# lxtGH/Video-K-Net

Hardware: AMD Instinct MI355X
Metric: frames/sec (S=3, N=100, 1024x2048) (higher is better)
Workload: dtype f32; 1 GPU; cfg2 video_knet_s3_r50: VideoKernelIterHead S=3, N=100 proposals + 17 stuff = 117 kernels, C=256, 1024x2048 frame -> 128x256 stride-8 features, ffn tracking link, x4 bilinear upsample of the final logits; streams_per_gpu=1, parallelism=frame-sharded dp1, x_storage=fp32

## Files before the change

include/vkn.h:

```cpp
#ifndef VKN_H
#define VKN_H
#include <stddef.h>
#include <stdint.h>

#ifdef __cplusplus
extern "C" {
#endif

#define VKN_VERSION 0x000600

#define VKN_OK 0
#define VKN_E_ARG (-1)
#define VKN_E_SHAPE (-2)
#define VKN_E_WORKSPACE (-3)
#define VKN_E_LAUNCH (-4)
#define VKN_E_ALIGN (-5)
#define VKN_E_RANGE (-6)

#define VKN_STATUS_RANGE 1u

#define VKN_FLAG_REF_KERNELS 1u
#define VKN_FLAG_EXACT_GEMM 2u
#define VKN_FLAG_LOGITS_HANDOFF 4u
#define VKN_FLAG_BITS_HANDOFF 16u
#define VKN_X_F32 0
#define VKN_X_F16 1
#define VKN_X_BF16 2
#define VKN_FLAG_X_F16 64u
#define VKN_FLAG_X_BF16 128u
#define VKN_FLAG_CHAIN_LAUNCHES 256u
#define VKN_FLAG_CHAIN_PERSISTENT 512u
#define VKN_FLAG_JOIN_EARLY 32768u
#define VKN_FLAG_LINK_RESERVE 262144u
#define VKN_FLAG_LINK_NO_RESERVE 524288u
#define VKN_FLAG_SCALED_F16 16384u
#define VKN_FLAG_CHAIN_BF16X3 65536u
#define VKN_FLAG_CHAIN_KSPLIT 8192u
#define VKN_FLAG_SERIAL_LINK 32u
#define VKN_FLAG_CLIP_LINK 8u

#define VKN_FLAG_INIT_SEPARATE 131072u
#define VKN_FLAG_PHASE_A 1024u
#define VKN_FLAG_PHASE_B 2048u
#define VKN_FLAG_PHASE_C 4096u
#define VKN_FLAG_PHASE_MASK (VKN_FLAG_PHASE_A | VKN_FLAG_PHASE_B | VKN_FLAG_PHASE_C)

#define VKN_MAX_FCS 4

typedef struct VknDims {
    int B;
    int N;
    int C;
    int H, W;
    int heads;
    int ff;
    int ncls;
    int n_cls_fcs, n_mask_fcs;
    float thr_logit;
    float ln_eps;
} VknDims;

typedef struct VknStageWeights {
    const float *ft_w, *ft_b, *ft_wT;
    const float *dyn_w, *dyn_b;
    const float *inp_w, *inp_b;
    const float *ig_w, *ig_b, *ug_w, *ug_b;
    const float *norm_in_w, *norm_in_b;
    const float *norm_out_w, *norm_out_b;
    const float *inorm_in_w, *inorm_in_b;
    const float *inorm_out_w, *inorm_out_b;
    const float *fc_w, *fc_b, *fc_norm_w, *fc_norm_b;
    const float *attn_in_w, *attn_in_b;
    const float *attn_out_w, *attn_out_b;
    const float *attn_norm_w, *attn_norm_b;
    const float *ffn1_w, *ffn1_b;
    const float *ffn2_w, *ffn2_b;
    const float *ffn_norm_w, *ffn_norm_b;
    const float *cls_fc_w[VKN_MAX_FCS], *cls_ln_w[VKN_MAX_FCS], *cls_ln_b[VKN_MAX_FCS];
    const float *fc_cls_w, *fc_cls_b;
    const float *mask_fc_w[VKN_MAX_FCS], *mask_ln_w[VKN_MAX_FCS], *mask_ln_b[VKN_MAX_FCS];
    const float *fc_mask_w, *fc_mask_b;
    const float *pa_in_w, *pa_in_b, *pa_out_w, *pa_out_b, *pa_norm_w, *pa_norm_b;
    const float *lffn1_w, *lffn1_b, *lffn2_w, *lffn2_b, *lffn_norm_w, *lffn_norm_b;
    const void* prepared;
    size_t prepared_bytes;
} VknStageWeights;

int vkn_version(void);
const char* vkn_strerror(int code);
int vkn_workspace_init(void* ws, size_t ws_bytes, void* stream);
int vkn_workspace_status(void* ws, size_t ws_bytes, void* stream);
size_t vkn_sizeof_dims(void);
size_t vkn_sizeof_stage_weights(void);

size_t vkn_gather_workspace_bytes(int B, int N, int C, int P);
int vkn_mask_gather_f32(const float* x, const float* mask_logits, float thr_logit, float* xraw_out, float* cnt_out, int B,
                        int N, int C, int P, void* ws, size_t ws_bytes, unsigned flags, void* stream);

int vkn_mask_gather_real_f32(const float* x, const float* a, float* out, float* asum_out, int B, int N, int C, int P, void* ws,
                             size_t ws_bytes, void* stream);

size_t vkn_decode_workspace_bytes(int B, int N, int C);
int vkn_mask_decode_f32(const float* x, const float* kernels, const float* bias, float* out, int B, int N, int C, int P,
                        void* ws, size_t ws_bytes, unsigned flags, void* stream);
int vkn_mask_decode_scaled_f32(const float* x, const float* kernels, const float* bias, const float* out_scale, float* out, int B,
                               int N, int C, int P, void* ws, size_t ws_bytes, unsigned flags, void* stream);

int vkn_split_planes_f32(const float* kernels, void* kf_hi, void* kf_lo, int B, int N, int C, void* stream);
int vkn_mask_decode_planes_f32(const float* x, const void* kf_hi, const void* kf_lo, const float* bias, float* out, int B,
                               int N, int C, int P, void* stream);
int vkn_mask_decode_planes_x(const void* x, int x_dtype, const void* kf_hi, const void* kf_lo, const float* bias, float* out, int B,
                             int N, int C, int P, void* stream);

int vkn_decode_gather_supported(int C, int P);
int vkn_decode_gather_f32(const float* x, const void* kf_hi, const void* kf_lo, const float* bias, float thr_logit,
                          float* xraw_out, float* cnt_out, int B, int N, int C, int P, void* ws, size_t ws_bytes, void* stream);
int vkn_decode_gather_x(const void* x, int x_dtype, const void* kf_hi, const void* kf_lo, const float* bias, float thr_logit,
                        float* xraw_out, float* cnt_out, int B, int N, int C, int P, void* ws, size_t ws_bytes, void* stream);

int vkn_upsample_bilinear_f32(const float* in, float* out, int planes, int H, int W, int S, void* stream);
int vkn_upsample_bilinear_f16out(const float* in, void* out_f16, int planes, int H, int W, int S, void* stream);
int vkn_upsample_bilinear_bwd_f32(const float* grad_out, float* grad_in, int planes, int H, int W, int S, void* stream);

int vkn_focal_loss_blocks(int M, int ncls);
int vkn_focal_loss_f32(const float* logits, const long long* labels, const float* weight, int weight_elementwise, int M, int ncls,
                       float alpha, float gamma, float* partial, float* grad, void* stream);

size_t vkn_prepared_bytes(const VknDims* d, const VknStageWeights* w);
int vkn_prepare_stage_f32(const VknDims* d, const VknStageWeights* w, void* prepared, size_t bytes, void* stream);

int vkn_split_weight_f32(const float* W, void* w_split, int Nout, int K, void* stream);
int vkn_linear_f32(const float* A, const float* W, const void* w_split, const float* bias, float* out, int M, int K, int Nout,
                   int act, int ksplit, void* ws, size_t ws_bytes, void* stream);

int vkn_split_weight_t_f32(const float* W, void* w_split_t, int Nout, int K, void* stream);
#define VKN_SPLIT_MAX_ITEMS 64
typedef struct VknSplitItem {
    const float* W;
    void* images;
    long long ldn, ldk;
    int Nout, K, kvalid, reserved;
} VknSplitItem;
size_t vkn_sizeof_split_item(void);
int vkn_split_weights_batch_f32(const VknSplitItem* items, int nitems, void* stream);
int vkn_linear_dw_f32(const float* dY, int ldy, const float* A, int lda, float* dW, float* db, int M, int K, int Nout, int accumulate,
                      void* stream);
#define VKN_DW_MAX_ITEMS 48
typedef struct VknDwItem {
    const float* dY;
    const float* A;
    float* dW;
    float* db;
    int ldy, lda, Nout, K;
} VknDwItem;
size_t vkn_sizeof_dw_item(void);
int vkn_linear_dw_batch_f32(const VknDwItem* items, int nitems, int M, void* stream);
int vkn_layernorm_act_fwd_f32(const float* in, int ldi, const float* resid, int ldr, const float* gamma, const float* beta, float eps,
                              int act, float* out, int ldo, float* stats, int M, int C, void* stream);
int vkn_layernorm_act_bwd_f32(const float* dy, int lddy, const float* in, int ldi, const float* resid, int ldr, const float* gamma,
                              const float* beta, const float* stats, int act, float* dx, int lddx, float* dgamma, float* dbeta, int M,
                              int C, void* stream);
typedef struct VknUpdatorNorms {
    const float *norm_in_w, *norm_in_b, *norm_out_w, *norm_out_b, *input_norm_in_w, *input_norm_in_b, *input_norm_out_w, *input_norm_out_b;
    const float *input_gate_b, *update_gate_b;
} VknUpdatorNorms;
typedef struct VknUpdatorNormGrads {
    float *norm_in_w, *norm_in_b, *norm_out_w, *norm_out_b, *input_norm_in_w, *input_norm_in_b, *input_norm_out_w, *input_norm_out_b;
} VknUpdatorNormGrads;
size_t vkn_sizeof_updator_norms(void);
size_t vkn_sizeof_updator_norm_grads(void);
int vkn_updator_gate_product_f32(const float* params, const float* inputs, float* gate_feats, int M, int C, void* stream);
int vkn_updator_gate_product_bwd_f32(const float* d_gate_feats, const float* params, const float* inputs, float* d_params, float* d_inputs,
                                     int M, int C, void* stream);
int vkn_updator_mix_fwd_f32(const float* gates, const float* params, const float* inputs, const VknUpdatorNorms* norms, float eps,
                            float* features, float* stats, int M, int C, void* stream);
int vkn_updator_mix_bwd_f32(const float* d_features, const float* gates, const float* params, const float* inputs,
                            const VknUpdatorNorms* norms, const float* stats, float* d_gates, float* d_params, float* d_inputs,
                            const VknUpdatorNormGrads* d_norms, int M, int C, void* stream);
int vkn_attention_f32(const float* Q, int ldq, const float* K, const float* V, int ldkv, float* out, int ldo, int B, int Nq, int Nk,
                      int heads, int hd, void* stream);
int vkn_attention_bwd_f32(const float* Q, int ldq, const float* K, const float* V, int ldkv, const float* O, int ldo, const float* dO,
                          int lddo, float* dQ, int lddq, float* dK, float* dV, int lddkv, int B, int Nq, int Nk, int heads, int hd,
                          void* stream);

int vkn_kernel_updator_f32(const VknDims* d, const VknStageWeights* w, const float* update_feature,
                           const float* input_feature, float* out, void* ws, size_t ws_bytes, void* stream);

size_t vkn_stage_workspace_bytes(const VknDims* d);
int vkn_stage_forward_f32(const VknDims* d, const VknStageWeights* w, const float* x, const float* obj_in,
                          const float* masks_in, const float* prev_obj, float* cls_logits, float* masks_out, float* obj_out,
                          float* x_feat_out, float* track_out, void* ws, size_t ws_bytes, unsigned flags, void* stream);

int vkn_track_link_f32(const VknDims* d, const VknStageWeights* w, const float* cur_obj, const float* prev_obj,
                       float* track_out, void* ws, size_t ws_bytes, void* stream);
int vkn_track_link_flags_f32(const VknDims* d, const VknStageWeights* w, const float* cur_obj, const float* prev_obj,
                             float* track_out, void* ws, size_t ws_bytes, unsigned flags, void* stream);

int vkn_link_block_f32(const VknDims* d, const VknStageWeights* w, const float* update_feature, const float* cur,
                       const float* prev, float* out, void* ws, size_t ws_bytes, void* stream);

size_t vkn_query_merge_workspace_bytes(const VknDims* d, int num_frames);
int vkn_query_merge_f32(const VknDims* d, int num_frames, const VknStageWeights* w, const float* query, const float* keys,
                        const float* pos, float* out, void* ws, size_t ws_bytes, void* stream);

int vkn_stage_forward_link_f32(const VknDims* d, const VknStageWeights* w, const VknStageWeights* link_pre,
                               const VknStageWeights* link_track, int track_src, const float* x, const float* obj_in,
                               const float* masks_in, const float* prev_obj, float* cls_logits, float* masks_out, float* obj_out,
                               float* x_feat_out, float* track_out, void* ws, size_t ws_bytes, unsigned flags, void* stream);

int vkn_stage_chain_f32(const VknDims* d, const VknStageWeights* w, const float* x_feat, const float* obj_in, float* cls_logits,
                        float* kernels_out, float* kb_out, float* obj_out, void* ws, size_t ws_bytes, unsigned flags,
                        void* stream);

size_t vkn_head_workspace_bytes(const VknDims* d);
int vkn_head_forward_f32(const VknDims* d, int num_stages, const VknStageWeights* stages, const float* x,
                         const float* proposal_feats, const float* mask_preds_in, const float* prev_obj, float* obj_out,
                         float* cls_prob, float* mask_preds_out, float* scaled_out, int upsample_stride, float* track_out,
                         void* ws, size_t ws_bytes, unsigned flags, void* stream);

int vkn_head_forward_link_f32(const VknDims* d, int num_stages, const VknStageWeights* stages, const VknStageWeights* link_pre,
                              const VknStageWeights* link_track, int track_src, const float* x, const float* proposal_feats,
                              const float* mask_preds_in, const float* prev_obj, float* obj_out, float* cls_prob,
                              float* mask_preds_out, float* scaled_out, int upsample_stride, float* track_out, void* ws,
                              size_t ws_bytes, unsigned flags, void* stream);

int vkn_head_forward_prof_f32(const VknDims* d, int num_stages, const VknStageWeights* stages, const float* x,
                              const float* proposal_feats, const float* mask_preds_in, const float* prev_obj, float* obj_out,
                              float* cls_prob, float* mask_preds_out, float* scaled_out, int upsample_stride, float* track_out,
                              void* ws, size_t ws_bytes, unsigned flags, void* stream, void* ev_decode_start,
                              void* ev_decode_stop);

size_t vkn_kernel_init_workspace_bytes(int B, int Np, int ncls, int C, int P);
int vkn_kernel_init_f32(const float* loc_feats, const float* sem_feats, const float* init_w, const float* seg_w,
                        const float* seg_b, int num_thing_classes, int cat_stuff, int with_obj, float thr_logit, float* x_feats,
                        float* mask_preds, float* seg_preds, float* proposal_feats, int B, int Np, int ncls, int C, int P,
                        void* ws, size_t ws_bytes, unsigned flags, void* stream);

typedef struct VknPanopticCfg {
    int num_proposals;
    int num_thing_classes;
    int max_per_img;
    float instance_score_thr;
    double overlap_thr;
    int up;
    int Hm, Wm;
    int Hb, Wb;
    int h, w;
    int Ho, Wo;
} VknPanopticCfg;
#define VKN_PANOPTIC_INFO_FIELDS 6
size_t vkn_sizeof_panoptic_cfg(void);
size_t vkn_panoptic_workspace_bytes(const VknPanopticCfg* cfg, int B, int N);
int vkn_panoptic_joint_f32(const VknPanopticCfg* cfg, const float* cls_prob, const float* mask_logits, int B, int N, int ncls,
                           int* panoptic_seg, int* info, int* nseg, int* bbox, void* ws, size_t ws_bytes, void* stream);

size_t vkn_merge_workspace_bytes(int Kt, int Ks);
int vkn_panoptic_thing_first_u8(const unsigned char* thing_masks, const float* thing_scores, const int* thing_labels,
                                const int* thing_order, int Kt, const unsigned char* stuff_masks, const int* stuff_labels,
                                const int* stuff_order, int Ks, int HW, double instance_score_thr, double iou_thr,
                                int stuff_max_area, int* panoptic_seg, int* info, int* nseg, void* ws, size_t ws_bytes,
                                void* stream);

typedef struct VknAssignCfg {
    float cls_weight, dice_weight, mask_weight;
    float focal_alpha, focal_gamma, focal_eps;
    float dice_eps;
    float dice_pred_min, mask_pred_min;
} VknAssignCfg;
size_t vkn_sizeof_assign_cfg(void);
size_t vkn_assign_workspace_bytes(int N, int G, int P);
int vkn_assign_costs_f32(const VknAssignCfg* cfg, const float* mask_logits, const float* cls_logits, const float* gt_masks,
                         const int* gt_labels, int N, int G, int ncls, int P, float* cost_out, void* ws, size_t ws_bytes,
                         void* stream);
typedef struct VknAssignProblem {
    const float* mask_logits;
    const float* cls_logits;
    const float* gt_masks;
    const int* gt_labels;
    int G;
    float* cost_out;
} VknAssignProblem;
size_t vkn_sizeof_assign_problem(void);
int vkn_assign_costs_batch_f32(const VknAssignCfg* cfg, const VknAssignProblem* probs, int nprob, int N, int ncls, int P, void* ws,
                               size_t ws_bytes, void* stream);
size_t vkn_assign_lowres_workspace_bytes(int nprob, int N, int Gmax, int h, int w, int S);
int vkn_assign_costs_lowres_batch_f32(const VknAssignCfg* cfg, const VknAssignProblem* probs, int nprob, int N, int ncls, int h, int w,
                                      int S, void* ws, size_t ws_bytes, void* stream);
int vkn_lsap_f32(const float* cost, int nr, int nc, int* row_ind, int* col_ind);
#define VKN_LSAP_MAX_BATCH 64
typedef struct VknLsapProblem {
    const float* cost;
    int nr, nc;
    long long* gt_inds;
    int* row_ind;
    int* col_ind;
} VknLsapProblem;
size_t vkn_sizeof_lsap_problem(void);
int vkn_lsap_batch_f32(const VknLsapProblem* probs, int nprob, int* status, void* stream);

int vkn_mask_losses_chunks(int P);
int vkn_mask_losses_blocks(int P);
int vkn_mask_losses_fwd_f32(const float* pred, const float* target, const long long* pos_rows, const int* rowk, int K, int B, int Ns,
                            int P, int with_rank, float* row_partial, float* lse, int* top, float* rank_partial, void* stream);
int vkn_mask_losses_bwd_f32(const float* pred, const float* target, const int* rowk, const float* rowcoef, const float* coef,
                            const float* lse, const int* top, int B, int Ns, int P, int with_rank, float* grad, void* stream);

#define VKN_TAIL_MAX_IMAGES 64
typedef struct VknTailImage {
    const int* row_ind;
    const int* col_ind;
    const long long* gt_labels;
    const long long* sem_cls;
    int k, n_sem;
    int gt_row0, sem_row0;
    int pos0;
    int reserved;
} VknTailImage;
typedef struct VknTailCfg {
    float w_cls, w_mask, w_dice, dice_eps, w_rank, avg_factor;
    int with_rank;
} VknTailCfg;
size_t vkn_sizeof_tail_image(void);
size_t vkn_sizeof_tail_cfg(void);
int vkn_stage_targets(const VknTailImage* imgs, int B, int N, int S, int T, int ncls, float pos_weight, long long* labels,
                      float* label_weights, float* row_weight, int* rowk, long long* pos_rows, int* tgt_row, int* status, void* stream);
int vkn_mask_losses_fwd_bank_f32(const float* pred, const float* bank, const int* tgt_row, const long long* pos_rows, const int* rowk,
                                 int K, int B, int Ns, int P, int with_rank, float* row_partial, float* lse, int* top,
                                 float* rank_partial, void* stream);
int vkn_stage_losses_final_f32(const VknTailCfg* cfg, const float* avg_factor_dev, const float* focal_partial, int n_focal,
                               const float* row_partial, int K, int nchunk, const float* rank_partial, int n_rank,
                               const float* cls_logits, const long long* labels, const long long* pos_rows, int ncls, int B, int P,
                               float* losses, float* dice_a, float* dice_bc, void* stream);
int vkn_mask_losses_bwd_bank_f32(const float* pred, const float* bank, const int* tgt_row, const int* rowk, const float* dice_a,
                                 const float* dice_bc, const float* g_mask, const float* g_dice, const float* g_rank, float w_mask,
                                 float w_dice, float w_rank, int K, const float* lse, const int* top, int B, int Ns, int P,
                                 int with_rank, float* grad, void* stream);
int vkn_mask_losses_bwd_lowres_f32(const float* low, const float* bank, const int* tgt_row, const int* rowk, const float* dice_a,
                                   const float* dice_bc, const float* g_mask, const float* g_dice, const float* g_rank, float w_mask,
                                   float w_dice, float w_rank, int K, const float* lse, const int* top, int B, int Ns, int h, int w, int S,
                                   int with_rank, float* grad_low, void* stream);
// ... 75 lines not shown
```

video-k-net_amd/csrc/vkn_api.hip:

```cpp
#include "../../include/vkn.h"
#include "../../include/vkn_decode.h"
#include "vkn_common.h"
#include "vkn_launch.h"

namespace {

struct Carver {
    char* base;
    size_t off;
    template <class T>
    T* take(size_t n) {
        off = (off + 255) & ~(size_t)255;
        T* p = base ? reinterpret_cast<T*>(base + off) : nullptr;
        off += n * sizeof(T);
        return p;
    }
};

inline bool aligned16(const void* p) { return (reinterpret_cast<uintptr_t>(p) & 15) == 0; }
inline int npt_of(int N) { return (N + 31) / 32 * 32; }

struct StageWs {
    float *part, *cntp, *xraw, *cnt, *xfeat, *params, *inputf, *ig, *ug, *f, *obj1, *qkv, *ao, *obj2, *h, *partial, *t1, *t2,
        *maskfeat, *kb, *kern32, *lq, *lkv, *lobj, *lupd, *lf;
    _Float16 *kfh, *kfl;
    int* status;
};


enum MasksFrom {
    FROM_LOGITS,
    FROM_BITS,
    FROM_GATHERED,
    FROM_XFEAT
};
enum MasksTo {
    TO_LOGITS,
    TO_BITS,
    TO_GATHER,
    TO_KERNELS,
    TO_NONE
};
struct StageCall {
    const VknStageWeights* w = nullptr;
    const float *x = nullptr, *obj_in = nullptr;
    float *obj_out = nullptr, *cls_logits = nullptr, *x_feat_out = nullptr;
    bool cls_sigmoid = false;
    MasksFrom from = FROM_LOGITS;
    const float *masks_in = nullptr, *xfeat_in = nullptr;
    const unsigned* bits_in = nullptr;
    MasksTo to = TO_LOGITS;
    float* masks_out = nullptr;
    unsigned* bits_out = nullptr;
    float *kern_out = nullptr, *kb_out = nullptr;
    hipEvent_t prof0 = nullptr, prof1 = nullptr, obj_ready = nullptr;
    float* up_out = nullptr;
    int up_stride = 0, up_chunk = 0;
    bool* up_done = nullptr;
    int link_reserve = 0;
    const float* prev_obj = nullptr;
    float* track_out = nullptr;
    const VknStageWeights* link_pre = nullptr;
    const float* prev_pre = nullptr;
    const VknStageWeights* link_track = nullptr;
    int track_src = 0;
    bool keep_xfeat = false;
    const void* touch_next = nullptr;
    size_t touch_next_bytes = 0;
};

struct PrepW {
    const void *ft, *ftT, *dyn, *inp, *ig, *ug, *fc, *attn_in, *attn_out, *ffn1, *ffn2, *cls_fc[VKN_MAX_FCS], *fc_cls,
        *mask_fc[VKN_MAX_FCS], *fc_mask, *pa_in, *pa_in_kv, *pa_out, *lffn1, *lffn2;
    const void *dynft, *dec;
    float *dynft32, *bcnt, *dec32, *decb, *dvec, *kb0, *fmT;
    float* chain_consts;
    const void* h2[VKN_H2_COUNT];
    float* h2_scale;
    unsigned* h2_scratch;
};

inline bool has_composites(const VknDims* d, const VknStageWeights* w) {
    return w->ft_w && w->ft_wT && w->ft_b && w->dyn_w && w->dyn_b && w->fc_mask_w && w->fc_mask_b && d->n_mask_fcs > 0;
}

struct PrepItem {
    const float* src;
    int nout, k;
    const void** dst;
};

struct H2Shape { int nout, k; };
inline H2Shape h2_shape(const VknDims* d, const VknStageWeights* w, int i) {
    const int C = d->C, FF = d->ff;
    switch (i) {
        case VKN_H2_DYNFT: case VKN_H2_DYN: case VKN_H2_INP: return H2Shape{2 * C, C};
        case VKN_H2_IN: return H2Shape{3 * C, C};
        case VKN_H2_FFN1: return H2Shape{FF, C};
        case VKN_H2_FFN2: return H2Shape{C, FF};
        case VKN_H2_FCCLS: return H2Shape{w->fc_cls_w ? d->ncls : 0, C};
        default: return H2Shape{C, C};
    }
}

inline bool chain_width_ok(const VknDims* d) { return d->C == 256 && d->ff % 256 == 0 && d->ff <= 2048; }
inline bool chain_shape_ok(const VknDims* d) { return chain_width_ok(d) && d->n_cls_fcs == 1 && d->n_mask_fcs == 1; }

size_t carve_prepared(const VknDims* d, const VknStageWeights* w, char* base, PrepW* p, PrepItem* it = nullptr, int* n_out = nullptr) {
    const int C = d->C, FF = d->ff;
    Carver c{base, 0};
    int n = 0;
    auto add = [&](const float* src, int nout, int k, const void** dst) {
        *dst = src ? c.take<char>(vkn_split_w3_bytes(nout, k)) : nullptr;
        if (src && it) it[n] = PrepItem{src, nout, k, dst};
        if (src) ++n;
    };
    add(w->ft_w, C, C, &p->ft); add(w->ft_wT, C, C, &p->ftT);
    add(w->dyn_w, 2 * C, C, &p->dyn); add(w->inp_w, 2 * C, C, &p->inp);
    add(w->ig_w, C, C, &p->ig); add(w->ug_w, C, C, &p->ug); add(w->fc_w, C, C, &p->fc);
    add(w->attn_in_w, 3 * C, C, &p->attn_in); add(w->attn_out_w, C, C, &p->attn_out);
    add(w->ffn1_w, FF, C, &p->ffn1); add(w->ffn2_w, C, FF, &p->ffn2);
    for (int i = 0; i < VKN_MAX_FCS; ++i) add(i < d->n_cls_fcs ? w->cls_fc_w[i] : nullptr, C, C, &p->cls_fc[i]);
    add(w->fc_cls_w, d->ncls, C, &p->fc_cls);
    for (int i = 0; i < VKN_MAX_FCS; ++i) add(i < d->n_mask_fcs ? w->mask_fc_w[i] : nullptr, C, C, &p->mask_fc[i]);
    add(w->fc_mask_w, C, C, &p->fc_mask);
    add(w->pa_in_w, C, C, &p->pa_in); add(w->pa_in_w ? w->pa_in_w + (size_t)C * C : nullptr, 2 * C, C, &p->pa_in_kv);
    add(w->pa_out_w, C, C, &p->pa_out);
    add(w->lffn1_w, FF, C, &p->lffn1); add(w->lffn2_w, C, FF, &p->lffn2);
    p->dynft = p->dec = nullptr;
    p->dynft32 = p->bcnt = p->dec32 = p->decb = p->dvec = p->kb0 = p->fmT = p->chain_consts = nullptr;
    if (has_composites(d, w)) {
        const size_t Cs = d->C;
        p->dynft = c.take<char>(vkn_split_w3_bytes(2 * C, C));
        p->dec = c.take<char>(vkn_split_w3_bytes(C, C));
        p->dynft32 = c.take<float>(2 * Cs * Cs);
        p->bcnt = c.take<float>(2 * Cs);
        p->dec32 = c.take<float>(Cs * Cs);
        p->decb = c.take<float>(Cs);
        p->dvec = c.take<float>(Cs);
        p->kb0 = c.take<float>(4);
        p->fmT = c.take<float>(Cs * Cs);
        if (C == 256 && FF <= 2048) p->chain_consts = c.take<float>(vkn_chain_consts_floats());
    }
    for (int i = 0; i < VKN_H2_COUNT; ++i) p->h2[i] = nullptr;
    p->h2_scale = nullptr;
    p->h2_scratch = nullptr;
    if (has_composites(d, w) && chain_shape_ok(d) && w->inp_w && w->ig_w && w->ug_w && w->fc_w && w->attn_in_w && w->attn_out_w && w->ffn1_w &&
        w->ffn2_w && w->cls_fc_w[0] && w->mask_fc_w[0]) {
        for (int i = 0; i < VKN_H2_COUNT; ++i) {
            const H2Shape h = h2_shape(d, w, i);
            if (h.nout > 0) p->h2[i] = c.take<char>(vkn_split_h2_bytes(h.nout, h.k));
        }
        p->h2_scale = c.take<float>(VKN_H2_COUNT * 8);
        p->h2_scratch = c.take<unsigned>(4);
    }
    if (n_out) *n_out = n;
    return (c.off + 255) & ~(size_t)255;
}

int ffn_hsplit(int M, int FF) {
    if (FF % 256 != 0) return 0;
    const int chunks = FF / 256, rt = (M + 31) / 32;
    int hs = 1;
    while (hs < chunks && rt * hs < 256 && chunks % (hs * 2) == 0) hs *= 2;
    return hs;
}

int ffn_ksplit(int M, int K) {
    const int rt = (M + 31) / 32, ktiles = K / 32;
    int ks = 256 / (rt > 0 ? rt : 1);
    if (ks > 16) ks = 16;
    if (ks > ktiles) ks = ktiles;
    if (ks < 1) ks = 1;
    return ks;
}

size_t carve_stage(const VknDims* d, char* base, StageWs* s) {
    Carver c{base, 0};
    const size_t B = d->B, N = d->N, C = d->C, P = (size_t)d->H * d->W, M = B * N, FF = d->ff;
    const size_t G = vkn_gather_groups(d->B, (int)P), NPT = npt_of(d->N);
    s->status = c.take<int>(64);
    s->part = c.take<float>(B * G * NPT * C);
    s->cntp = c.take<float>(B * G * NPT);
    s->xraw = c.take<float>(M * C);
    s->cnt = c.take<float>(M);
    s->xfeat = c.take<float>(M * C);
    s->params = c.take<float>(M * 2 * C);
    s->inputf = c.take<float>(M * 2 * C);
    s->ig = c.take<float>(M * 2 * C);
    s->ug = c.take<float>(M * C);
    s->f = c.take<float>(M * C);
    s->obj1 = c.take<float>(M * C);
    s->qkv = c.take<float>(M * 3 * C);
    s->ao = c.take<float>(M * C);
    s->obj2 = c.take<float>(M * C);
    s->h = c.take<float>(M * FF);
    {
        const size_t ks = (size_t)ffn_ksplit((int)M, (int)FF), hs = (size_t)ffn_hsplit((int)M, (int)FF);
        const size_t ks1 = (size_t)ffn_ksplit((int)N, (int)FF), hs1 = (size_t)ffn_hsplit((int)N, (int)FF);
        const size_t k4 = 4;
        const size_t a = (ks > hs ? (ks > k4 ? ks : k4) : (hs > k4 ? hs : k4)) * M * C, b1 = (ks1 > hs1 ? (ks1 > k4 ? ks1 : k4) : (hs1 > k4 ? hs1 : k4)) * N * C;
        s->partial = c.take<float>(a > b1 ? a : b1);
    }
    s->t1 = c.take<float>(M * C);
    s->t2 = c.take<float>(M * C);
    s->maskfeat = c.take<float>(M * C);
    s->kb = c.take<float>(M);
    s->kern32 = c.take<float>(M * C);
    s->lq = c.take<float>(M * C);
    s->lkv = c.take<float>(M * 2 * C);
    s->lobj = c.take<float>(M * C);
    s->lupd = c.take<float>(M * C);
    s->lf = c.take<float>(M * C);
    s->kfh = c.take<_Float16>(B * NPT * C);
    s->kfl = c.take<_Float16>(B * NPT * C);
    return (c.off + 255) & ~(size_t)255;
}

int stage_ws(const VknDims* d, void* ws, size_t ws_bytes, StageWs* s) {
    if (!ws || ws_bytes < carve_stage(d, nullptr, s) || !aligned16(ws)) return VKN_E_WORKSPACE;
    carve_stage(d, static_cast<char*>(ws), s);
    return VKN_OK;
}

struct GatherWs { float *part, *cntp, *cnt; };
size_t carve_gather(int B, int N, int C, int P, char* base, GatherWs* g) {
    const size_t G = vkn_gather_groups(B, P), NPT = npt_of(N);
    Carver c{base, 0};
    g->part = c.take<float>((size_t)B * G * NPT * C);
    g->cntp = c.take<float>((size_t)B * G * NPT);
    g->cnt = c.take<float>((size_t)B * N);
    return (c.off + 255) & ~(size_t)255;
}
size_t carve_planes(int B, int N, int C, char* base, _Float16** kfh, _Float16** kfl) {
    Carver c{base, 0};
    *kfh = c.take<_Float16>((size_t)B * npt_of(N) * C);
    *kfl = c.take<_Float16>((size_t)B * npt_of(N) * C);
    return (c.off + 255) & ~(size_t)255;
}

int check_dims(const VknDims* d) {
    if (!d) return VKN_E_ARG;
    if (d->B <= 0 || d->N <= 0 || d->C <= 0 || d->H <= 0 || d->W <= 0 || d->heads <= 0 || d->ff <= 0 || d->ncls <= 0)
        return VKN_E_ARG;
    if (d->C % 32 != 0 || d->C > 256) return VKN_E_SHAPE;
    if (d->C % d->heads != 0 || d->C / d->heads > 64 || (d->C % 8) != 0 || d->C / 8 > 64) return VKN_E_SHAPE;
    {
        const int hd = d->C / d->heads, hd8 = d->C / 8;
        if (hd < 4 || (hd & (hd - 1)) || hd8 < 4 || (hd8 & (hd8 - 1))) return VKN_E_SHAPE;
    }
    if (d->ff % 32 != 0) return VKN_E_SHAPE;
    if (d->N > 256) return VKN_E_SHAPE;
    if (d->ncls > 256) return VKN_E_SHAPE;
    if (d->n_cls_fcs < 0 || d->n_cls_fcs > VKN_MAX_FCS || d->n_mask_fcs < 0 || d->n_mask_fcs > VKN_MAX_FCS) return VKN_E_SHAPE;
    return VKN_OK;
}

inline int xdt_of(unsigned flags) { return (flags & VKN_FLAG_X_F16) ? 1 : ((flags & VKN_FLAG_X_BF16) ? 2 : 0); }

VknEpi mk_epi(const VknDims* d) {
    VknEpi e{};
    e.eps = d->ln_eps;
    return e;
}

#define VKN_TRY(expr)             \
    do {                          \
        const int rc_ = (expr);   \
        if (rc_ != VKN_OK) return rc_; \
    } while (0)

int run_ffn(const VknDims* d, const StageWs& s, const float* in, const float* w1, const void* w1s, const float* b1,
            const float* w2, const void* w2s, const float* b2, const float* nw, const float* nb, float* out, hipStream_t st) {
    const int M = d->B * d->N, C = d->C, FF = d->ff;
    VknEpi e = mk_epi(d);
    int hsplit = ffn_hsplit(M, FF);
    {
        const int hs_dbg = vkn_dbg_env("VKN_FFN_HS", 0);
        if (hs_dbg > 0 && hs_dbg <= hsplit) hsplit = hs_dbg;
    }
    if (w1s && w2s && C == 256 && hsplit > 0 && vkn_dbg_env("VKN_FFN_FUSED", 1) != 0) {
        e.bias = b2; e.resid = in; e.ldr = C; e.ln_w = nw; e.ln_b = nb; e.out = out; e.ldo = C;
        return vkn_launch_ffn_fused(in, C, w1s, b1, w2s, M, C, FF, hsplit, s.partial, e, st);
    }
    e.bias = b1; e.act = 1; e.out = s.h; e.ldo = FF;
    VKN_TRY(vkn_launch_gemm(in, nullptr, C, w1, w1s, M, C, FF, 1, nullptr, e, st));
    e = mk_epi(d);
    e.bias = b2; e.resid = in; e.ldr = C; e.ln_w = nw; e.ln_b = nb; e.out = out; e.ldo = C;
    return vkn_launch_gemm(s.h, nullptr, FF, w2, w2s, M, FF, C, ffn_ksplit(M, FF), s.partial, e, st);
}

int run_attention(const VknDims* d, const StageWs& s, const float* qsrc, const float* kvsrc, int heads, const float* in_w,
                  const void* in_ws, const void* in_kv_ws, const float* in_b, const float* out_w, const void* out_ws, const float* out_b,
                  const float* nw, const float* nb, float* out, hipStream_t st) {
    const int M = d->B * d->N, C = d->C, hd = C / heads;
    VknEpi e = mk_epi(d);
    if (qsrc == kvsrc) {
        e.bias = in_b; e.out = s.qkv; e.ldo = 3 * C;
        VKN_TRY(vkn_launch_gemm(qsrc, nullptr, C, in_w, in_ws, M, C, 3 * C, 1, nullptr, e, st));
        VKN_TRY(vkn_launch_attn(s.qkv, 3 * C, s.qkv + C, s.qkv + 2 * C, 3 * C, s.ao, C, d->B, d->N, d->N, heads, hd, st));
    } else {
        e.bias = in_b; e.out = s.lq; e.ldo = C;
        VKN_TRY(vkn_launch_gemm(qsrc, nullptr, C, in_w, in_ws, M, C, C, 1, nullptr, e, st));
        e = mk_epi(d);
        e.bias = in_b + C; e.out = s.lkv; e.ldo = 2 * C;
        VKN_TRY(vkn_launch_gemm(kvsrc, nullptr, C, in_w + (size_t)C * C, in_kv_ws, M, C, 2 * C, 1, nullptr, e, st));
        VKN_TRY(vkn_launch_attn(s.lq, C, s.lkv, s.lkv + C, 2 * C, s.ao, C, d->B, d->N, d->N, heads, hd, st));
    }
    e = mk_epi(d);
    e.bias = out_b; e.resid = qsrc; e.ldr = C; e.ln_w = nw; e.ln_b = nb; e.out = out; e.ldo = C;
    return vkn_launch_gemm(s.ao, nullptr, C, out_w, out_ws, M, C, C, 1, nullptr, e, st);
}

int run_updator(const VknDims* d, const VknStageWeights* w, const PrepW& pw, const float* xfeat, const float* xraw,
                const float* cnt, const float* obj_in, float* out, const StageWs& s, hipStream_t st) {
    const int C = d->C, M = d->B * d->N;
    const bool fuse = (C == 256);
    VknGemmProb pr[2];
    VknEpi e = mk_epi(d); e.out = s.params; e.ldo = 2 * C;
    if (fuse) { e.ln_w = w->norm_out_w; e.ln_b = w->norm_out_b; e.ln_from_col = C; }
    if (xraw && pw.dynft) {
        e.bias = pw.bcnt; e.rowscale = cnt; e.bias2 = w->dyn_b;
        pr[0] = VknGemmProb{xraw, nullptr, nullptr, nullptr, C, pw.dynft32, pw.dynft, 2 * C, e};
    } else {
        e.bias = w->dyn_b;
        pr[0] = VknGemmProb{xfeat, nullptr, nullptr, nullptr, C, w->dyn_w, pw.dyn, 2 * C, e};
    }
    e = mk_epi(d); e.bias = w->inp_b; e.out = s.inputf; e.ldo = 2 * C;
    if (fuse) { e.ln_w = w->inorm_out_w; e.ln_b = w->inorm_out_b; e.ln_from_col = C; }
    pr[1] = VknGemmProb{obj_in, nullptr, nullptr, nullptr, C, w->inp_w, pw.inp, 2 * C, e};
    VKN_TRY(vkn_launch_gemm_group(pr, 2, M, C, 1, nullptr, st));
    float* ig = s.ig;
    float* ug = fuse ? s.ig + C : s.ug;
    const int ldg = fuse ? 2 * C : C;
    e = mk_epi(d); e.bias = w->ig_b; e.ln_w = w->inorm_in_w; e.ln_b = w->inorm_in_b; e.act = 2; e.out = ig; e.ldo = ldg;
    pr[0] = VknGemmProb{s.inputf, s.params, nullptr, nullptr, 2 * C, w->ig_w, pw.ig, C, e};
    e = mk_epi(d); e.bias = w->ug_b; e.ln_w = w->norm_in_w; e.ln_b = w->norm_in_b; e.act = 2; e.out = ug; e.ldo = ldg;
    pr[1] = VknGemmProb{s.inputf, s.params, nullptr, nullptr, 2 * C, w->ug_w, pw.ug, C, e};
    VKN_TRY(vkn_launch_gemm_group(pr, 2, M, C, 1, nullptr, st));
    e = mk_epi(d); e.bias = w->fc_b; e.ln_w = w->fc_norm_w; e.ln_b = w->fc_norm_b; e.act = 1; e.out = out; e.ldo = C;
    if (fuse) {
        pr[0] = VknGemmProb{ug, s.params + C, ig, s.inputf + C, 2 * C, w->fc_w, pw.fc, C, e};
        return vkn_launch_gemm_group(pr, 1, M, C, 1, nullptr, st);
    }
    VKN_TRY(vkn_launch_ku_mix(s.params, s.inputf, ig, ug, w->norm_out_w, w->norm_out_b, w->inorm_out_w, w->inorm_out_b,
                              d->ln_eps, s.f, M, C, st));
    return vkn_launch_gemm(s.f, nullptr, C, w->fc_w, pw.fc, M, C, C, 1, nullptr, e, st);
}

bool link_ks_ok(const VknDims* d, const VknStageWeights* w, const PrepW& pw, unsigned flags);
int run_link_ks(const VknDims* d, const VknStageWeights* w, const PrepW& pw, const float* cur, const float* kv, float* out,
                const StageWs& s, hipStream_t st);
int run_link(const VknDims* d, const VknStageWeights* w, const PrepW& pw, const float* cur, const float* prev,
             float* out, const StageWs& s, hipStream_t st, const float* update_feature = nullptr, unsigned flags = 0) {
    if (!w->pa_in_w || !w->lffn1_w) return VKN_E_ARG;
    const float* kv = prev;
    if (update_feature) {
        if (!w->dyn_w) return VKN_E_ARG;
        StageWs su = s;
        su.f = s.lf;
        VKN_TRY(run_updator(d, w, pw, update_feature, nullptr, nullptr, prev, s.lupd, su, st));
        kv = s.lupd;
    }
    if (link_ks_ok(d, w, pw, flags)) return run_link_ks(d, w, pw, cur, kv, out, s, st);
    VKN_TRY(run_attention(d, s, cur, kv, 8, w->pa_in_w, pw.pa_in, pw.pa_in_kv, w->pa_in_b, w->pa_out_w, pw.pa_out, w->pa_out_b,
                          w->pa_norm_w, w->pa_norm_b, s.t1, st));
    return run_ffn(d, s, s.t1, w->lffn1_w, pw.lffn1, w->lffn1_b, w->lffn2_w, pw.lffn2, w->lffn2_b, w->lffn_norm_w,
                   w->lffn_norm_b, out, st);
}

int carve_pw(const VknDims* d, const VknStageWeights* w, unsigned flags, PrepW* pw) {
    *pw = PrepW{};
    if (w->prepared && !(flags & VKN_FLAG_EXACT_GEMM) &&
        carve_prepared(d, w, static_cast<char*>(const_cast<void*>(w->prepared)), pw) > w->prepared_bytes)
        return VKN_E_WORKSPACE;
    return VKN_OK;
}

int run_track_link(const VknDims* d, const StageWs& s, hipStream_t st, const float* cur, const float* prev, float* out,
                   const VknStageWeights* w, const VknStageWeights* link_track, int track_src, const float* xfeat, unsigned flags) {
    const VknStageWeights* lw = link_track ? link_track : w;
    PrepW pw;
    VKN_TRY(carve_pw(d, lw, flags, &pw));
    return run_link(d, lw, pw, cur, prev, out, s, st, link_track ? (track_src == 2 ? cur : xfeat) : nullptr, flags);
}

int run_gather(const VknDims* d, const float* x, const float* masks, const unsigned* bits, const StageWs& s, unsigned flags,
               hipStream_t st, const void* touch = nullptr, size_t touch_bytes = 0) {
    const int B = d->B, N = d->N, C = d->C, P = d->H * d->W, xdt = xdt_of(flags);
    if (flags & VKN_FLAG_REF_KERNELS) return vkn_launch_gather_ref(x, masks, d->thr_logit, s.xraw, s.cnt, B, N, C, P, st);
    if (bits) return vkn_launch_gather_bits(x, bits, s.xraw, s.cnt, s.part, s.cntp, B, N, C, P, st, xdt, s.status, touch, touch_bytes);
    return vkn_launch_gather(x, masks, d->thr_logit, s.xraw, s.cnt, s.part, s.cntp, B, N, C, P, st, xdt, s.status, touch, touch_bytes);
}

int final_decode(const VknDims* d, const float* x, const StageWs& s, const float* kb, float* masks_out, unsigned flags,
                 hipStream_t st, hipEvent_t prof0, hipEvent_t prof1, float* up_out, int up_stride, int up_chunk, bool* up_done,
                 int max_workgroups = 0) {
    const int B = d->B, N = d->N, C = d->C, P = d->H * d->W;
    if ((flags & VKN_FLAG_REF_KERNELS) || (P & 1)) return vkn_launch_decode_ref(x, s.kern32, kb, masks_out, B, N, C, P, st);
    const int ch = (up_out && up_chunk > 0 && up_chunk < B) ? up_chunk : B;
    const size_t NPTC = (size_t)npt_of(N) * C;
    for (int b0 = 0; b0 < B; b0 += ch) {
        const int bn = (B - b0 < ch) ? B - b0 : ch;
        const float* xb = reinterpret_cast<const float*>(reinterpret_cast<const char*>(x) + (size_t)b0 * C * P * (xdt_of(flags) ? 2 : 4));
        if (b0 == 0 && prof0 && hipEventRecord(prof0, st) != hipSuccess) return VKN_E_LAUNCH;
        VKN_TRY(vkn_launch_decode_wg(xb, s.kfh + b0 * NPTC, s.kfl + b0 * NPTC, kb ? kb + (size_t)b0 * N : nullptr,
                                     masks_out + (size_t)b0 * N * P, bn, N, C, P, ch == B ? max_workgroups : 0, st, xdt_of(flags)));
        if (b0 == 0 && prof1 && hipEventRecord(prof1, st) != hipSuccess) return VKN_E_LAUNCH;
        if (ch < B)
            VKN_TRY(vkn_launch_upsample(masks_out + (size_t)b0 * N * P,
                                        (flags & VKN_FLAG_SCALED_F16) ? reinterpret_cast<float*>(reinterpret_cast<_Float16*>(up_out) + (size_t)b0 * N * P * up_stride * up_stride)
                                                                      : up_out + (size_t)b0 * N * P * up_stride * up_stride,
                                        bn * N, d->H, d->W, up_stride, st, (flags & VKN_FLAG_SCALED_F16) ? 1 : 0));
    }
    if (ch < B && up_done) *up_done = true;
    return VKN_OK;
}

#define VKN_LINK_RESERVE_CUS 64
#define VKN_LINK_RESERVE_MIN_FRAMES 8
inline int link_reserve_wg(const VknDims* d, int mode, bool persistent_chain, unsigned flags) {
    const VknDecodeSplit dflt = vkn_decode_split(d->B, d->H * d->W, 0);
    const long long grid = (long long)d->B * dflt.G2;
    const int full = VKN_DECODE_CUS - VKN_LINK_RESERVE_CUS;
    if (mode == 2) {
        const long long q = grid * 3 / 4;
        return (int)(q > full ? full : (q < d->B ? d->B : q));
    }
    if (mode != 1 || !persistent_chain || d->B < VKN_LINK_RESERVE_MIN_FRAMES || xdt_of(flags) != 0) return 0;
    return grid == VKN_DECODE_CUS ? full : 0;
}

inline int persistent_min_row_tiles(const PrepW& pw, unsigned flags) {
    return (!(flags & VKN_FLAG_CHAIN_BF16X3) && pw.h2_scale && pw.h2[VKN_H2_DYNFT]) ? 22 : 64;
}
inline unsigned pw_off(const VknStageWeights* w, const void* p) {
    return (unsigned)(static_cast<const char*>(p) - static_cast<const char*>(w->prepared));
}
inline bool chain_weights_ok(const PrepW& pw, bool have_cls) {
    return pw.dynft && pw.dyn && pw.dec && pw.inp && pw.ig && pw.ug && pw.fc && pw.attn_in && pw.attn_out && pw.ffn1 && pw.ffn2 &&
           pw.cls_fc[0] && pw.mask_fc[0] && (!have_cls || pw.fc_cls);
}
inline bool chain_stage_ok(const VknDims* d, const VknStageWeights* w, const PrepW& pw, bool have_cls) {
    return chain_shape_ok(d) && w->prepared && w->prepared_bytes < (1ull << 31) && chain_weights_ok(pw, have_cls) && w->ffn1_w &&
           w->cls_ln_w[0] && w->mask_ln_w[0];
}
bool chain_fast_ok(const VknDims* d, const VknStageWeights* w, const PrepW& pw, unsigned flags, bool have_cls) {
    if (flags & (VKN_FLAG_CHAIN_LAUNCHES | VKN_FLAG_EXACT_GEMM)) return false;
    if (vkn_dbg_env("VKN_CHAIN_LAUNCHES", 0)) return false;
    if (!(flags & VKN_FLAG_CHAIN_PERSISTENT) && !vkn_dbg_env("VKN_CHAIN_PERSISTENT", 0) &&
        (d->B * d->N + 31) / 32 < persistent_min_row_tiles(pw, flags))
        return false;
    return pw.chain_consts && chain_stage_ok(d, w, pw, have_cls);
}
inline bool chain_h2(const PrepW& pw, unsigned flags, bool have_cls) {
    return !(flags & VKN_FLAG_CHAIN_BF16X3) && pw.h2_scale && pw.h2[VKN_H2_DYNFT] && pw.h2[VKN_H2_DEC] && (!have_cls || pw.h2[VKN_H2_FCCLS]);
}

int run_chain_fast(const VknDims* d, const VknStageWeights* w, const PrepW& pw, const float* a0, bool a0_raw, const float* cnt,
                   const float* obj_in, float* obj_out, float* cls_logits, bool cls_sigmoid, float* kern32_out, const StageWs& s,
                   hipStream_t st, bool h2 = false) {
    const int M = d->B * d->N, C = d->C;
    VknChainA a{};
    a.a0 = a0; a.obj_in = obj_in; a.rowscale = a0_raw ? cnt : nullptr;
    a.wbase = w->prepared; a.wbytes = w->prepared_bytes;
    if (h2) {
        a.off_dyn = pw_off(w, pw.h2[a0_raw ? VKN_H2_DYNFT : VKN_H2_DYN]);
        a.off_inp = pw_off(w, pw.h2[VKN_H2_INP]); a.off_ig = pw_off(w, pw.h2[VKN_H2_IG]); a.off_ug = pw_off(w, pw.h2[VKN_H2_UG]);
        a.off_fc = pw_off(w, pw.h2[VKN_H2_FC]); a.off_in = pw_off(w, pw.h2[VKN_H2_IN]);
    } else {
        a.off_dyn = pw_off(w, a0_raw ? pw.dynft : pw.dyn);
        a.off_inp = pw_off(w, pw.inp); a.off_ig = pw_off(w, pw.ig); a.off_ug = pw_off(w, pw.ug); a.off_fc = pw_off(w, pw.fc);
        a.off_in = pw_off(w, pw.attn_in);
    }
    a.consts = pw.chain_consts;
    a.eps = d->ln_eps; a.M = M; a.obj1 = s.obj1; a.qkv = s.qkv; a.status = s.status;
    VKN_TRY(h2 ? vkn_launch_chain_a_h2(a, st) : vkn_launch_chain_a(a, st));
    VKN_TRY(vkn_launch_attn(s.qkv, 3 * C, s.qkv + C, s.qkv + 2 * C, 3 * C, s.ao, C, d->B, d->N, d->N, d->heads, C / d->heads, st));
    VknChainC c{};
    c.ao = s.ao; c.obj1 = s.obj1; c.wbase = w->prepared; c.wbytes = w->prepared_bytes;
    if (h2) {
        c.off_out = pw_off(w, pw.h2[VKN_H2_OUT]); c.off_ffn1 = pw_off(w, pw.h2[VKN_H2_FFN1]); c.off_ffn2 = pw_off(w, pw.h2[VKN_H2_FFN2]);
        c.off_clsfc = pw_off(w, pw.h2[VKN_H2_CLSFC]); c.off_maskfc = pw_off(w, pw.h2[VKN_H2_MASKFC]);
        c.off_fccls = pw.h2[VKN_H2_FCCLS] ? pw_off(w, pw.h2[VKN_H2_FCCLS]) : 0u; c.off_dec = pw_off(w, pw.h2[VKN_H2_DEC]);
    } else {
        c.off_out = pw_off(w, pw.attn_out); c.off_ffn1 = pw_off(w, pw.ffn1); c.off_ffn2 = pw_off(w, pw.ffn2);
        c.off_clsfc = pw_off(w, pw.cls_fc[0]); c.off_maskfc = pw_off(w, pw.mask_fc[0]);
        c.off_fccls = pw.fc_cls ? pw_off(w, pw.fc_cls) : 0u; c.off_dec = pw_off(w, pw.dec);
    }
    c.consts = pw.chain_consts; c.kb0 = pw.kb0;
    c.ff = d->ff; c.ncls = d->ncls; c.cls_sigmoid = cls_sigmoid ? 1 : 0; c.eps = d->ln_eps; c.M = M;
    c.obj_out = obj_out; c.cls_out = cls_logits; c.kb_out = s.kb;
    if (kern32_out) c.kern_out = kern32_out;
    else { c.plane_hi = s.kfh; c.plane_lo = s.kfl; }
    c.rows_per_frame = d->N; c.NPT = npt_of(d->N); c.status = s.status;
    return h2 ? vkn_launch_chain_c_h2(c, st) : vkn_launch_chain_c(c, st);
}

#define VKN_KS_MAX_ROW_TILES 16
inline bool ks_width_ok(const VknDims* d) {
    return chain_width_ok(d) && (d->ff % 512 == 0 || d->ff <= 1024);
}
bool chain_ks_ok(const VknDims* d, const VknStageWeights* w, const PrepW& pw, unsigned flags, bool have_cls) {
    if (flags & (VKN_FLAG_CHAIN_LAUNCHES | VKN_FLAG_CHAIN_PERSISTENT | VKN_FLAG_EXACT_GEMM)) return false;
    if (vkn_dbg_env("VKN_CHAIN_LAUNCHES", 0) || vkn_dbg_env("VKN_CHAIN_PERSISTENT", 0) || !vkn_dbg_env("VKN_CHAIN_KSPLIT", 1)) return false;
    if (!(flags & VKN_FLAG_CHAIN_KSPLIT) && (d->B * d->N + 31) / 32 > VKN_KS_MAX_ROW_TILES) return false;
    if (!ks_width_ok(d) || !chain_stage_ok(d, w, pw, have_cls)) return false;
    const void* v16[] = {w->inorm_in_w, w->inorm_in_b, w->norm_in_w, w->norm_in_b, w->norm_out_w, w->norm_out_b, w->inorm_out_w, w->inorm_out_b,
                         w->fc_norm_w, w->fc_norm_b, w->attn_norm_w, w->attn_norm_b, w->ffn_norm_w, w->ffn_norm_b, w->ffn2_b,
                         w->cls_ln_w[0], w->cls_ln_b[0], w->mask_ln_w[0], w->mask_ln_b[0], pw.dvec};
    for (const void* p : v16)
        if (!p || !aligned16(p)) return false;
    return true;
}

VknKsProb ks_prob(const float* a, int lda, const void* W, int Nout, int KT, float eps) {
    VknKsProb p{};
    p.pro.a[0] = a; p.pro.lda[0] = lda; p.pro.nsum = 1; p.pro.eps = eps;
    p.Wsplit = W; p.Nout = Nout; p.KT = KT;
    return p;
}

int run_chain_ks(const VknDims* d, const VknStageWeights* w, const PrepW& pw, const float* a0, bool a0_raw, const float* cnt,
                 const float* obj_in, float* obj_out, float* cls_logits, bool cls_sigmoid, float* kern32_out, const StageWs& s,
                 hipStream_t st, hipEvent_t obj_ready) {
    const int M = d->B * d->N, C = d->C, FF = d->ff;
    const float eps = d->ln_eps;
    VknKsProb pr[2];
    pr[0] = ks_prob(a0, C, a0_raw ? pw.dynft : pw.dyn, 2 * C, 8, eps);
    if (a0_raw) { pr[0].epi.bias = pw.bcnt; pr[0].epi.rowscale = cnt; pr[0].epi.bias2 = w->dyn_b; }
    else pr[0].epi.bias = w->dyn_b;
    pr[0].epi.out = s.params; pr[0].epi.ldo = 2 * C;
    pr[1] = ks_prob(obj_in, C, pw.inp, 2 * C, 8, eps);
    pr[1].epi.bias = w->inp_b; pr[1].epi.out = s.inputf; pr[1].epi.ldo = 2 * C;
    VKN_TRY(vkn_launch_gemm_ks(pr, 2, 0, 0, 1, 0, M, st));
    pr[0] = ks_prob(s.inputf, 2 * C, pw.ig, C, 8, eps);
    pr[0].pro.a[1] = s.params; pr[0].pro.lda[1] = 2 * C;
    pr[1] = pr[0];
    pr[0].epi.bias = w->ig_b; pr[0].epi.out = s.ig; pr[0].epi.ldo = 2 * C;
    pr[1].Wsplit = pw.ug; pr[1].epi.bias = w->ug_b; pr[1].epi.out = s.ig + C; pr[1].epi.ldo = 2 * C;
    VKN_TRY(vkn_launch_gemm_ks(pr, 2, 1, 0, 1, 0, M, st));
    pr[0] = ks_prob(s.ig, 2 * C, pw.fc, C, 8, eps);
    pr[0].pro.a[1] = s.ig + C; pr[0].pro.lda[1] = 2 * C;
    pr[0].pro.a[2] = s.params + C; pr[0].pro.lda[2] = 2 * C;
    pr[0].pro.a[3] = s.inputf + C; pr[0].pro.lda[3] = 2 * C;
    pr[0].pro.ln_w[0] = w->inorm_in_w; pr[0].pro.ln_b[0] = w->inorm_in_b;
    pr[0].pro.ln_w[1] = w->norm_in_w; pr[0].pro.ln_b[1] = w->norm_in_b;
    pr[0].pro.ln_w[2] = w->norm_out_w; pr[0].pro.ln_b[2] = w->norm_out_b;
    pr[0].pro.ln_w[3] = w->inorm_out_w; pr[0].pro.ln_b[3] = w->inorm_out_b;
    pr[0].epi.bias = w->fc_b; pr[0].epi.out = s.f; pr[0].epi.ldo = C;
    VKN_TRY(vkn_launch_gemm_ks(pr, 1, 2, 0, 1, 0, M, st));
    pr[0] = ks_prob(s.f, C, pw.attn_in, 3 * C, 8, eps);
    pr[0].pro.ln_w[0] = w->fc_norm_w; pr[0].pro.ln_b[0] = w->fc_norm_b; pr[0].pro.act = 1;
    pr[0].pro.side_out = s.obj1; pr[0].pro.ld_side = C;
    pr[0].epi.bias = w->attn_in_b; pr[0].epi.out = s.qkv; pr[0].epi.ldo = 3 * C;
    VKN_TRY(vkn_launch_gemm_ks(pr, 1, 0, 0, 1, 0, M, st));
    VKN_TRY(vkn_launch_attn(s.qkv, 3 * C, s.qkv + C, s.qkv + 2 * C, 3 * C, s.ao, C, d->B, d->N, d->N, d->heads, C / d->heads, st));
    pr[0] = ks_prob(s.ao, C, pw.attn_out, C, 8, eps);
    pr[0].epi.bias = w->attn_out_b; pr[0].epi.resid = s.obj1; pr[0].epi.ldr = C; pr[0].epi.out = s.obj2; pr[0].epi.ldo = C;
    VKN_TRY(vkn_launch_gemm_ks(pr, 1, 0, 0, 1, 0, M, st));
    pr[0] = ks_prob(s.obj2, C, pw.ffn1, FF, 8, eps);
    pr[0].pro.ln_w[0] = w->attn_norm_w; pr[0].pro.ln_b[0] = w->attn_norm_b;
    pr[0].pro.side_out = s.t1; pr[0].pro.ld_side = C;
    pr[0].epi.bias = w->ffn1_b; pr[0].epi.act = 1; pr[0].epi.out = s.h; pr[0].epi.ldo = FF;
    VKN_TRY(vkn_launch_gemm_ks(pr, 1, 0, 0, 1, 0, M, st));
    const int kpw = (FF % 512 == 0) ? 2 : 1, zch = FF / (256 * kpw);
    pr[0] = ks_prob(s.h, FF, pw.ffn2, C, FF / 32, eps);
    pr[0].epi.out = s.partial; pr[0].epi.ldo = C;
    VKN_TRY(vkn_launch_gemm_ks(pr, 1, 0, zch, kpw, (long long)M * C, M, st));
    pr[0] = ks_prob(s.partial, C, pw.cls_fc[0], C, 8, eps);
    pr[0].pro.nsum = zch; pr[0].pro.sum_stride = (long long)M * C;
    pr[0].pro.pbias = w->ffn2_b; pr[0].pro.presid = s.t1; pr[0].pro.ldr = C;
    pr[0].pro.ln_w[0] = w->ffn_norm_w; pr[0].pro.ln_b[0] = w->ffn_norm_b;
    pr[1] = pr[0];
    pr[0].pro.side_out = obj_out; pr[0].pro.ld_side = C;
    pr[0].epi.out = s.lkv; pr[0].epi.ldo = 2 * C;
    pr[1].Wsplit = pw.mask_fc[0]; pr[1].epi.out = s.lkv + C; pr[1].epi.ldo = 2 * C;
    VKN_TRY(vkn_launch_gemm_ks(pr, 2, 0, 0, 1, 0, M, st));
    if (obj_ready && hipEventRecord(obj_ready, st) != hipSuccess) return VKN_E_LAUNCH;
    int np = 0;
    if (cls_logits) {
        pr[np] = ks_prob(s.lkv, 2 * C, pw.fc_cls, d->ncls, 8, eps);
        pr[np].pro.ln_w[0] = w->cls_ln_w[0]; pr[np].pro.ln_b[0] = w->cls_ln_b[0]; pr[np].pro.act = 1;
        pr[np].epi.bias = w->fc_cls_b; pr[np].epi.act = cls_sigmoid ? 2 : 0; pr[np].epi.out = cls_logits; pr[np].epi.ldo = d->ncls;
        ++np;
    }
    pr[np] = ks_prob(s.lkv + C, 2 * C, pw.dec, C, 8, eps);
    pr[np].pro.ln_w[0] = w->mask_ln_w[0]; pr[np].pro.ln_b[0] = w->mask_ln_b[0]; pr[np].pro.act = 1;
    pr[np].pro.dot_vec = pw.dvec; pr[np].pro.dot_bias = pw.kb0; pr[np].pro.dot_out = s.kb;
    pr[np].epi.bias = pw.decb; pr[np].epi.ldo = C;
    if (kern32_out) pr[np].epi.out = kern32_out;
    else { pr[np].epi.plane_hi = s.kfh; pr[np].epi.plane_lo = s.kfl; pr[np].epi.rows_per_frame = d->N; pr[np].epi.NPT = npt_of(d->N); }
    ++np;
    return vkn_launch_gemm_ks(pr, np, 0, 0, 1, 0, M, st);
}

bool link_ks_ok(const VknDims* d, const VknStageWeights* w, const PrepW& pw, unsigned flags) {
    if (flags & (VKN_FLAG_CHAIN_LAUNCHES | VKN_FLAG_CHAIN_PERSISTENT | VKN_FLAG_EXACT_GEMM)) return false;
    if (vkn_dbg_env("VKN_CHAIN_LAUNCHES", 0) || !vkn_dbg_env("VKN_CHAIN_KSPLIT", 1)) return false;
    if (!(flags & VKN_FLAG_CHAIN_KSPLIT) && (d->B * d->N + 31) / 32 > VKN_KS_MAX_ROW_TILES) return false;
    if (!ks_width_ok(d)) return false;
    if (!pw.pa_in || !pw.pa_in_kv || !pw.pa_out || !pw.lffn1 || !pw.lffn2) return false;
    if (!w->pa_norm_w || !w->pa_norm_b || !aligned16(w->pa_norm_w) || !aligned16(w->pa_norm_b)) return false;
    return true;
}

int run_link_ks(const VknDims* d, const VknStageWeights* w, const PrepW& pw, const float* cur, const float* kv, float* out,
                const StageWs& s, hipStream_t st) {
    const int M = d->B * d->N, C = d->C, FF = d->ff;
    const float eps = d->ln_eps;
    VknKsProb pr[2];
    pr[0] = ks_prob(cur, C, pw.pa_in, C, 8, eps);
    pr[0].epi.bias = w->pa_in_b; pr[0].epi.out = s.lq; pr[0].epi.ldo = C;
    pr[1] = ks_prob(kv, C, pw.pa_in_kv, 2 * C, 8, eps);
    pr[1].epi.bias = w->pa_in_b ? w->pa_in_b + C : nullptr; pr[1].epi.out = s.lkv; pr[1].epi.ldo = 2 * C;
    VKN_TRY(vkn_launch_gemm_ks(pr, 2, 0, 0, 1, 0, M, st));
    VKN_TRY(vkn_launch_attn(s.lq, C, s.lkv, s.lkv + C, 2 * C, s.ao, C, d->B, d->N, d->N, 8, C / 8, st));
    pr[0] = ks_prob(s.ao, C, pw.pa_out, C, 8, eps);
    pr[0].epi.bias = w->pa_out_b; pr[0].epi.resid = cur; pr[0].epi.ldr = C; pr[0].epi.out = s.t1; pr[0].epi.ldo = C;
    VKN_TRY(vkn_launch_gemm_ks(pr, 1, 0, 0, 1, 0, M, st));
    pr[0] = ks_prob(s.t1, C, pw.lffn1, FF, 8, eps);
    pr[0].pro.ln_w[0] = w->pa_norm_w; pr[0].pro.ln_b[0] = w->pa_norm_b;
    pr[0].pro.side_out = s.lf; pr[0].pro.ld_side = C;
    pr[0].epi.bias = w->lffn1_b; pr[0].epi.act = 1; pr[0].epi.out = s.h; pr[0].epi.ldo = FF;
    VKN_TRY(vkn_launch_gemm_ks(pr, 1, 0, 0, 1, 0, M, st));
    const int kpw = (FF % 512 == 0) ? 2 : 1, zch = FF / (256 * kpw);
    pr[0] = ks_prob(s.h, FF, pw.lffn2, C, FF / 32, eps);
    pr[0].epi.out = s.partial; pr[0].epi.ldo = C;
    VKN_TRY(vkn_launch_gemm_ks(pr, 1, 0, zch, kpw, (long long)M * C, M, st));
    VknEpi e = mk_epi(d);
    e.bias = w->lffn2_b; e.resid = s.lf; e.ldr = C; e.ln_w = w->lffn_norm_w; e.ln_b = w->lffn_norm_b; e.out = out; e.ldo = C;
    return vkn_launch_rowepi(s.partial, zch, M, C, e, st);
}

int emit_masks(const VknDims* d, const StageCall& c, const StageWs& s, bool ref_decode, const float* kern32, const float* kb,
               const void* touch, size_t touch_bytes, unsigned flags, hipStream_t st, bool persistent_chain = false) {
    const int B = d->B, N = d->N, C = d->C, P = d->H * d->W, xdt = xdt_of(flags);
    if (c.to == TO_KERNELS) {
        if (c.kb_out && kb && hipMemcpyAsync(c.kb_out, kb, (size_t)B * N * sizeof(float), hipMemcpyDeviceToDevice, st) != hipSuccess)
            return VKN_E_LAUNCH;
        return VKN_OK;
    }
    if (c.to == TO_NONE) return VKN_OK;
    if (ref_decode) return vkn_launch_decode_ref(c.x, kern32, kb, c.masks_out, B, N, C, P, st);
    if (c.to == TO_GATHER)
        return vkn_launch_fused_decode_gather(c.x, s.kfh, s.kfl, kb, d->thr_logit, s.xraw, s.cnt, s.part, s.cntp, B, N, C, P, st, xdt, s.status,
                                              touch, touch_bytes);
    if (c.to == TO_BITS) return vkn_launch_decode_bits(c.x, s.kfh, s.kfl, kb, c.bits_out, d->thr_logit, B, N, C, P, st, xdt);
    return final_decode(d, c.x, s, kb, c.masks_out, flags, st, c.prof0, c.prof1, c.up_out, c.up_stride, c.up_chunk, c.up_done,
                        link_reserve_wg(d, c.link_reserve, persistent_chain, flags));
}

int run_stage(const VknDims* d, const StageCall& c, const StageWs& s, unsigned flags, hipStream_t st) {
    const VknStageWeights* w = c.w;
    const int N = d->N, C = d->C, P = d->H * d->W, M = d->B * N;
    const bool ref = (flags & VKN_FLAG_REF_KERNELS) != 0;
    const bool chain_only = c.to == TO_KERNELS, given_xfeat = c.from == FROM_XFEAT;
    const bool ref_decode = ref || (P & 1) || chain_only;
    const bool has_ft = w->ft_w != nullptr;
    const bool have_cls = w->fc_cls_w && c.cls_logits;
    float* const cls_logits = have_cls ? c.cls_logits : nullptr;
    const bool pre_link = c.link_pre && c.prev_pre;
    const bool need_xfeat = (pre_link && c.link_pre->dyn_w) || (c.link_track && c.track_src == 1) || c.keep_xfeat;
    if (xdt_of(flags) && !chain_only && (ref || (P % 64) != 0)) return VKN_E_SHAPE;
    PrepW pw;
    VKN_TRY(carve_pw(d, w, flags, &pw));
    const bool comp = pw.dynft != nullptr;
    const bool fewrow = comp && chain_ks_ok(d, w, pw, flags, have_cls), persistent = comp && chain_fast_ok(d, w, pw, flags, have_cls);
    const bool fast = fewrow || persistent;

    const bool will_fast = !given_xfeat && persistent && vkn_dbg_env("VKN_CHAIN_TOUCH", 1);
    const void* touch_nx = vkn_dbg_env("VKN_CHAIN_TOUCH", 1) ? c.touch_next : nullptr;
    const size_t touch_nx_bytes = touch_nx ? c.touch_next_bytes : 0;
    if (c.from == FROM_LOGITS || c.from == FROM_BITS)
        VKN_TRY(run_gather(d, c.x, c.masks_in, c.from == FROM_BITS ? c.bits_in : nullptr, s, flags, st, will_fast ? w->prepared : nullptr,
                           will_fast ? w->prepared_bytes : 0));

    float* xfeat = c.x_feat_out ? c.x_feat_out : s.xfeat;
    VknEpi e = mk_epi(d);
    if (given_xfeat) {
        xfeat = const_cast<float*>(c.xfeat_in);
    } else if (has_ft) {
        if (!comp || c.x_feat_out || need_xfeat) {
            e.bias = w->ft_b; e.rowscale = s.cnt; e.out = xfeat; e.ldo = C;
            VKN_TRY(vkn_launch_gemm(s.xraw, nullptr, C, w->ft_w, pw.ft, M, C, C, 1, nullptr, e, st));
        }
    } else {
        if (hipMemcpyAsync(xfeat, s.xraw, (size_t)M * C * sizeof(float), hipMemcpyDeviceToDevice, st) != hipSuccess)
            return VKN_E_LAUNCH;
    }

    const float* obj_in = c.obj_in;
    if (pre_link) {
        PrepW pl;
        VKN_TRY(carve_pw(d, c.link_pre, flags, &pl));
        VKN_TRY(run_link(d, c.link_pre, pl, obj_in, c.prev_pre, s.lobj, s, st, c.link_pre->dyn_w ? xfeat : nullptr, flags));
        obj_in = s.lobj;
    }

    const float* kb = has_ft ? s.kb : nullptr;
    float* const kern32 = ref_decode ? (chain_only ? c.kern_out : s.kern32) : nullptr;
    const bool link = c.prev_obj && c.track_out;
    if (fast) {
        const bool raw = !given_xfeat;
        if (fewrow) {
            VKN_TRY(run_chain_ks(d, w, pw, raw ? s.xraw : xfeat, raw, s.cnt, obj_in, c.obj_out, cls_logits, c.cls_sigmoid, kern32, s, st, c.obj_ready));
        } else {
            VKN_TRY(run_chain_fast(d, w, pw, raw ? s.xraw : xfeat, raw, s.cnt, obj_in, c.obj_out, cls_logits, c.cls_sigmoid, kern32, s, st,
                                   chain_h2(pw, flags, have_cls)));
            if (c.obj_ready && hipEventRecord(c.obj_ready, st) != hipSuccess) return VKN_E_LAUNCH;
        }
        VKN_TRY(emit_masks(d, c, s, ref_decode, s.kern32, kb, touch_nx, touch_nx_bytes, flags, st, !fewrow));
        if (link) VKN_TRY(run_track_link(d, s, st, c.obj_out, c.prev_obj, c.track_out, w, c.link_track, c.track_src, xfeat, flags));
        return VKN_OK;
    }

    VKN_TRY(run_updator(d, w, pw, xfeat, (comp && !given_xfeat) ? s.xraw : nullptr, s.cnt, obj_in, s.obj1, s, st));

    VKN_TRY(run_attention(d, s, s.obj1, s.obj1, d->heads, w->attn_in_w, pw.attn_in, nullptr, w->attn_in_b, w->attn_out_w,
                          pw.attn_out, w->attn_out_b, w->attn_norm_w, w->attn_norm_b, s.obj2, st));
    if (w->ffn1_w) {
        VKN_TRY(run_ffn(d, s, s.obj2, w->ffn1_w, pw.ffn1, w->ffn1_b, w->ffn2_w, pw.ffn2, w->ffn2_b, w->ffn_norm_w,
                        w->ffn_norm_b, c.obj_out, st));
    } else {
        if (hipMemcpyAsync(c.obj_out, s.obj2, (size_t)M * C * sizeof(float), hipMemcpyDeviceToDevice, st) != hipSuccess)
            return VKN_E_LAUNCH;
    }
    const float* obj3 = c.obj_out;

    const bool fork_late = vkn_dbg_env("VKN_LINK_FORK_LATE", 0) != 0;
    if (c.obj_ready && !fork_late && hipEventRecord(c.obj_ready, st) != hipSuccess) return VKN_E_LAUNCH;

    const float* tc = obj3;
    const float* tm = obj3;
    const int nl = d->n_cls_fcs > d->n_mask_fcs ? d->n_cls_fcs : d->n_mask_fcs;
    VknGemmProb pr[2];
    for (int i = 0; i < nl; ++i) {
        int np = 0;
        if (i < d->n_cls_fcs) {
            float* dst = (i & 1) ? s.t2 : s.t1;
            e = mk_epi(d); e.ln_w = w->cls_ln_w[i]; e.ln_b = w->cls_ln_b[i]; e.act = 1; e.out = dst; e.ldo = C;
            pr[np++] = VknGemmProb{tc, nullptr, nullptr, nullptr, C, w->cls_fc_w[i], pw.cls_fc[i], C, e};
            tc = dst;
        }
        if (i < d->n_mask_fcs) {
            float* dst = (i & 1) ? s.lq : s.f;
            e = mk_epi(d); e.ln_w = w->mask_ln_w[i]; e.ln_b = w->mask_ln_b[i]; e.act = 1; e.out = dst; e.ldo = C;
            if (comp && i == d->n_mask_fcs - 1) { e.dot_vec = pw.dvec; e.dot_bias = pw.kb0; e.dot_out = s.kb; }
            pr[np++] = VknGemmProb{tm, nullptr, nullptr, nullptr, C, w->mask_fc_w[i], pw.mask_fc[i], C, e};
            tm = dst;
        }
        VKN_TRY(vkn_launch_gemm_group(pr, np, M, C, 1, nullptr, st));
    }
    auto to_kernels = [&](VknEpi& ep) {
        ep.ldo = C;
        if (kern32) ep.out = kern32;
        else { ep.plane_hi = s.kfh; ep.plane_lo = s.kfl; ep.rows_per_frame = N; ep.NPT = npt_of(N); }
    };
    int np = 0;
    if (have_cls) {
        e = mk_epi(d); e.bias = w->fc_cls_b; e.out = cls_logits; e.ldo = d->ncls;
        if (c.cls_sigmoid) e.act = 2;
        pr[np++] = VknGemmProb{tc, nullptr, nullptr, nullptr, C, w->fc_cls_w, pw.fc_cls, d->ncls, e};
    }
    const float* kern = s.kern32;
    if (comp) {
        e = mk_epi(d); e.bias = pw.decb; to_kernels(e);
        pr[np++] = VknGemmProb{tm, nullptr, nullptr, nullptr, C, pw.dec32, pw.dec, C, e};
        VKN_TRY(vkn_launch_gemm_group(pr, np, M, C, 1, nullptr, st));
    } else {
        e = mk_epi(d); e.bias = w->fc_mask_b; e.out = (chain_only && !has_ft) ? c.kern_out : s.maskfeat; e.ldo = C;
        if (has_ft) { e.dot_vec = w->ft_b; e.dot_out = s.kb; }
        pr[np++] = VknGemmProb{tm, nullptr, nullptr, nullptr, C, w->fc_mask_w, pw.fc_mask, C, e};
        VKN_TRY(vkn_launch_gemm_group(pr, np, M, C, 1, nullptr, st));
        if (has_ft) {
            e = mk_epi(d); to_kernels(e);
            VKN_TRY(vkn_launch_gemm(s.maskfeat, nullptr, C, w->ft_wT, pw.ftT, M, C, C, 1, nullptr, e, st));
        } else if (chain_only) {
            if (c.kb_out && hipMemsetAsync(c.kb_out, 0, (size_t)M * sizeof(float), st) != hipSuccess) return VKN_E_LAUNCH;
        } else if (!ref_decode) {
            VKN_TRY(vkn_launch_split_planes(s.maskfeat, s.kfh, s.kfl, d->B, N, C, st));
        } else if (c.to == TO_NONE) {
            if (hipMemcpyAsync(s.kern32, s.maskfeat, (size_t)M * C * sizeof(float), hipMemcpyDeviceToDevice, st) != hipSuccess)
                return VKN_E_LAUNCH;
        } else {
            kern = s.maskfeat;
        }
    }
    VKN_TRY(emit_masks(d, c, s, ref_decode, kern, kb, touch_nx, touch_nx_bytes, flags, st));

    if (c.obj_ready && fork_late && hipEventRecord(c.obj_ready, st) != hipSuccess) return VKN_E_LAUNCH;
    if (link) VKN_TRY(run_track_link(d, s, st, obj3, c.prev_obj, c.track_out, w, c.link_track, c.track_src, xfeat, flags));
    return VKN_OK;
}

StageWs frame_ws(const StageWs& s, const VknDims* d, int b) {
    StageWs r = s;
    const size_t R = (size_t)b * d->N, C = d->C;
    r.xraw += R * C; r.cnt += R; r.xfeat += R * C; r.params += R * 2 * C; r.inputf += R * 2 * C; r.ig += R * 2 * C; r.ug += R * C;
    r.f += R * C; r.obj1 += R * C; r.qkv += R * 3 * C; r.ao += R * C; r.obj2 += R * C; r.h += R * d->ff; r.t1 += R * C; r.t2 += R * C;
    r.maskfeat += R * C; r.kb += R; r.kern32 += R * C; r.lq += R * C; r.lkv += R * 2 * C; r.lobj += R * C; r.lupd += R * C; r.lf += R * C;
    r.kfh += (size_t)b * npt_of(d->N) * C; r.kfl += (size_t)b * npt_of(d->N) * C;
    return r;
}

struct InitWs {
    _Float16 *ih, *il, *sh, *sl;
    float *part, *cntp, *cnt, *obj, *seg;
    _Float16 *ph, *pl;
    unsigned* bits;
};
size_t carve_init(int B, int Np, int ncls, int C, int P, bool need_seg, char* base, InitWs* s) {
    Carver c{base, 0};
    const size_t G = vkn_gather_groups(B, P), NPTp = npt_of(Np), NPTs = npt_of(ncls > 0 ? ncls : 1);
    s->ih = c.take<_Float16>(NPTp * C);
    s->il = c.take<_Float16>(NPTp * C);
    s->sh = c.take<_Float16>(NPTs * C);
    s->sl = c.take<_Float16>(NPTs * C);
    s->part = c.take<float>((size_t)B * G * NPTp * C);
    s->cntp = c.take<float>((size_t)B * G * NPTp);
    s->cnt = c.take<float>((size_t)B * Np);
    s->obj = c.take<float>((size_t)B * Np * C);
    s->seg = need_seg ? c.take<float>((size_t)B * ncls * P) : nullptr;
    s->ph = s->pl = nullptr;
    s->bits = nullptr;
    if (ncls > 0 && vkn_init_pass_supported(Np, ncls, C, P)) {
        s->ph = c.take<_Float16>((size_t)160 * C);
        s->pl = c.take<_Float16>((size_t)160 * C);
        s->bits = c.take<unsigned>((size_t)B * (P / 32) * NPTp);
    }
    return (c.off + 255) & ~(size_t)255;
}

}

extern "C" {

int vkn_version(void) { return VKN_VERSION; }
size_t vkn_sizeof_dims(void) { return sizeof(VknDims); }
size_t vkn_sizeof_stage_weights(void) { return sizeof(VknStageWeights); }

const char* vkn_strerror(int code) {
    switch (code) {
        case VKN_OK: return "ok";
        case VKN_E_ARG: return "invalid argument (null pointer or non-positive size)";
        case VKN_E_SHAPE:
            return "unsupported shape (need C % 32 == 0, C <= 256, N <= 256, head_dim a power of two in [4, 64], ff % 32 == 0, ncls <= 256, "
                   "conv_kernel_size == 1)";
        case VKN_E_WORKSPACE: return "workspace missing or too small";
        case VKN_E_LAUNCH: return "HIP launch failed";
        case VKN_E_ALIGN: return "pointer not 16-byte aligned";
        case VKN_E_RANGE:
            return "feature map outside the f16-split envelope: |x| >= 65504 or a non-finite x reached a mask gather (its sums are not finite)";
        default: return "unknown error";
    }
}

size_t vkn_gather_workspace_bytes(int B, int N, int C, int P) {
    if (B <= 0 || N <= 0 || C <= 0 || P <= 0) return 0;
    GatherWs g;
    return carve_gather(B, N, C, P, nullptr, &g);
}

int vkn_mask_gather_f32(const float* x, const float* mask_logits, float thr_logit, float* xraw_out, float* cnt_out, int B,
                        int N, int C, int P, void* ws, size_t ws_bytes, unsigned flags, void* stream) {
    if (!x || !mask_logits || !xraw_out || B <= 0 || N <= 0 || C <= 0 || P <= 0) return VKN_E_ARG;
    if (!aligned16(x) || !aligned16(mask_logits) || !aligned16(xraw_out)) return VKN_E_ALIGN;
    if (C % 32 != 0 || C > 256 || N > 256) return VKN_E_SHAPE;
    if (!ws || ws_bytes < vkn_gather_workspace_bytes(B, N, C, P) || !aligned16(ws)) return VKN_E_WORKSPACE;
    GatherWs g;
    carve_gather(B, N, C, P, static_cast<char*>(ws), &g);
    float* cnt = cnt_out ? cnt_out : g.cnt;
    hipStream_t st = static_cast<hipStream_t>(stream);
    if (flags & VKN_FLAG_REF_KERNELS) {
        if (xdt_of(flags)) return VKN_E_SHAPE;
        return vkn_launch_gather_ref(x, mask_logits, thr_logit, xraw_out, cnt, B, N, C, P, st);
    }
    return vkn_launch_gather(x, mask_logits, thr_logit, xraw_out, cnt, g.part, g.cntp, B, N, C, P, st, xdt_of(flags));
}

int vkn_mask_gather_real_f32(const float* x, const float* a, float* out, float* asum_out, int B, int N, int C, int P, void* ws,
                             size_t ws_bytes, void* stream) {
    if (!x || !a || !out || B <= 0 || N <= 0 || C <= 0 || P <= 0) return VKN_E_ARG;
    if (!aligned16(x) || !aligned16(a) || !aligned16(out)) return VKN_E_ALIGN;
    if (C % 32 != 0 || C > 256 || N > 256) return VKN_E_SHAPE;
    if (!ws || ws_bytes < vkn_gather_workspace_bytes(B, N, C, P) || !aligned16(ws)) return VKN_E_WORKSPACE;
    GatherWs g;
    carve_gather(B, N, C, P, static_cast<char*>(ws), &g);
    return vkn_launch_gather_real(x, a, out, asum_out ? asum_out : g.cnt, g.part, g.cntp, B, N, C, P, N, static_cast<hipStream_t>(stream));
}

size_t vkn_decode_workspace_bytes(int B, int N, int C) {
    if (B <= 0 || N <= 0 || C <= 0) return 0;
    _Float16 *kfh, *kfl;
    return carve_planes(B, N, C, nullptr, &kfh, &kfl);
}

int vkn_mask_decode_f32(const float* x, const float* kernels, const float* bias, float* out, int B, int N, int C, int P,
                        void* ws, size_t ws_bytes, unsigned flags, void* stream) {
    if (!x || !kernels || !out || B <= 0 || N <= 0 || C <= 0 || P <= 0) return VKN_E_ARG;
    if (!aligned16(x) || !aligned16(kernels) || !aligned16(out)) return VKN_E_ALIGN;
    if (C % 32 != 0 || C > 256 || N > 256) return VKN_E_SHAPE;
    hipStream_t st = static_cast<hipStream_t>(stream);
    if ((flags & VKN_FLAG_REF_KERNELS) || (P & 1)) {
        if (xdt_of(flags)) return VKN_E_SHAPE;
        return vkn_launch_decode_ref(x, kernels, bias, out, B, N, C, P, st);
    }
    if (!ws || ws_bytes < vkn_decode_workspace_bytes(B, N, C) || !aligned16(ws)) return VKN_E_WORKSPACE;
    _Float16 *kfh, *kfl;
    carve_planes(B, N, C, static_cast<char*>(ws), &kfh, &kfl);
    VKN_TRY(vkn_launch_split_planes(kernels, kfh, kfl, B, N, C, st));
    return vkn_launch_decode(x, kfh, kfl, bias, out, B, N, C, P, st, xdt_of(flags));
}

int vkn_mask_decode_scaled_f32(const float* x, const float* kernels, const float* bias, const float* out_scale, float* out, int B,
                               int N, int C, int P, void* ws, size_t ws_bytes, unsigned flags, void* stream) {
    if (!x || !kernels || !out || !out_scale || B <= 0 || N <= 0 || C <= 0 || P <= 0) return VKN_E_ARG;
    if (!aligned16(x) || !aligned16(kernels) || !aligned16(out)) return VKN_E_ALIGN;
    if (C % 32 != 0 || C > 256 || N > 256) return VKN_E_SHAPE;
    if ((flags & VKN_FLAG_REF_KERNELS) || (P & 1)) return VKN_E_SHAPE;
    if (!ws || ws_bytes < vkn_decode_workspace_bytes(B, N, C) || !aligned16(ws)) return VKN_E_WORKSPACE;
    hipStream_t st = static_cast<hipStream_t>(stream);
    _Float16 *kfh, *kfl;
    carve_planes(B, N, C, static_cast<char*>(ws), &kfh, &kfl);
    VKN_TRY(vkn_launch_split_planes(kernels, kfh, kfl, B, N, C, st));
    return vkn_launch_decode_ex(x, kfh, kfl, bias, out, B, N, C, P, 0, N, st, xdt_of(flags), out_scale);
}

int vkn_split_planes_f32(const float* kernels, void* kf_hi, void* kf_lo, int B, int N, int C, void* stream) {
    if (!kernels || !kf_hi || !kf_lo || B <= 0 || N <= 0 || C <= 0) return VKN_E_ARG;
    if (!aligned16(kf_hi) || !aligned16(kf_lo)) return VKN_E_ALIGN;
    return vkn_launch_split_planes(kernels, static_cast<_Float16*>(kf_hi), static_cast<_Float16*>(kf_lo), B, N, C,
                                   static_cast<hipStream_t>(stream));
}

int vkn_mask_decode_planes_f32(const float* x, const void* kf_hi, const void* kf_lo, const float* bias, float* out, int B,
                               int N, int C, int P, void* stream) {
    return vkn_mask_decode_planes_x(x, VKN_X_F32, kf_hi, kf_lo, bias, out, B, N, C, P, stream);
}

int vkn_mask_decode_planes_x(const void* x, int x_dtype, const void* kf_hi, const void* kf_lo, const float* bias, float* out, int B,
                             int N, int C, int P, void* stream) {
    if (!x || !kf_hi || !kf_lo || !out || B <= 0 || N <= 0 || C <= 0 || P <= 0 || x_dtype < 0 || x_dtype > 2) return VKN_E_ARG;
    if (!aligned16(x) || !aligned16(kf_hi) || !aligned16(kf_lo) || !aligned16(out)) return VKN_E_ALIGN;
    if (C % 32 != 0 || C > 256 || N > 256) return VKN_E_SHAPE;
    return vkn_launch_decode(static_cast<const float*>(x), static_cast<const _Float16*>(kf_hi), static_cast<const _Float16*>(kf_lo),
                             bias, out, B, N, C, P, static_cast<hipStream_t>(stream), x_dtype);
}

int vkn_mask_decode_planes_wg_f32(const float* x, const void* kf_hi, const void* kf_lo, const float* bias, float* out, int B,
// ... 663 lines not shown
```

video-k-net_amd/csrc/vkn_fused.hip:

```cpp
#include "vkn_common.h"
#include "vkn_launch.h"

#define FU_THREADS 256
#define FU_WAVES 4
#define FU_TILE 64

typedef unsigned int fu_u32x2 __attribute__((ext_vector_type(2)));

#ifdef VKN_DEBUG
#include "../../tools/experiments/fused_variants.inc"
#endif

#define FS_THREADS 512
#define FS_TILE 32

#define FS_V_DEFAULT 7
#ifdef VKN_DEBUG
__device__ unsigned long long g_fs_prof[8][8];
#define FS_STAMP(k)                                                     \
    do {                                                                \
        if constexpr ((V & 8) != 0) {                                   \
            const unsigned long long now_ = __builtin_amdgcn_s_memtime(); \
            prof[k] += now_ - tprev;                                    \
            tprev = now_;                                               \
        }                                                               \
    } while (0)
#else
#define FS_STAMP(k) do { } while (0)
#endif
typedef short fs_short4 __attribute__((ext_vector_type(4)));
typedef short fs_short8 __attribute__((ext_vector_type(8)));
#define FS_WRITELANE(wd, val, row) asm volatile("v_writelane_b32 %0, %1, %2" : "+v"(wd) : "s"(val), "n"(row))

#ifdef VKN_DEBUG
#include "../../tools/experiments/fused_older.inc"
#endif

template <int NB, int C, int XH = 0, int PF = 0>
__global__ __launch_bounds__(FS_THREADS, 2) void k_fused_il(const float* __restrict__ x, const _Float16* __restrict__ kfh,
                                                             const _Float16* __restrict__ kfl, const float* __restrict__ kb,
                                                             float thr, float* __restrict__ part, float* __restrict__ cntp,
                                                             int N, int NPT, int n0_in, int P, int NZ) {
    constexpr int KS = C / 16;
    constexpr int NFG = KS / 16, NFD = KS / 4 - NFG, NF = NFD;
    static_assert(KS % 4 == 0 && 4 * (NFD + NFG) == KS, "C must be a multiple of 64");
    constexpr int NCB = C / 32;
    constexpr int CBW = (NCB + 3) / 4;
    constexpr bool ALLDEC = (NB == 4), ALLCB = (NCB % 4) == 0;
    constexpr int LDK = C + 8;
    constexpr int PLANE = FS_TILE * LDK;
    constexpr int IMG = 2 * PLANE;
    constexpr int V = PF ? 8 : 0;

    extern __shared__ __attribute__((aligned(16))) char smem[];
    _Float16* dimg = reinterpret_cast<_Float16*>(smem);
    half8* lut = reinterpret_cast<half8*>(dimg + 3 * IMG);
    unsigned* wbits = reinterpret_cast<unsigned*>(lut + 256);
    float* kbs = reinterpret_cast<float*>(wbits + 256);

    const int b = blockIdx.y, gidx = blockIdx.x / NZ, G = gridDim.x / NZ;
    const int n0 = n0_in + (blockIdx.x - gidx * NZ) * (NB * 32);
    const int tid = threadIdx.x, lane = tid & 63;
    const int wave = __builtin_amdgcn_readfirstlane(tid >> 6);
    const int g = lane >> 5, li = lane & 31;
    unsigned long long prof[8] = {0, 0, 0, 0, 0, 0, 0, 0}, tprev = 0;
    (void)prof; (void)tprev;

    const int nsup = ((P >> 6) - gidx + G - 1) / G;
    const int T = 2 * nsup;
    auto tile_p0 = [&](int t) { return (((t >> 1) * G + gidx) << 6) + ((t & 1) << 5); };

    for (int v = tid; v < 256; v += FS_THREADS) {
        half8 h;
#pragma unroll
        for (int e = 0; e < 8; ++e) h[e] = ((v >> ((e >> 1) + 4 * (e & 1))) & 1) ? (_Float16)1.f : (_Float16)0.f;
        lut[v] = h;
    }
    if (tid < 128) {
        const int n = n0 + tid;
        kbs[tid] = (kb && tid < NB * 32 && n < N) ? kb[(size_t)b * N + n] : 0.f;
        wbits[128 + tid] = 0u;
    }
    for (int v = tid; v < IMG / 8; v += FS_THREADS)
        reinterpret_cast<half8*>(dimg + 2 * IMG)[v] = half8{0, 0, 0, 0, 0, 0, 0, 0};

    const __amdgpu_buffer_rsrc_t xrs =
        XH ? __builtin_amdgcn_make_buffer_rsrc(const_cast<unsigned short*>(reinterpret_cast<const unsigned short*>(x) + (size_t)b * C * P), 0,
                                               C * P * 2, 0x00020000)
           : __builtin_amdgcn_make_buffer_rsrc(const_cast<float*>(x + (size_t)b * C * P), 0, C * P * 4, 0x00020000);
    const int lq = lane >> 4, lp = lane & 15;
    constexpr int XSH = XH ? 1 : 2;
    const int voff = (((lq << 2) * P + 2 * lp) << XSH);
    fu_u32x2 raw[2][NF][4];
    auto frag_ks = [&](int f) { return wave < 4 ? wave + 4 * f : 4 * NFD + (wave - 4) + 4 * f; };
    auto issue = [&](int slot, int t, int f) {
        const int ks = frag_ks(f);
        {
            const int soff = ((ks << 4) * P + tile_p0(t)) << XSH;
#pragma unroll
            for (int e = 0; e < 4; ++e) {
                if (XH) raw[slot][f][e] = fu_u32x2{__builtin_amdgcn_raw_buffer_load_b32(xrs, voff, soff + ((e * P) << 1), 0), 0u};
                else raw[slot][f][e] = __builtin_amdgcn_raw_buffer_load_b64(xrs, voff, soff + ((e * P) << 2), 3);
            }
        }
    };
    auto commit = [&](int slot, int buf, int f) {
        const int ks = frag_ks(f);
        {
            half4 h0, l0, h1, l1;
#pragma unroll
            for (int e = 0; e < 4; ++e) {
                const unsigned u0 = raw[slot][f][e][0], u1 = raw[slot][f][e][1];
                _Float16 h, l;
                if (XH == 1) {
                    h0[e] = __builtin_bit_cast(_Float16, (unsigned short)(u0 & 0xFFFFu));
                    h1[e] = __builtin_bit_cast(_Float16, (unsigned short)(u0 >> 16));
                } else if (XH == 2) {
                    h0[e] = (_Float16)__uint_as_float(u0 << 16);
                    h1[e] = (_Float16)__uint_as_float(u0 & 0xFFFF0000u);
                } else {
                    vkn_split_f16(__uint_as_float(u0), h, l);
                    h0[e] = h;
                    l0[e] = l;
                    vkn_split_f16(__uint_as_float(u1), h, l);
                    h1[e] = h;
                    l1[e] = l;
                }
            }
            _Float16* dh = dimg + (size_t)buf * IMG + lp * LDK + (ks << 4) + (lq << 2);
            *reinterpret_cast<half4*>(dh) = h0;
            *reinterpret_cast<half4*>(dh + 16 * LDK) = h1;
            if (!XH) {
                *reinterpret_cast<half4*>(dh + PLANE) = l0;
                *reinterpret_cast<half4*>(dh + 16 * LDK + PLANE) = l1;
            }
        }
    };
    half4 ch0, cl0, ch1, cl1;
    auto loader_unit = [&](int nf, int slot, int buf, int tnext, int u) {
        const int NU = nf * 4;
        if (!XH && !VKN_ABL_IS(PF, 4) && u < NU) {
            const int ff = u >> 2, j = u & 3, px = j >> 1, ep = j & 1, ks = frag_ks(ff);
            vkn_half2 h2, l2;
            vkn_split_f16x2(__uint_as_float(raw[slot][ff][2 * ep][px]), __uint_as_float(raw[slot][ff][2 * ep + 1][px]), h2, l2);
            if (px == 0) {
                ch0[2 * ep] = h2[0]; ch0[2 * ep + 1] = h2[1];
                cl0[2 * ep] = l2[0]; cl0[2 * ep + 1] = l2[1];
            } else {
                ch1[2 * ep] = h2[0]; ch1[2 * ep + 1] = h2[1];
                cl1[2 * ep] = l2[0]; cl1[2 * ep + 1] = l2[1];
            }
            if (j == 3) {
                _Float16* dh = dimg + (size_t)buf * IMG + lp * LDK + (ks << 4) + (lq << 2);
                *reinterpret_cast<half4*>(dh) = ch0;
                *reinterpret_cast<half4*>(dh + 16 * LDK) = ch1;
                *reinterpret_cast<half4*>(dh + PLANE) = cl0;
                *reinterpret_cast<half4*>(dh + 16 * LDK + PLANE) = cl1;
            }
        } else if (u < NU) {
            const int ff = u >> 2, e = u & 3, ks = frag_ks(ff);
            {
                const unsigned u0 = raw[slot][ff][e][0], u1 = raw[slot][ff][e][1];
                _Float16 h, l;
                if (XH == 1) {
                    ch0[e] = __builtin_bit_cast(_Float16, (unsigned short)(u0 & 0xFFFFu));
                    ch1[e] = __builtin_bit_cast(_Float16, (unsigned short)(u0 >> 16));
                } else if (XH == 2) {
                    ch0[e] = (_Float16)__uint_as_float(u0 << 16);
                    ch1[e] = (_Float16)__uint_as_float(u0 & 0xFFFF0000u);
                } else {
                    vkn_split_f16(__uint_as_float(u0), h, l);
                    ch0[e] = h;
                    cl0[e] = l;
                    vkn_split_f16(__uint_as_float(u1), h, l);
                    ch1[e] = h;
                    cl1[e] = l;
                }
                if (e == 3) {
                    _Float16* dh = dimg + (size_t)buf * IMG + lp * LDK + (ks << 4) + (lq << 2);
                    *reinterpret_cast<half4*>(dh) = ch0;
                    *reinterpret_cast<half4*>(dh + 16 * LDK) = ch1;
                    if (!XH) {
                        *reinterpret_cast<half4*>(dh + PLANE) = cl0;
                        *reinterpret_cast<half4*>(dh + 16 * LDK + PLANE) = cl1;
                    }
                }
            }
        } else if (u < 2 * NU) {
            const int v = u - NU, ff = v >> 2, e = v & 3, ks = frag_ks(ff);
            {
                const int soff = ((ks << 4) * P + tile_p0(tnext)) << XSH;
                if (XH) raw[slot][ff][e] = fu_u32x2{__builtin_amdgcn_raw_buffer_load_b32(xrs, voff, soff + ((e * P) << 1), 0), 0u};
                else raw[slot][ff][e] = __builtin_amdgcn_raw_buffer_load_b64(xrs, voff, soff + ((e * P) << 2), 3);
            }
        }
    };
    const int tlast = max(T - 1, 0);
    float* pp = part + ((size_t)b * G + gidx) * NPT * C;

    if (wave < 4) {
        if constexpr (PF == 2) __builtin_amdgcn_s_setprio(2);
        const bool has_dec = wave < NB;
        half8 Ah[KS], Al[KS];
        {
            const int n = n0 + wave * 32 + li;
            const bool ok = has_dec && (n < N);
            const size_t base = ((size_t)b * NPT + (ok ? n : 0)) * C + (g << 3);
#pragma unroll
            for (int ks = 0; ks < KS; ++ks) {
                half8 vh = {0, 0, 0, 0, 0, 0, 0, 0}, vl = {0, 0, 0, 0, 0, 0, 0, 0};
                if (ok) {
                    vh = *reinterpret_cast<const half8*>(kfh + base + (ks << 4));
                    vl = *reinterpret_cast<const half8*>(kfl + base + (ks << 4));
                }
                Ah[ks] = vh;
                Al[ks] = vl;
            }
        }
        unsigned cnt_i = 0;
#pragma unroll
        for (int f = 0; f < NFD; ++f) issue(0, 0, f);
#pragma unroll
        for (int f = 0; f < NFD; ++f) issue(1, min(1, tlast), f);
        __builtin_amdgcn_s_waitcnt(0x0F70);
        __builtin_amdgcn_sched_barrier(0);
#pragma unroll
        for (int f = 0; f < NFD; ++f) commit(0, 0, f);
        __builtin_amdgcn_sched_barrier(0);
#pragma unroll
        for (int f = 0; f < NFD; ++f) issue(0, min(2, tlast), f);
        __syncthreads();
#ifdef VKN_DEBUG
        if constexpr (PF != 0) tprev = __builtin_amdgcn_s_memtime();
#endif
        for (int i0 = 0; i0 < T; i0 += 2) {
#pragma unroll
            for (int u = 0; u < 2; ++u) {
                const int i = i0 + u;
                f32x16 acc;
                const _Float16* bp = dimg + (size_t)(i % 3) * IMG + li * LDK + (g << 3);
#pragma unroll
                for (int r = 0; r < 16; ++r) acc[r] = kbs[wave * 32 + vkn_cd_row(r, lane)];
                {
                    half8 rbh[3], rbl[3];
                    auto ldb = [&](int slot, int ks) {
                        rbh[slot] = *reinterpret_cast<const half8*>(bp + (ks << 4));
                        if (!XH) rbl[slot] = *reinterpret_cast<const half8*>(bp + (ks << 4) + PLANE);
                    };
                    ldb(0, 0);
                    if (KS > 1) ldb(1, 1);
                    constexpr int NUNIT = 2 * NFD * 4;
#pragma unroll
                    for (int ks = 0; ks < KS; ++ks) {
                        if (ks + 2 < KS) ldb((ks + 2) % 3, ks + 2);
                        if (ALLDEC || has_dec) {
                            acc = __builtin_amdgcn_mfma_f32_32x32x16_f16(Ah[ks], rbh[ks % 3], acc, 0, 0, 0);
                            if (!XH) acc = __builtin_amdgcn_mfma_f32_32x32x16_f16(Ah[ks], rbl[ks % 3], acc, 0, 0, 0);
                            acc = __builtin_amdgcn_mfma_f32_32x32x16_f16(Al[ks], rbh[ks % 3], acc, 0, 0, 0);
                        }
#pragma unroll
                        for (int uu = (ks * NUNIT) / KS; uu < ((ks + 1) * NUNIT) / KS; ++uu) loader_unit(NFD, u ^ 1, (i + 1) % 3, min(i + 3, tlast), uu);
                        __builtin_amdgcn_sched_barrier(0);
                    }
                }
                if (ALLDEC || has_dec) {
                    unsigned long long m[16];
#pragma unroll
                    for (int r = 0; r < 16; ++r) m[r] = __ballot(acc[r] >= thr);
                    __builtin_amdgcn_sched_barrier(0);
                    int wd = 0;
#define FS_WL2(r) (int)(unsigned)m[r], (int)(unsigned)(m[r] >> 32)
#define FS_WL8(wd, r0)                                                                                                              \
    asm volatile("v_writelane_b32 %0, %1, %17\n\tv_writelane_b32 %0, %2, %18\n\tv_writelane_b32 %0, %3, %19\n\tv_writelane_b32 %0, %4, %20\n\t"   \
                 "v_writelane_b32 %0, %5, %21\n\tv_writelane_b32 %0, %6, %22\n\tv_writelane_b32 %0, %7, %23\n\tv_writelane_b32 %0, %8, %24\n\t"   \
                 "v_writelane_b32 %0, %9, %25\n\tv_writelane_b32 %0, %10, %26\n\tv_writelane_b32 %0, %11, %27\n\tv_writelane_b32 %0, %12, %28\n\t" \
                 "v_writelane_b32 %0, %13, %29\n\tv_writelane_b32 %0, %14, %30\n\tv_writelane_b32 %0, %15, %31\n\tv_writelane_b32 %0, %16, %32"      \
                 : "+v"(wd)                                                                                                         \
                 : "s"((int)(unsigned)m[r0]), "s"((int)(unsigned)(m[r0] >> 32)), "s"((int)(unsigned)m[r0 + 1]),                     \
                   "s"((int)(unsigned)(m[r0 + 1] >> 32)), "s"((int)(unsigned)m[r0 + 2]), "s"((int)(unsigned)(m[r0 + 2] >> 32)),      \
                   "s"((int)(unsigned)m[r0 + 3]), "s"((int)(unsigned)(m[r0 + 3] >> 32)), "s"((int)(unsigned)m[r0 + 4]),              \
                   "s"((int)(unsigned)(m[r0 + 4] >> 32)), "s"((int)(unsigned)m[r0 + 5]), "s"((int)(unsigned)(m[r0 + 5] >> 32)),      \
                   "s"((int)(unsigned)m[r0 + 6]), "s"((int)(unsigned)(m[r0 + 6] >> 32)), "s"((int)(unsigned)m[r0 + 7]),              \
                   "s"((int)(unsigned)(m[r0 + 7] >> 32)), "n"(FS_ROW(r0)), "n"(FS_ROW(r0) + 4), "n"(FS_ROW(r0 + 1)),                 \
                   "n"(FS_ROW(r0 + 1) + 4), "n"(FS_ROW(r0 + 2)), "n"(FS_ROW(r0 + 2) + 4), "n"(FS_ROW(r0 + 3)), "n"(FS_ROW(r0 + 3) + 4), \
                   "n"(FS_ROW(r0 + 4)), "n"(FS_ROW(r0 + 4) + 4), "n"(FS_ROW(r0 + 5)), "n"(FS_ROW(r0 + 5) + 4), "n"(FS_ROW(r0 + 6)),   \
                   "n"(FS_ROW(r0 + 6) + 4), "n"(FS_ROW(r0 + 7)), "n"(FS_ROW(r0 + 7) + 4))
#define FS_ROW(r) (((r)&3) + 8 * ((r) >> 2))
                    FS_WL8(wd, 0);
                    FS_WL8(wd, 8);
                    if (lane < 32) {
                        wbits[(i & 1) * 128 + wave * 32 + lane] = (unsigned)wd;
                        cnt_i += __popc((unsigned)wd);
                    }
                }
                __builtin_amdgcn_sched_barrier(0);
                FS_STAMP(4);
                __syncthreads();
                FS_STAMP(5);
            }
        }
#ifdef VKN_DEBUG
        if constexpr (PF != 0)
            if (lane == 0 && blockIdx.x == 0 && blockIdx.y == 0)
                for (int k = 0; k < 8; ++k) g_fs_prof[wave][k] = prof[k];
#endif
        if (has_dec && lane < 32 && n0 + wave * 32 + lane < NPT) cntp[((size_t)b * G + gidx) * NPT + n0 + wave * 32 + lane] = (float)cnt_i;
    } else {
        if constexpr (PF == 3) __builtin_amdgcn_s_setprio(2);
        const int gw = wave - 4;
        f32x16 accg[CBW][NB];
#pragma unroll
        for (int j = 0; j < CBW; ++j)
#pragma unroll
            for (int nb = 0; nb < NB; ++nb)
#pragma unroll
                for (int r = 0; r < 16; ++r) accg[j][nb][r] = 0.f;
#pragma unroll
        for (int f = 0; f < NFG; ++f) issue(0, 0, f);
#pragma unroll
        for (int f = 0; f < NFG; ++f) issue(1, min(1, tlast), f);
        __builtin_amdgcn_s_waitcnt(0x0F70);
        __builtin_amdgcn_sched_barrier(0);
#pragma unroll
        for (int f = 0; f < NFG; ++f) commit(0, 0, f);
        __builtin_amdgcn_sched_barrier(0);
#pragma unroll
        for (int f = 0; f < NFG; ++f) issue(0, min(2, tlast), f);
        __syncthreads();
        constexpr int NSTEP = 2 * CBW;
        half8 a[2][NB], fbh[3], fbl[3];
        typedef __attribute__((address_space(3))) fs_short4 lds_s4;
        const int tg = lane >> 4, ta = (lane >> 2) & 3, tq = lane & 3;
        const int toff = (4 * (tg >> 1) + (ta >> 1) + 16 * (ta & 1)) * LDK + 16 * (tg & 1) + 4 * tq;
        auto ldf = [&](int slot, int st, const _Float16* dh) {
            const int cb = gw + 4 * (st >> 1);
            if (ALLCB || cb < NCB) {
                const _Float16* cp = dh + toff + (8 * (st & 1)) * LDK + cb * 32;
                const fs_short4 h0 = __builtin_amdgcn_ds_read_tr16_b64_v4i16((lds_s4*)(cp));
                const fs_short4 h1 = __builtin_amdgcn_ds_read_tr16_b64_v4i16((lds_s4*)(cp + 2 * LDK));
                fbh[slot] = __builtin_bit_cast(half8, (fs_short8)__builtin_shufflevector(h0, h1, 0, 1, 2, 3, 4, 5, 6, 7));
                if (!XH) {
                    const fs_short4 l0 = __builtin_amdgcn_ds_read_tr16_b64_v4i16((lds_s4*)(cp + PLANE));
                    const fs_short4 l1 = __builtin_amdgcn_ds_read_tr16_b64_v4i16((lds_s4*)(cp + PLANE + 2 * LDK));
                    fbl[slot] = __builtin_bit_cast(half8, (fs_short8)__builtin_shufflevector(l0, l1, 0, 1, 2, 3, 4, 5, 6, 7));
                }
            }
        };
        auto prep = [&](int img, int wb) {
            const _Float16* dh = dimg + (size_t)img * IMG;
#pragma unroll
            for (int nb = 0; nb < NB; ++nb) {
                const unsigned wv = wbits[wb * 128 + nb * 32 + li];
#pragma unroll
                for (int ps = 0; ps < 2; ++ps)
                    a[ps][nb] = lut[((wv >> (8 * ps + 4 * g)) & 0xFu) | (((wv >> (16 + 8 * ps + 4 * g)) & 0xFu) << 4)];
            }
            ldf(0, 0, dh);
            if (NSTEP > 1) ldf(1, 1, dh);
        };
        auto gather = [&](int t) {
            const _Float16* dh = dimg + (size_t)(t % 3) * IMG;
#pragma unroll
            for (int st = 0; st < NSTEP; ++st) {
                if (st + 2 < NSTEP) ldf((st + 2) % 3, st + 2, dh);
                const int j = st >> 1, ps = st & 1, cb = gw + 4 * j;
                if (ALLCB || cb < NCB) {
#pragma unroll
                    for (int nb = 0; nb < NB; ++nb) {
                        accg[j][nb] = __builtin_amdgcn_mfma_f32_32x32x16_f16(a[ps][nb], fbh[st % 3], accg[j][nb], 0, 0, 0);
                        if (!XH) accg[j][nb] = __builtin_amdgcn_mfma_f32_32x32x16_f16(a[ps][nb], fbl[st % 3], accg[j][nb], 0, 0, 0);
                    }
                }
            }
        };
#ifdef VKN_DEBUG
        if constexpr (PF != 0) tprev = __builtin_amdgcn_s_memtime();
#endif
        for (int i0 = 0; i0 < T; i0 += 2) {
#pragma unroll
            for (int u = 0; u < 2; ++u) {
                const int i = i0 + u;
                prep((i + 2) % 3, (i + 1) & 1);
                {
                    const _Float16* dh = dimg + (size_t)((i + 2) % 3) * IMG;
                    constexpr int NUNIT = 2 * NFG * 4, NCH = NSTEP * (XH ? 1 : 2);
                    int ch = 0;
#pragma unroll
                    for (int st = 0; st < NSTEP; ++st) {
                        if (st + 2 < NSTEP) ldf((st + 2) % 3, st + 2, dh);
                        const int j = st >> 1, ps = st & 1, cb = gw + 4 * j;
#pragma unroll
                        for (int pl = 0; pl < (XH ? 1 : 2); ++pl) {
                            if (ALLCB || cb < NCB) {
#pragma unroll
                                for (int nb = 0; nb < NB; ++nb)
                                    accg[j][nb] = __builtin_amdgcn_mfma_f32_32x32x16_f16(a[ps][nb], pl ? fbl[st % 3] : fbh[st % 3], accg[j][nb], 0, 0, 0);
                            }
#pragma unroll
                            for (int uu = (ch * NUNIT) / NCH; uu < ((ch + 1) * NUNIT) / NCH; ++uu) loader_unit(NFG, u ^ 1, (i + 1) % 3, min(i + 3, tlast), uu);
                            ++ch;
                            __builtin_amdgcn_sched_barrier(0);
                        }
                    }
                }
                __builtin_amdgcn_sched_barrier(0);
                FS_STAMP(4);
                __syncthreads();
                FS_STAMP(5);
            }
        }
        if (T >= 1) {
            prep((T - 1) % 3, (T - 1) & 1);
            gather(T - 1);
        }
#ifdef VKN_DEBUG
        if constexpr (PF != 0)
            if (lane == 0 && blockIdx.x == 0 && blockIdx.y == 0)
                for (int k = 0; k < 8; ++k) g_fs_prof[wave][k] = prof[k];
#endif
#pragma unroll
        for (int j = 0; j < CBW; ++j) {
            const int cb = gw + 4 * j;
            if (cb < NCB) {
#pragma unroll
                for (int nb = 0; nb < NB; ++nb)
#pragma unroll
                    for (int r = 0; r < 16; ++r) {
                        const int n = n0 + nb * 32 + vkn_cd_row(r, lane);
                        if (n < NPT) pp[(size_t)n * C + cb * 32 + li] = accg[j][nb][r];
                    }
            }
        }
    }
}

#ifdef VKN_DEBUG
#include "../../tools/experiments/fused_w4.inc"
#endif


#ifdef VKN_DEBUG
static size_t fusedw4_lds_bytes(int C) { return (size_t)4 * 2 * FS_TILE * (C + 8) * sizeof(_Float16) + 256 * 16 + 256 * 4 + 128 * 4; }
#endif
static size_t fuseds_lds_bytes(int C) { return (size_t)3 * 2 * FS_TILE * (C + 8) * sizeof(_Float16) + 256 * 16 + 256 * 4 + 128 * 4; }

#ifdef VKN_DEBUG
static size_t fused_lds_bytes(int C) { return (size_t)4 * FU_TILE * (C + 8) * sizeof(_Float16) + 256 * 16 + 256 * 4 + 128 * 4; }
static size_t fused8_lds_bytes(int C) {
    return (size_t)(2 * FU_TILE + 128) * (C + 8) * sizeof(_Float16) + 256 * 16 + 256 * 4 + 128 * 4 + 128 * 4;
}
#endif

int vkn_fused_supported(int C, int P) {
    return (C == 64 || C == 128 || C == 256) && (P % 64) == 0 && (size_t)C * P * 4 < ((size_t)1 << 31);
}

int vkn_launch_fused_decode_gather(const float* x, const _Float16* kfh, const _Float16* kfl, const float* kb, float thr,
                                   float* xraw, float* cnt, float* part, float* cntp, int B, int N, int C, int P,
                                   hipStream_t stream, int xdt, int* status, const void* touch, size_t touch_bytes) {
    if (B <= 0 || N <= 0 || P <= 0 || xdt < 0 || xdt > 2) return VKN_E_ARG;
    if (!vkn_fused_supported(C, P)) return VKN_E_SHAPE;
    const int NPT = (N + 31) / 32 * 32;
    const int G = vkn_gather_groups(B, P);
#ifdef VKN_DEBUG
    const int variant = vkn_dbg_env("VKN_FUSED", 10);
    const bool eight = variant == 1;
    const size_t lds = variant >= 2 ? fuseds_lds_bytes(C) : (eight ? fused8_lds_bytes(C) : fused_lds_bytes(C));
#else
    const size_t lds = fuseds_lds_bytes(C);
#endif
#ifdef VKN_DEBUG
    const bool one_pass = (variant >= 10 && variant <= 19) && !vkn_dbg_env("VKN_FUSED_CHUNK_LOOP", 0);
#else
    const bool one_pass = true;
#endif
    const int NZ = one_pass ? (NPT + 127) / 128 : 1;
    const int nb_one = (NPT / 32 + NZ - 1) / NZ;
    for (int n0 = 0; n0 < (one_pass ? 1 : NPT); n0 += 128) {
        const int nb = one_pass ? nb_one : ((NPT - n0 >= 128) ? 4 : (NPT - n0) / 32);
        dim3 grid(G * NZ, B, 1);
#ifdef VKN_DEBUG
#define FU_LAUNCH_XV(NBV, CV, XHV, VV)                                                                                         \
    do {                                                                                                                       \
        VKN_ALLOW_FULL_LDS((k_fused_dgs<NBV, CV, XHV, VV>));                                                                   \
        hipLaunchKernelGGL((k_fused_dgs<NBV, CV, XHV, VV>), grid, dim3(FS_THREADS), lds, stream, x, kfh, kfl, kb, thr, part,   \
                           cntp, N, NPT, n0, P);                                                                               \
    } while (0)
#define FU_LAUNCH_PQ(NBV, CV, XHV, PFV)                                                                                        \
    do {                                                                                                                       \
        VKN_ALLOW_FULL_LDS((k_fused_pq<NBV, CV, XHV, PFV>));                                                                   \
        hipLaunchKernelGGL((k_fused_pq<NBV, CV, XHV, PFV>), grid, dim3(FS_THREADS), fusedq_lds_bytes(C), stream, x, kfh, kfl,  \
                           kb, thr, part, cntp, N, NPT, n0, P);                                                                \
    } while (0)
#endif
#define FU_LAUNCH_IL(NBV, CV, XHV, PFV)                                                                                        \
    do {                                                                                                                       \
        VKN_ALLOW_FULL_LDS((k_fused_il<NBV, CV, XHV, PFV>));                                                                   \
        hipLaunchKernelGGL((k_fused_il<NBV, CV, XHV, PFV>), grid, dim3(FS_THREADS), lds, stream, x, kfh, kfl, kb, thr, part,   \
                           cntp, N, NPT, n0, P, NZ);                                                                           \
    } while (0)
#ifdef VKN_DEBUG
#define FU_LAUNCH_W4(NBV, CV, XHV, PFV)                                                                                        \
    do {                                                                                                                       \
        VKN_ALLOW_FULL_LDS((k_fused_w4<NBV, CV, XHV, PFV>));                                                                   \
        hipLaunchKernelGGL((k_fused_w4<NBV, CV, XHV, PFV>), grid, dim3(W4_THREADS), fusedw4_lds_bytes(C), stream, x, kfh, kfl,  \
                           kb, thr, part, cntp, N, NPT, n0, P, NZ);                                                            \
    } while (0)
#endif
#ifdef VKN_DEBUG
#define FU_LAUNCH_PP(NBV, CV, XHV, PFV)                                                                                        \
    do {                                                                                                                       \
        VKN_ALLOW_FULL_LDS((k_fused_pp<NBV, CV, XHV, PFV>));                                                                   \
        hipLaunchKernelGGL((k_fused_pp<NBV, CV, XHV, PFV>), grid, dim3(FS_THREADS), lds, stream, x, kfh, kfl, kb, thr, part,   \
                           cntp, N, NPT, n0, P);                                                                               \
    } while (0)
#endif
#ifdef VKN_DEBUG
#define FU_LAUNCH_X(NBV, CV, XHV)                                                          \
    do {                                                                                   \
        const int vv = vkn_dbg_env("VKN_FUSED_V", FS_V_DEFAULT);                           \
        const bool cfg2 = NBV == 4 && CV == 256 && XHV == 0;                               \
        if (variant == 4 && cfg2) FU_LAUNCH_PP(4, 256, 0, 1);                              \
        else if (variant == 6 && cfg2) FU_LAUNCH_PQ(4, 256, 0, 1);                         \
        else if (variant == 7 && cfg2) FU_LAUNCH_PQ(4, 256, 0, 2);                         \
        else if (variant == 8 && cfg2) FU_LAUNCH_PQ(4, 256, 0, 3);                         \
        else if (variant == 9 && cfg2) FU_LAUNCH_PQ(4, 256, 0, 4);                         \
        else if (variant == 3) FU_LAUNCH_PP(NBV, CV, XHV, 0);                              \
        else if (variant == 10) FU_LAUNCH_IL(NBV, CV, XHV, 0);                             \
        else if (variant == 12) FU_LAUNCH_W4(NBV, CV, XHV, 0);                             \
        else if (variant == 13 && cfg2) FU_LAUNCH_W4(4, 256, 0, 1);                        \
        else if (variant == 14 && cfg2) FU_LAUNCH_W4(4, 256, 0, 2);                        \
        else if (variant == 15 && cfg2) FU_LAUNCH_W4(4, 256, 0, 3);                        \
        else if (variant == 16 && cfg2) FU_LAUNCH_W4(4, 256, 0, 4);                        \
        else if (variant == 11 && cfg2) FU_LAUNCH_IL(4, 256, 0, 1);                        \
        else if (variant == 17 && cfg2) FU_LAUNCH_IL(4, 256, 0, 2);                        \
        else if (variant == 18 && cfg2) FU_LAUNCH_IL(4, 256, 0, 3);                        \
        else if (variant == 19 && cfg2) FU_LAUNCH_IL(4, 256, 0, 4);                        \
        else if (variant == 5) FU_LAUNCH_PQ(NBV, CV, XHV, 0);                              \
        else if (cfg2 && vv != FS_V_DEFAULT) {                                             \
            switch (vv) {                                                                  \
                case 0: FU_LAUNCH_XV(4, 256, 0, 0); break;                                 \
                case 1: FU_LAUNCH_XV(4, 256, 0, 1); break;                                 \
                case 2: FU_LAUNCH_XV(4, 256, 0, 2); break;                                 \
                case 3: FU_LAUNCH_XV(4, 256, 0, 3); break;                                 \
                case 4: FU_LAUNCH_XV(4, 256, 0, 4); break;                                 \
                case 5: FU_LAUNCH_XV(4, 256, 0, 5); break;                                 \
                case 15: FU_LAUNCH_XV(4, 256, 0, 15); break;                               \
                default: FU_LAUNCH_XV(4, 256, 0, 6); break;                                \
            }                                                                              \
        } else FU_LAUNCH_XV(NBV, CV, XHV, FS_V_DEFAULT);                                   \
    } while (0)
#else
#define FU_LAUNCH_X(NBV, CV, XHV) FU_LAUNCH_IL(NBV, CV, XHV, 0)
#endif
#define FU_LAUNCH_S(NBV, CV)                        \
    do {                                            \
        if (xdt == 1) FU_LAUNCH_X(NBV, CV, 1);      \
        else if (xdt == 2) FU_LAUNCH_X(NBV, CV, 2); \
        else FU_LAUNCH_X(NBV, CV, 0);               \
    } while (0)
#ifdef VKN_DEBUG
#define FU_LAUNCH(NBV, CV)                                                                                                     \
    do {                                                                                                                       \
        if (variant >= 2 || xdt != 0) FU_LAUNCH_S(NBV, CV);                                                                    \
        else if (eight) {                                                                                                      \
            VKN_ALLOW_FULL_LDS((k_fused_dg8<NBV, CV>));                                                                        \
            hipLaunchKernelGGL((k_fused_dg8<NBV, CV>), grid, dim3(FU8_THREADS), lds, stream, x, kfh, kfl, kb, thr, part, cntp, \
                               N, NPT, n0, P);                                                                                 \
        } else {                                                                                                               \
            VKN_ALLOW_FULL_LDS((k_fused_dg<NBV, CV>));                                                                         \
            hipLaunchKernelGGL((k_fused_dg<NBV, CV>), grid, dim3(FU_THREADS), lds, stream, x, kfh, kfl, kb, thr, part, cntp,   \
                               N, NPT, n0, P);                                                                                 \
        }                                                                                                                      \
    } while (0)
#else
#define FU_LAUNCH(NBV, CV) FU_LAUNCH_S(NBV, CV)
#endif
#define FU_CASE(NBV)                               \
    case NBV:                                      \
        if (C == 256) FU_LAUNCH(NBV, 256);         \
        else if (C == 128) FU_LAUNCH(NBV, 128);    \
        else FU_LAUNCH(NBV, 64);                   \
        break;
        switch (nb) {
            FU_CASE(1)
            FU_CASE(2)
            FU_CASE(3)
            FU_CASE(4)
            default:
                return VKN_E_SHAPE;
        }
#undef FU_CASE
#undef FU_LAUNCH
#undef FU_LAUNCH_S
#undef FU_LAUNCH_X
#undef FU_LAUNCH_IL
#ifdef VKN_DEBUG
#undef FU_LAUNCH_XV
#undef FU_LAUNCH_PP
#undef FU_LAUNCH_PQ
#undef FU_LAUNCH_W4
#endif
        VKN_CHECK_LAUNCH();
    }
    return vkn_launch_gather_reduce(part, cntp, xraw, cnt, B, N, C, G, stream, status, touch, touch_bytes);
}

#ifdef VKN_DEBUG
extern "C" int vkn_dbg_fused_prof(unsigned long long* out64) {
    return hipMemcpyFromSymbol(out64, HIP_SYMBOL(g_fs_prof), sizeof(unsigned long long) * 64) == hipSuccess ? 0 : -4;
}
#endif
```

video-k-net_amd/csrc/vkn_gather.hip:

```cpp
#include "vkn_common.h"
#include "vkn_launch.h"

#define GA_THREADS 512
#define GA_WAVES 8
#define GA_PT 32
#define GA_LDR 40

template <int NB, int BITS, int XH = 0>
__global__ __launch_bounds__(GA_THREADS, 2) void k_gather_mfma(const float* __restrict__ x,
                                                               const float* __restrict__ masks, float thr,
                                                               float* __restrict__ part, float* __restrict__ cntp, int N,
                                                               int NPT, int n0, int C, int P, int px_per_wg,
                                                               long long mask_fs, int ileave, int x_alias) {
    extern __shared__ __attribute__((aligned(16))) char smem[];
    constexpr bool REAL = (BITS == 2 || BITS == 3);
    static_assert(!(XH && REAL), "half-storage x: binary operands only");
    constexpr int XCH = XH ? 2 : 4;
    const int rows_buf = 2 * C + (REAL ? 2 : 1) * NB * 32;
    _Float16* lds = reinterpret_cast<_Float16*>(smem);

    const int b = blockIdx.y, gidx = blockIdx.x, G = gridDim.x;
    const int tid = threadIdx.x, lane = tid & 63;
    const int wave = __builtin_amdgcn_readfirstlane(tid >> 6);
    const int g = lane >> 5, li = lane & 31;

    const int p_begin = ileave ? 0 : gidx * px_per_wg;
    const int p_end = ileave ? 0 : min(P, p_begin + px_per_wg);
    const int nsup_i = ileave ? (((P >> 6) - gidx + G - 1) / G) : 0;
    const int ntiles = ileave ? 2 * nsup_i : ((p_end > p_begin) ? (p_end - p_begin + GA_PT - 1) / GA_PT : 0);
    auto tile_p0 = [&](int t) { return ileave ? ((((t >> 1) * G + gidx) << 6) + ((t & 1) << 5)) : p_begin + t * GA_PT; };

    const float* xb = x + (size_t)b * C * P;
    const unsigned short* xb16 = reinterpret_cast<const unsigned short*>(x) + (size_t)b * C * P;
    const float* mb = masks + (size_t)b * mask_fs;
    const unsigned* wb = reinterpret_cast<const unsigned*>(masks) + (size_t)b * (P >> 5) * NPT + n0;
    const bool vec_ok = ((P & 3) == 0);
    half8* lut = reinterpret_cast<half8*>(lds + (size_t)2 * rows_buf * GA_LDR);
    if (BITS == 1) {
        for (int v = tid; v < 256; v += GA_THREADS) {
            half8 h;
#pragma unroll
            for (int e = 0; e < 8; ++e) h[e] = ((v >> ((e >> 1) + 4 * (e & 1))) & 1) ? (_Float16)1.f : (_Float16)0.f;
            lut[v] = h;
        }
    }

    const int nxch = XH ? C * 4 : C * 8;
    const int nmch = NB * 32 * 8;
    f32x4 xrA[4], xrB[4];
    f32x4 mrA[2], mrB[2];

    const float off_v = (BITS == 2) ? 0.f : -INFINITY;
    const f32x4 neg_inf = {off_v, off_v, off_v, off_v};

    auto issue = [&](int t, f32x4 (&xr)[4], f32x4 (&mr)[2]) {
        const int p0 = tile_p0(t);
#pragma unroll
        for (int i = 0; i < XCH; ++i) {
            const int idc = min(tid + i * GA_THREADS, nxch - 1);
            if (XH)
                xr[i] = *reinterpret_cast<const f32x4*>(xb16 + (size_t)(idc >> 2) * P + p0 + ((idc & 3) << 3));
            else if (BITS == 2 && x_alias >= 0) {
                const int ch = idc >> 3;
                xr[i] = *reinterpret_cast<const f32x4*>(xb + (size_t)(ch >= x_alias ? ch - x_alias : ch) * P + p0 + ((idc & 7) << 2));
            } else
                xr[i] = __builtin_nontemporal_load(reinterpret_cast<const f32x4*>(xb + (size_t)(idc >> 3) * P + p0 + ((idc & 7) << 2)));
        }
        if (BITS == 1) {
            const unsigned* wp = wb + (size_t)((p0 >> 6) << 1) * NPT + min(tid, NB * 32 - 1);
            const unsigned we = wp[0], wo = wp[NPT];
            mr[0][0] = __uint_as_float(we);
            mr[0][1] = __uint_as_float(wo);
        } else {
#pragma unroll
            for (int i = 0; i < 2; ++i) {
                const int idc = min(tid + i * GA_THREADS, nmch - 1);
                const int n = min(n0 + (idc >> 3), N - 1);
                mr[i] = *reinterpret_cast<const f32x4*>(mb + (size_t)n * P + p0 + ((idc & 7) << 2));
            }
        }
    };

    auto issue_slow = [&](int t, f32x4 (&xr)[4], f32x4 (&mr)[2]) {
        const int p0 = tile_p0(t);
#pragma unroll
        for (int i = 0; i < 4; ++i) {
            const int idx = tid + i * GA_THREADS;
            f32x4 v = {0.f, 0.f, 0.f, 0.f};
            if (idx < nxch) {
                const int p = p0 + ((idx & 7) << 2);
                const int ch = idx >> 3;
                const float* src = xb + (size_t)((BITS == 2 && x_alias >= 0 && ch >= x_alias) ? ch - x_alias : ch) * P + p;
#pragma unroll
                for (int k = 0; k < 4; ++k)
                    if (p + k < p_end) v[k] = src[k];
            }
            xr[i] = v;
        }
#pragma unroll
        for (int i = 0; i < 2; ++i) {
            const int idx = tid + i * GA_THREADS;
            f32x4 v = neg_inf;
            if (idx < nmch) {
                const int n = n0 + (idx >> 3), p = p0 + ((idx & 7) << 2);
                if (n < N) {
                    const float* src = mb + (size_t)n * P + p;
#pragma unroll
                    for (int k = 0; k < 4; ++k)
                        if (p + k < p_end) v[k] = src[k];
                }
            }
            mr[i] = v;
        }
    };

    auto commit = [&](int buf, const f32x4 (&xr)[4], const f32x4 (&mr)[2]) {
        _Float16* xh = lds + (size_t)buf * rows_buf * GA_LDR;
        _Float16* xl = xh + C * GA_LDR;
        _Float16* mk = xl + C * GA_LDR;
        if (XH) {
#pragma unroll
            for (int i = 0; i < XCH; ++i) {
                const int idx = tid + i * GA_THREADS;
                if (idx < nxch) {
                    f32x4 v = xr[i];
                    if (XH == 2) {
                        half8 h;
#pragma unroll
                        for (int k = 0; k < 4; ++k) {
                            const unsigned u = __float_as_uint(xr[i][k]);
                            h[2 * k] = (_Float16)__uint_as_float(u << 16);
                            h[2 * k + 1] = (_Float16)__uint_as_float(u & 0xFFFF0000u);
                        }
                        v = __builtin_bit_cast(f32x4, h);
                    }
                    *reinterpret_cast<f32x4*>(xh + (idx >> 2) * GA_LDR + ((idx & 3) << 3)) = v;
                }
            }
        } else
#pragma unroll
        for (int i = 0; i < 4; ++i) {
            const int idx = tid + i * GA_THREADS;
            if (idx < nxch) {
                half4 h, l;
                const bool floor_ch = (BITS == 2) && x_alias >= 0 && (idx >> 3) >= x_alias;
#pragma unroll
                for (int k = 0; k < 4; ++k) {
                    _Float16 hh, ll;
                    float xv = xr[i][k];
                    if (BITS == 2) xv = floor_ch ? fmaxf(xv, thr) : xv;
                    vkn_split_f16(xv, hh, ll);
                    h[k] = hh;
                    l[k] = ll;
                }
                const int off = (idx >> 3) * GA_LDR + ((idx & 7) << 2);
                *reinterpret_cast<half4*>(xh + off) = h;
                *reinterpret_cast<half4*>(xl + off) = l;
            }
        }
        if (BITS == 1) {
            const float w0 = mr[0][0], w1 = mr[0][1];
            if (tid < NB * 32) {
                reinterpret_cast<unsigned*>(mk)[tid] = __float_as_uint(w0);
                reinterpret_cast<unsigned*>(mk)[NB * 32 + tid] = __float_as_uint(w1);
            }
        } else
#pragma unroll
        for (int i = 0; i < 2; ++i) {
            const int idx = tid + i * GA_THREADS;
            if (idx < nmch) {
                const bool row_ok = (n0 + (idx >> 3)) < N;
                half4 m, ml;
#pragma unroll
                for (int k = 0; k < 4; ++k) {
                    if (REAL) {
                        _Float16 hh, ll;
                        float av = row_ok ? mr[i][k] : 0.f;
                        if (BITS == 3)
                            av = (row_ok && mr[i][k] >= thr) ? 1.0f / (1.0f + expf(-mr[i][k])) : 0.f;
                        vkn_split_f16(av, hh, ll);
                        m[k] = hh;
                        ml[k] = ll;
                    } else {
                        m[k] = (row_ok && mr[i][k] >= thr) ? (_Float16)1.f : (_Float16)0.f;
                    }
                }
                *reinterpret_cast<half4*>(mk + (idx >> 3) * GA_LDR + ((idx & 7) << 2)) = m;
                if (REAL) *reinterpret_cast<half4*>(mk + (NB * 32 + (idx >> 3)) * GA_LDR + ((idx & 7) << 2)) = ml;
            }
        }
    };

    f32x16 acc[NB];
    f32x16 accc;
#pragma unroll
    for (int nb = 0; nb < NB; ++nb)
#pragma unroll
        for (int r = 0; r < 16; ++r) acc[nb][r] = 0.f;
#pragma unroll
    for (int r = 0; r < 16; ++r) accc[r] = 0.f;
    half8 ones;
#pragma unroll
    for (int e = 0; e < 8; ++e) ones[e] = (_Float16)1.f;

    const bool has_cb = (wave * 32 < C);
    const bool has_cnt = (wave < NB);

    auto compute = [&](int buf, int odd32) {
        const _Float16* xh = lds + (size_t)buf * rows_buf * GA_LDR;
        const _Float16* xl = xh + C * GA_LDR;
        const _Float16* mk = xl + C * GA_LDR;
#pragma unroll
        for (int ks = 0; ks < 2; ++ks) {
            const int off = (ks << 4) + (g << 3);
            const int bsh = 16 * odd32 + 8 * ks + 4 * g;
            if (has_cb) {
                const half8 bh = *reinterpret_cast<const half8*>(xh + (wave * 32 + li) * GA_LDR + off);
                const half8 bl = *reinterpret_cast<const half8*>(xl + (wave * 32 + li) * GA_LDR + off);
#pragma unroll
                for (int nb = 0; nb < NB; ++nb) {
                    half8 a;
                    if (BITS == 1) {
                        const unsigned we = reinterpret_cast<const unsigned*>(mk)[nb * 32 + li];
                        const unsigned wo = reinterpret_cast<const unsigned*>(mk)[NB * 32 + nb * 32 + li];
                        a = lut[((we >> bsh) & 0xFu) | (((wo >> bsh) & 0xFu) << 4)];
                    } else {
                        a = *reinterpret_cast<const half8*>(mk + (nb * 32 + li) * GA_LDR + off);
                    }
                    acc[nb] = __builtin_amdgcn_mfma_f32_32x32x16_f16(a, bh, acc[nb], 0, 0, 0);
                    if (!XH) acc[nb] = __builtin_amdgcn_mfma_f32_32x32x16_f16(a, bl, acc[nb], 0, 0, 0);
                    if (REAL) {
                        const half8 al = *reinterpret_cast<const half8*>(mk + (NB * 32 + nb * 32 + li) * GA_LDR + off);
                        acc[nb] = __builtin_amdgcn_mfma_f32_32x32x16_f16(al, bh, acc[nb], 0, 0, 0);
                    }
                }
            }
            if (has_cnt) {
                half8 a;
                if (BITS == 1) {
                    const unsigned we = reinterpret_cast<const unsigned*>(mk)[wave * 32 + li];
                    const unsigned wo = reinterpret_cast<const unsigned*>(mk)[NB * 32 + wave * 32 + li];
                    a = lut[((we >> bsh) & 0xFu) | (((wo >> bsh) & 0xFu) << 4)];
                } else {
                    a = *reinterpret_cast<const half8*>(mk + (wave * 32 + li) * GA_LDR + off);
                }
                accc = __builtin_amdgcn_mfma_f32_32x32x16_f16(a, ones, accc, 0, 0, 0);
                if (REAL) {
                    const half8 al = *reinterpret_cast<const half8*>(mk + (NB * 32 + wave * 32 + li) * GA_LDR + off);
                    accc = __builtin_amdgcn_mfma_f32_32x32x16_f16(al, ones, accc, 0, 0, 0);
                }
            }
        }
    };

    const int nfull = ileave ? ntiles : (vec_ok ? (p_end - p_begin) / GA_PT : 0);
    if (nfull > 0) {
        issue(0, xrA, mrA);
        issue(min(1, nfull - 1), xrB, mrB);
        commit(0, xrA, mrA);
        __syncthreads();
        for (int t = 0; t < nfull; t += 2) {
            issue(min(t + 2, nfull - 1), xrA, mrA);
            compute(0, (tile_p0(t) >> 5) & 1);
            if (t + 1 < nfull) commit(1, xrB, mrB);
            __syncthreads();
            if (t + 1 >= nfull) break;
            issue(min(t + 3, nfull - 1), xrB, mrB);
            compute(1, (tile_p0(t + 1) >> 5) & 1);
            if (t + 2 < nfull) commit(0, xrA, mrA);
            __syncthreads();
        }
    }
    for (int t = nfull; t < ntiles; ++t) {
        issue_slow(t, xrA, mrA);
        commit(0, xrA, mrA);
        __syncthreads();
        compute(0, 0);
        __syncthreads();
    }

    float* pp = part + ((size_t)b * G + gidx) * NPT * C;
    if (has_cb) {
#pragma unroll
        for (int nb = 0; nb < NB; ++nb)
#pragma unroll
            for (int r = 0; r < 16; ++r) {
                const int n = n0 + nb * 32 + vkn_cd_row(r, lane);
                pp[(size_t)n * C + wave * 32 + li] = acc[nb][r];
            }
    }
    if (has_cnt && li == 0) {
        float* cp = cntp + ((size_t)b * G + gidx) * NPT;
#pragma unroll
        for (int r = 0; r < 16; ++r) cp[n0 + wave * 32 + vkn_cd_row(r, lane)] = accc[r];
    }
}

template <int NB>
__global__ __launch_bounds__(GA_THREADS, 2) void k_gather_bits_w(const float* __restrict__ x, const unsigned* __restrict__ bits,
                                                                  float* __restrict__ part, float* __restrict__ cntp, int N,
                                                                  int NPT, int n0, int C, int P, int px_per_wg, int ileave) {
    extern __shared__ __attribute__((aligned(16))) char smem[];
    constexpr int WTILE = 2 * 32 * GA_LDR;
    const int b = blockIdx.y, gidx = blockIdx.x, G = gridDim.x;
    const int tid = threadIdx.x, lane = tid & 63;
    const int wave = __builtin_amdgcn_readfirstlane(tid >> 6);
    const int g = lane >> 5, li = lane & 31;
    _Float16* wl = reinterpret_cast<_Float16*>(smem) + (size_t)wave * 2 * WTILE;
    half8* lut = reinterpret_cast<half8*>(reinterpret_cast<_Float16*>(smem) + (size_t)GA_WAVES * 2 * WTILE);
    for (int v = tid; v < 256; v += GA_THREADS) {
        half8 h;
#pragma unroll
        for (int e = 0; e < 8; ++e) h[e] = ((v >> ((e >> 1) + 4 * (e & 1))) & 1) ? (_Float16)1.f : (_Float16)0.f;
        lut[v] = h;
    }
    __syncthreads();

    const int p_begin = gidx * px_per_wg;
    const int p_end = min(P, p_begin + px_per_wg);
    const int nsup = ileave ? (((P >> 6) - gidx + G - 1) / G)
                            : ((p_end > p_begin) ? (p_end - p_begin) >> 6 : 0);
    auto sup_p0 = [&](int s) { return ileave ? ((s * G + gidx) << 6) : p_begin + (s << 6); };
    const bool has_cb = (wave * 32 < C);
    const bool has_cnt = (wave < NB);

    f32x16 acc[NB];
#pragma unroll
    for (int nb = 0; nb < NB; ++nb)
#pragma unroll
        for (int r = 0; r < 16; ++r) acc[nb][r] = 0.f;
    unsigned cnt_i = 0;

    if (has_cb && nsup > 0) {
        const float* xw = x + ((size_t)b * C + wave * 32) * P;
        const unsigned* wb = bits + (size_t)b * (P >> 5) * NPT + n0 + li;
        const int lrow = lane >> 3, lchk = lane & 7;
        f32x4 xa[8], xb[8];
        unsigned wa[2 * NB], wv[2 * NB];

        auto issue = [&](int s, f32x4 (&xr)[8], unsigned (&wr)[2 * NB]) {
            const int p0 = sup_p0(s);
#pragma unroll
            for (int h = 0; h < 2; ++h)
#pragma unroll
                for (int i = 0; i < 4; ++i)
                    xr[h * 4 + i] = __builtin_nontemporal_load(
                        reinterpret_cast<const f32x4*>(xw + (size_t)(lrow + 8 * i) * P + p0 + 32 * h + (lchk << 2)));
            const unsigned* wp = wb + (size_t)((p0 >> 6) << 1) * NPT;
#pragma unroll
            for (int nb = 0; nb < NB; ++nb) {
                wr[nb] = wp[nb * 32];
                wr[NB + nb] = wp[NPT + nb * 32];
            }
        };
        auto commit = [&](const f32x4 (&xr)[8]) {
#pragma unroll
            for (int h = 0; h < 2; ++h) {
                _Float16* xh = wl + h * WTILE;
                _Float16* xl = xh + 32 * GA_LDR;
#pragma unroll
                for (int i = 0; i < 4; ++i) {
                    half4 hh, ll;
#pragma unroll
                    for (int k = 0; k < 4; ++k) {
                        _Float16 a, c2;
                        vkn_split_f16(xr[h * 4 + i][k], a, c2);
                        hh[k] = a;
                        ll[k] = c2;
                    }
                    const int off = (lrow + 8 * i) * GA_LDR + (lchk << 2);
                    *reinterpret_cast<half4*>(xh + off) = hh;
                    *reinterpret_cast<half4*>(xl + off) = ll;
                }
            }
        };
        auto compute = [&](const unsigned (&wr)[2 * NB]) {
#pragma unroll
            for (int h = 0; h < 2; ++h) {
                const _Float16* xh = wl + h * WTILE;
                const _Float16* xl = xh + 32 * GA_LDR;
#pragma unroll
                for (int ks = 0; ks < 2; ++ks) {
                    const int off = (ks << 4) + (g << 3);
                    const int bsh = 16 * h + 8 * ks + 4 * g;
                    const half8 bh = *reinterpret_cast<const half8*>(xh + li * GA_LDR + off);
                    const half8 bl = *reinterpret_cast<const half8*>(xl + li * GA_LDR + off);
#pragma unroll
                    for (int nb = 0; nb < NB; ++nb) {
                        const half8 a = lut[((wr[nb] >> bsh) & 0xFu) | (((wr[NB + nb] >> bsh) & 0xFu) << 4)];
                        acc[nb] = __builtin_amdgcn_mfma_f32_32x32x16_f16(a, bh, acc[nb], 0, 0, 0);
                        acc[nb] = __builtin_amdgcn_mfma_f32_32x32x16_f16(a, bl, acc[nb], 0, 0, 0);
                    }
                }
            }
        };
        auto lds_fence = [&]() {
            __builtin_amdgcn_s_waitcnt(0xc07f);
            __builtin_amdgcn_wave_barrier();
        };

        const int last = nsup - 1;
        issue(0, xa, wa);
        for (int s = 0; s < nsup; s += 2) {
            issue(min(s + 1, last), xb, wv);
            commit(xa);
            lds_fence();
            compute(wa);
            lds_fence();
            if (s + 1 >= nsup) break;
            issue(min(s + 2, last), xa, wa);
            commit(xb);
            lds_fence();
            compute(wv);
            lds_fence();
        }
    }

    if (has_cnt) {
        const unsigned* wc = bits + (size_t)b * (P >> 5) * NPT + n0 + wave * 32 + li;
        for (int s2 = 0; s2 < nsup; ++s2) {
            const unsigned* wp = wc + (size_t)((sup_p0(s2) >> 6) << 1) * NPT;
            cnt_i += __popc(wp[0]) + __popc(wp[NPT]);
        }
    }

    float* pp = part + ((size_t)b * G + gidx) * NPT * C;
    if (has_cb) {
#pragma unroll
        for (int nb = 0; nb < NB; ++nb)
#pragma unroll
            for (int r = 0; r < 16; ++r) {
                const int n = n0 + nb * 32 + vkn_cd_row(r, lane);
                pp[(size_t)n * C + wave * 32 + li] = acc[nb][r];
            }
    }
    if (has_cnt && g == 0) cntp[((size_t)b * G + gidx) * NPT + n0 + wave * 32 + li] = (float)cnt_i;
}

__global__ __launch_bounds__(256) void k_gather_reduce(const float* __restrict__ part, const float* __restrict__ cntp,
                                                        float* __restrict__ xraw, float* __restrict__ cnt, int N, int NPT,
                                                        int C, int G, int* __restrict__ status, const char* __restrict__ touch,
                                                        unsigned touch_bytes) {
    if (touch) {
        const unsigned per = (touch_bytes / gridDim.x + 15u) & ~15u;
        const unsigned t0 = blockIdx.x * per, t1 = min(t0 + per, touch_bytes & ~15u);
        for (unsigned o = t0 + threadIdx.x * 16u; o < t1; o += 256u * 16u) {
            const f32x4 v = *reinterpret_cast<const f32x4*>(touch + o);
            asm volatile("" ::"v"(v));
        }
    }
    __shared__ f32x4 comb[3][64];
    const int row = blockIdx.x;
    const int b = row / N, n = row - b * N;
    const int lane = threadIdx.x & 63;
    const int k = __builtin_amdgcn_readfirstlane(threadIdx.x >> 6);
    const size_t gstride = (size_t)NPT * C;
    const float* pp = part + ((size_t)b * G * NPT + n) * C;
    const int G4 = G & ~3;
    for (int c0 = 0; c0 < C; c0 += 256) {
        const int c4 = c0 + lane * 4;
        const bool ok = c4 < C;
        const float* pc = pp + (ok ? c4 : 0);
        f32x4 s = {0.f, 0.f, 0.f, 0.f};
        int gi = k;
        for (; gi + 28 < G4; gi += 32) {
            f32x4 v[8];
#pragma unroll
            for (int u = 0; u < 8; ++u) v[u] = *reinterpret_cast<const f32x4*>(pc + (size_t)(gi + 4 * u) * gstride);
#pragma unroll
            for (int u = 0; u < 8; ++u) s += v[u];
        }
        for (; gi < G4; gi += 4) s += *reinterpret_cast<const f32x4*>(pc + (size_t)gi * gstride);
        if (k == 0)
            for (gi = G4; gi < G; ++gi) s += *reinterpret_cast<const f32x4*>(pc + (size_t)gi * gstride);
        if (c0) __syncthreads();
        if (k) comb[k - 1][lane] = s;
        __syncthreads();
        if (k == 0 && ok) {
            const f32x4 r = (s + comb[0][lane]) + (comb[1][lane] + comb[2][lane]);
            *reinterpret_cast<f32x4*>(xraw + (size_t)row * C + c4) = r;
            if (status && !(fabsf(r[0]) <= 3.0e38f && fabsf(r[1]) <= 3.0e38f && fabsf(r[2]) <= 3.0e38f && fabsf(r[3]) <= 3.0e38f))
                atomicOr(status, 1);
        }
    }
    if (k == 1) {
        const float* cp = cntp + (size_t)b * G * NPT + n;
        float s = 0.f;
        for (int gi = lane; gi < G; gi += 64) s += cp[(size_t)gi * NPT];
        s = vkn_wave_sum(s);
        if (lane == 0) cnt[row] = s;
    }
}

__global__ __launch_bounds__(256) void k_gather_ref(const float* __restrict__ x, const float* __restrict__ masks,
                                                    float thr, float* __restrict__ xraw, float* __restrict__ cnt, int N,
                                                    int C, int P, long long mask_fs) {
    const int n = blockIdx.x, b = blockIdx.y;
    const float* mp = masks + (size_t)b * mask_fs + (size_t)n * P;
    for (int c = threadIdx.x; c < C; c += 256) {
        const float* xp = x + ((size_t)b * C + c) * P;
        float s = 0.f;
        for (int p = 0; p < P; ++p)
            if (mp[p] >= thr) s += xp[p];
        xraw[((size_t)b * N + n) * C + c] = s;
    }
    if (threadIdx.x == 0) {
        float s = 0.f;
        for (int p = 0; p < P; ++p)
            if (mp[p] >= thr) s += 1.f;
        cnt[(size_t)b * N + n] = s;
    }
}

int vkn_launch_gather_reduce(const float* part, const float* cntp, float* xraw, float* cnt, int B, int N, int C, int G,
                             hipStream_t stream, int* status, const void* touch, size_t touch_bytes) {
    if (touch_bytes >= (1ull << 31)) touch = nullptr;
    hipLaunchKernelGGL(k_gather_reduce, dim3(B * N), dim3(256), 0, stream, part, cntp, xraw, cnt, N, (N + 31) / 32 * 32, C, G, status,
                       static_cast<const char*>(touch), (unsigned)touch_bytes);
    VKN_CHECK_LAUNCH();
    return VKN_OK;
}

int vkn_gather_groups(int B, int P) {
    int wg_per_frame = 256 / (B > 0 ? B : 1);
    if (wg_per_frame < 1) wg_per_frame = 1;
    int px_per_wg = (P + wg_per_frame - 1) / wg_per_frame;
    px_per_wg = (px_per_wg + GA_PT - 1) / GA_PT * GA_PT;
    return (P + px_per_wg - 1) / px_per_wg;
}

int vkn_launch_gather(const float* x, const float* masks, float thr, float* xraw, float* cnt, float* part, float* cntp,
                      int B, int N, int C, int P, hipStream_t stream, int xdt, int* status, const void* touch, size_t touch_bytes) {
    return vkn_launch_gather_ex(x, masks, thr, xraw, cnt, part, cntp, B, N, C, P, N, stream, xdt, status, touch, touch_bytes);
}

static int gather_launch(const float* x, const float* masks, float thr, float* xraw, float* cnt, float* part, float* cntp, int B,
                         int N, int C, int P, int mask_rows, int bits, hipStream_t stream, int xdt = 0, int* status = nullptr,
                         const void* touch = nullptr, size_t touch_bytes = 0, int x_alias = -1);

int vkn_launch_gather_ex(const float* x, const float* masks, float thr, float* xraw, float* cnt, float* part, float* cntp,
                         int B, int N, int C, int P, int mask_rows, hipStream_t stream, int xdt, int* status, const void* touch,
                         size_t touch_bytes) {
    return gather_launch(x, masks, thr, xraw, cnt, part, cntp, B, N, C, P, mask_rows, 0, stream, xdt, status, touch, touch_bytes);
}

int vkn_launch_gather_real(const float* x, const float* a, float* xraw, float* cnt, float* part, float* cntp, int B, int N, int C,
                           int P, int mask_rows, hipStream_t stream, int x_alias, float x_floor) {
    if (x_alias > C || (x_alias > 0 && (C - x_alias > x_alias || B != 1))) return VKN_E_ARG;
    return gather_launch(x, a, x_alias >= 0 ? x_floor : 0.f, xraw, cnt, part, cntp, B, N, C, P, mask_rows, 2, stream, 0, nullptr, nullptr, 0,
                         x_alias);
}

int vkn_launch_gather_soft(const float* x, const float* masks, float thr, float* xraw, float* cnt, float* part, float* cntp, int B,
                           int N, int C, int P, int mask_rows, hipStream_t stream) {
    return gather_launch(x, masks, thr, xraw, cnt, part, cntp, B, N, C, P, mask_rows, 3, stream);
}

int vkn_launch_gather_bits(const float* x, const unsigned* bits, float* xraw, float* cnt, float* part, float* cntp, int B, int N,
                           int C, int P, hipStream_t stream, int xdt, int* status, const void* touch, size_t touch_bytes) {
    if ((P % 64) != 0) return VKN_E_SHAPE;
    return gather_launch(x, reinterpret_cast<const float*>(bits), 0.f, xraw, cnt, part, cntp, B, N, C, P, N, 1, stream, xdt, status, touch,
                         touch_bytes);
}

static int gather_launch(const float* x, const float* masks, float thr, float* xraw, float* cnt, float* part, float* cntp, int B,
                         int N, int C, int P, int mask_rows, int bits, hipStream_t stream, int xdt, int* status, const void* touch,
                         size_t touch_bytes, int x_alias) {
    if (x_alias >= 0 && bits != 2) return VKN_E_ARG;
    if (B <= 0 || N <= 0 || P <= 0 || mask_rows < N) return VKN_E_ARG;
    if (xdt < 0 || xdt > 2) return VKN_E_ARG;
    if (xdt && (bits >= 2 || (P % 64) != 0)) return VKN_E_SHAPE;
    const long long mask_fs = (long long)mask_rows * P;
    if (C % 32 != 0 || C > 256) return VKN_E_SHAPE;
    const int NPT = (N + 31) / 32 * 32;
    int wg_per_frame = 256 / B;
    if (wg_per_frame < 1) wg_per_frame = 1;
    int px_per_wg = (P + wg_per_frame - 1) / wg_per_frame;
    px_per_wg = (px_per_wg + GA_PT - 1) / GA_PT * GA_PT;
    const int G = (P + px_per_wg - 1) / px_per_wg;
    const int ileave = ((P % 64) == 0 && vkn_dbg_env("VKN_GATHER_ILEAVE", 1) != 0) ? 1 : 0;
    const bool wave_indep = bits == 1 && xdt == 0 && vkn_dbg_env("VKN_GATHER_BITS_W", 1) != 0 && (C % 32) == 0 &&
                            (px_per_wg % 64) == 0;
    for (int n0 = 0; n0 < NPT; n0 += 128) {
        const int nb = (NPT - n0 >= 128) ? 4 : (NPT - n0) / 32;
        dim3 grid(G, B, 1), block(GA_THREADS);
        if (wave_indep) {
            const size_t ldsw = (size_t)GA_WAVES * 2 * 2 * 32 * GA_LDR * sizeof(_Float16) + 4096;
            const unsigned* bw = reinterpret_cast<const unsigned*>(masks);
#define GA_WLAUNCH(NBV)                                                                                              \
    case NBV:                                                                                                        \
        VKN_ALLOW_FULL_LDS(k_gather_bits_w<NBV>);                                                                    \
        hipLaunchKernelGGL(k_gather_bits_w<NBV>, grid, block, ldsw, stream, x, bw, part, cntp, N, NPT, n0, C, P, px_per_wg, ileave); \
        break;
            switch (nb) {
                GA_WLAUNCH(1)
                GA_WLAUNCH(2)
                GA_WLAUNCH(3)
                GA_WLAUNCH(4)
                default:
                    return VKN_E_SHAPE;
            }
#undef GA_WLAUNCH
            VKN_CHECK_LAUNCH();
            continue;
        }
        const size_t lds = (size_t)2 * (2 * C + (bits >= 2 ? 2 : 1) * nb * 32) * GA_LDR * sizeof(_Float16) + (bits == 1 ? 4096 : 0);
#define GA_LAUNCH(NBV, BV, XHV)                                                                                  \
    do {                                                                                                         \
        VKN_ALLOW_FULL_LDS((k_gather_mfma<NBV, BV, XHV>));                                                       \
        hipLaunchKernelGGL((k_gather_mfma<NBV, BV, XHV>), grid, block, lds, stream, x, masks, thr, part, cntp, N, NPT, n0, C, P, \
                           px_per_wg, mask_fs, ileave, x_alias);                                                 \
    } while (0)
#define GA_CASE(NBV)                                 \
    case NBV:                                        \
        if (bits == 3) GA_LAUNCH(NBV, 3, 0);         \
        else if (bits == 2) GA_LAUNCH(NBV, 2, 0);    \
        else if (bits && xdt == 1) GA_LAUNCH(NBV, 1, 1); \
        else if (bits && xdt == 2) GA_LAUNCH(NBV, 1, 2); \
        else if (bits) GA_LAUNCH(NBV, 1, 0);         \
        else if (xdt == 1) GA_LAUNCH(NBV, 0, 1);     \
        else if (xdt == 2) GA_LAUNCH(NBV, 0, 2);     \
        else GA_LAUNCH(NBV, 0, 0);                   \
        break;
        switch (nb) {
            GA_CASE(1)
            GA_CASE(2)
            GA_CASE(3)
            GA_CASE(4)
            default:
                return VKN_E_SHAPE;
        }
#undef GA_CASE
#undef GA_LAUNCH
        VKN_CHECK_LAUNCH();
    }
    hipLaunchKernelGGL(k_gather_reduce, dim3(B * N), dim3(256), 0, stream, part, cntp, xraw, cnt, N, NPT, C, G, status,
                       static_cast<const char*>(touch), (unsigned)(touch_bytes < (1ull << 31) ? touch_bytes : 0));
    VKN_CHECK_LAUNCH();
    return VKN_OK;
}

int vkn_launch_gather_ref(const float* x, const float* masks, float thr, float* xraw, float* cnt, int B, int N, int C,
                          int P, hipStream_t stream) {
    return vkn_launch_gather_ref_ex(x, masks, thr, xraw, cnt, B, N, C, P, N, stream);
}

int vkn_launch_gather_ref_ex(const float* x, const float* masks, float thr, float* xraw, float* cnt, int B, int N, int C,
                             int P, int mask_rows, hipStream_t stream) {
    if (mask_rows < N) return VKN_E_ARG;
    hipLaunchKernelGGL(k_gather_ref, dim3(N, B), dim3(256), 0, stream, x, masks, thr, xraw, cnt, N, C, P,
                       (long long)mask_rows * P);
    VKN_CHECK_LAUNCH();
    return VKN_OK;
}
```

video-k-net_amd/csrc/vkn_launch.h:

```cpp
#pragma once
#include <hip/hip_runtime.h>
#include <stddef.h>

struct VknEpi {
    const float* bias;
    const float* rowscale;
    const float* bias2;
    const float* resid;
    int ldr;
    const float* ln_w;
    const float* ln_b;
    int ln_from_col;
    float eps;
    int act;
    float* out;
    int ldo;
    const float* dot_vec;
    const float* dot_bias;
    float* dot_out;
    _Float16* plane_hi;
    _Float16* plane_lo;
    int rows_per_frame;
    int NPT;
};

struct VknGemmProb {
    const float* A;
    const float* A2;
    const float* A3;
    const float* A4;
    int lda;
    const float* W;
    const void* Wsplit;
    int Nout;
    VknEpi epi;
};

int vkn_gather_groups(int B, int P);
int vkn_launch_gather_ex(const float* x, const float* masks, float thr, float* xraw, float* cnt, float* part, float* cntp,
                         int B, int N, int C, int P, int mask_rows, hipStream_t stream, int xdt = 0, int* status = nullptr,
                         const void* touch = nullptr, size_t touch_bytes = 0);
int vkn_launch_gather_ref_ex(const float* x, const float* masks, float thr, float* xraw, float* cnt, int B, int N, int C,
                             int P, int mask_rows, hipStream_t stream);
int vkn_launch_gather_real(const float* x, const float* a, float* xraw, float* cnt, float* part, float* cntp, int B, int N, int C,
                           int P, int mask_rows, hipStream_t stream, int x_alias = -1, float x_floor = 0.f);
int vkn_launch_gather_soft(const float* x, const float* masks, float thr, float* xraw, float* cnt, float* part, float* cntp, int B,
                           int N, int C, int P, int mask_rows, hipStream_t stream);
int vkn_launch_gather_bits(const float* x, const unsigned* bits, float* xraw, float* cnt, float* part, float* cntp, int B, int N,
                           int C, int P, hipStream_t stream, int xdt = 0, int* status = nullptr, const void* touch = nullptr,
                           size_t touch_bytes = 0);
int vkn_launch_gather_reduce(const float* part, const float* cntp, float* xraw, float* cnt, int B, int N, int C, int G,
                             hipStream_t stream, int* status = nullptr, const void* touch = nullptr, size_t touch_bytes = 0);
int vkn_fused_supported(int C, int P);
int vkn_launch_fused_decode_gather(const float* x, const _Float16* kfh, const _Float16* kfl, const float* kb, float thr,
                                   float* xraw, float* cnt, float* part, float* cntp, int B, int N, int C, int P,
                                   hipStream_t stream, int xdt = 0, int* status = nullptr, const void* touch = nullptr,
                                   size_t touch_bytes = 0);
int vkn_launch_gather(const float* x, const float* masks, float thr, float* xraw, float* cnt, float* part, float* cntp,
                      int B, int N, int C, int P, hipStream_t stream, int xdt = 0, int* status = nullptr, const void* touch = nullptr,
                      size_t touch_bytes = 0);
int vkn_launch_gather_ref(const float* x, const float* masks, float thr, float* xraw, float* cnt, int B, int N, int C,
                          int P, hipStream_t stream);
struct VknDecodeStrides {
    long long plane;
    long long kb;
    long long out;
};
int vkn_launch_decode_ex(const float* x, const _Float16* kfh, const _Float16* kfl, const float* kb, float* out, int B, int N,
                         int C, int P, int shared, int out_rows, hipStream_t stream, int xdt = 0, const float* oscale = nullptr);
#define VKN_DECODE_CUS 256
struct VknDecodeSplit {
    int px_per_wg, G2;
};
VknDecodeSplit vkn_decode_split(int B, int P, int max_workgroups);
int vkn_launch_decode_wg(const float* x, const _Float16* kfh, const _Float16* kfl, const float* kb, float* out, int B, int N,
                         int C, int P, int max_workgroups, hipStream_t stream, int xdt = 0);
int vkn_launch_decode_ref_ex(const float* x, const float* kern, const float* kb, float* out, int B, int N, int C, int P,
                             int shared, int out_rows, hipStream_t stream);
int vkn_launch_decode_bits(const float* x, const _Float16* kfh, const _Float16* kfl, const float* kb, unsigned* bits_out,
                           float thr, int B, int N, int C, int P, hipStream_t stream, int xdt = 0);
int vkn_launch_decode(const float* x, const _Float16* kfh, const _Float16* kfl, const float* kb, float* out, int B, int N,
                      int C, int P, hipStream_t stream, int xdt = 0);
int vkn_launch_decode_ref(const float* x, const float* kern, const float* kb, float* out, int B, int N, int C, int P,
                          hipStream_t stream);
int vkn_launch_split_planes(const float* kern, _Float16* kfh, _Float16* kfl, int B, int N, int C, hipStream_t stream);
int vkn_launch_gemm(const float* A, const float* A2, int lda, const float* W, const void* Wsplit, int M, int K, int Nout,
                    int ksplit, float* partial, const VknEpi& epi, hipStream_t stream);
int vkn_launch_gemm_group(const VknGemmProb* probs, int nprob, int M, int K, int ksplit, float* partial, hipStream_t stream);
size_t vkn_split_w3_bytes(int Nout, int K);
int vkn_launch_add2(const float* a, const float* b, float* out, size_t n, hipStream_t st);
int vkn_launch_add2_half(const void* a, const void* b, void* out, size_t n, int xdt, hipStream_t st);
int vkn_launch_add_rows(const float* a, const float* pos, float* out, size_t rows, int C, int period, hipStream_t st);
struct InitPassArgs {
    const float *loc, *sem;
    const _Float16 *kh, *kl;
    const float* seg_b;
    float *x_out, *masks, *seg;
    unsigned* bits;
    float thr;
    int Np, ncls, nth, cat, N, C, P, px_per_wg;
    int npt;
};
int vkn_init_pass_supported(int Np, int ncls, int C, int P);
int vkn_launch_init_pass(const InitPassArgs& a, int B, hipStream_t st);
int vkn_launch_init_finish(const float* init_w, const float* obj, const float* seg_w, float* out, int B, int Np, int N, int nth,
                           int C, hipStream_t st);
int vkn_launch_ffn_fused(const float* X, int ldx, const void* W1s, const float* b1, const void* W2s, int M, int C, int FF, int HS,
                         float* partial, const VknEpi& epi2, hipStream_t stream);
int vkn_launch_transpose(const float* src, float* dst, int R, int Cc, hipStream_t st);
int vkn_launch_split_w3(const float* W, void* Wp, int Nout, int K, hipStream_t stream);
int vkn_launch_split_w3_t(const float* W, void* Wp, int Nout, int K, hipStream_t stream);
int vkn_launch_ku_mix(const float* params, const float* inputf, const float* ig, const float* ug, const float* no_w,
                      const float* no_b, const float* ino_w, const float* ino_b, float eps, float* f, int M, int C,
                      hipStream_t stream);
int vkn_launch_attn(const float* Q, int ldq, const float* K, const float* V, int ldkv, float* out, int ldo, int B, int Nq,
                    int Nk, int heads, int hd, hipStream_t stream);
int vkn_launch_upsample(const float* in, float* out, int planes, int H, int W, int S, hipStream_t stream, int out_f16 = 0);

struct VknPanopticCfg;
size_t vkn_panoptic_ws_bytes(int B, int K, int Ho, int Wo);
int vkn_launch_panoptic_joint(const VknPanopticCfg* c, const float* cls, const float* masks, int B, int N, int ncls,
                              int* panoptic_seg, int* info, int* nseg, int* bbox, void* ws, size_t ws_bytes, hipStream_t st);

struct VknChainConsts {
    const float *bcnt, *dyn_b;
    const float *norm_out_w, *norm_out_b, *inp_b, *inorm_out_w, *inorm_out_b;
    const float *ig_b, *inorm_in_w, *inorm_in_b, *ug_b, *norm_in_w, *norm_in_b;
    const float *fc_b, *fc_norm_w, *fc_norm_b, *in_b;
    const float *out_b, *attn_norm_w, *attn_norm_b, *ffn1_b, *ffn2_b, *ffn_norm_w, *ffn_norm_b;
    const float *cls_ln_w, *cls_ln_b, *mask_ln_w, *mask_ln_b, *dvec, *fc_cls_b, *dec_b;
    int ff, ncls;
    const float* h2_inv[14];
};
enum { VKN_H2_DYNFT = 0, VKN_H2_DYN, VKN_H2_INP, VKN_H2_IG, VKN_H2_UG, VKN_H2_FC, VKN_H2_IN, VKN_H2_OUT, VKN_H2_FFN1, VKN_H2_FFN2,
       VKN_H2_CLSFC, VKN_H2_MASKFC, VKN_H2_FCCLS, VKN_H2_DEC, VKN_H2_COUNT };
size_t vkn_chain_consts_floats();
int vkn_chain_pack_consts(const VknChainConsts& c, float* out, hipStream_t stream);
struct VknChainA {
    const float* a0;
    const float* obj_in;
    const float* rowscale;
    const void* wbase;
    size_t wbytes;
    unsigned off_dyn, off_inp, off_ig, off_ug, off_fc, off_in;
    const float* consts;
    float eps;
    int M;
    float* obj1;
    float* qkv;
    int* status;
};
struct VknChainC {
    const float* ao;
    const float* obj1;
    const void* wbase;
    size_t wbytes;
    unsigned off_out, off_ffn1, off_ffn2, off_clsfc, off_maskfc, off_fccls, off_dec;
    const float* consts;
    const float* kb0;
    int ff, ncls, cls_sigmoid;
    float eps;
    int M;
    float* obj_out;
    float* cls_out;
    float* kb_out;
    _Float16 *plane_hi, *plane_lo;
    float* kern_out;
    int rows_per_frame, NPT;
    int* status;
};
int vkn_launch_gemm_t3(const VknGemmProb* probs, int nprob, int M, int K, hipStream_t stream);
int vkn_launch_chain_a(const VknChainA& p, hipStream_t stream);
int vkn_launch_chain_c(const VknChainC& p, hipStream_t stream);
int vkn_launch_chain_a_h2(const VknChainA& p, hipStream_t stream);
int vkn_launch_chain_c_h2(const VknChainC& p, hipStream_t stream);
size_t vkn_split_h2_bytes(int Nout, int K);
int vkn_launch_split_h2(const float* W, void* images, int Nout, int K, const float* scale, hipStream_t stream);

struct VknKsPro {
    const float* a[4];
    int lda[4];
    int nsum;
    long long sum_stride;
    const float* pbias;
    const float* presid;
    int ldr;
    const float* ln_w[4];
    const float* ln_b[4];
    float eps;
    int act;
    float* side_out;
    int ld_side;
    const float* dot_vec;
    const float* dot_bias;
    float* dot_out;
};
struct VknKsEpi {
    const float* bias;
    const float* rowscale;
    const float* bias2;
    const float* resid;
    int ldr;
    int act;
    float* out;
    int ldo;
    _Float16* plane_hi;
    _Float16* plane_lo;
    int rows_per_frame, NPT;
};
struct VknKsProb {
    VknKsPro pro;
    const void* Wsplit;
    int Nout;
    int KT;
    VknKsEpi epi;
};
int vkn_launch_rowepi(const float* partial, int ks, int M, int Nout, const VknEpi& epi, hipStream_t stream);
int vkn_launch_gemm_ks(const VknKsProb* probs, int nprob, int mode, int zchunks, int kpw, long long out_zstride, int M, hipStream_t stream);
```

video-k-net_amd/ops.py:

```python
import contextlib
import ctypes
import struct
import threading

import torch

from . import _lib
from ._lib import VknDims, VknStageWeights, check

_H = _lib.CONSTS
FLAG_REF_KERNELS = _H['VKN_FLAG_REF_KERNELS']
FLAG_EXACT_GEMM = _H['VKN_FLAG_EXACT_GEMM']
FLAG_LOGITS_HANDOFF = _H['VKN_FLAG_LOGITS_HANDOFF']
FLAG_BITS_HANDOFF = _H['VKN_FLAG_BITS_HANDOFF']
FLAG_CHAIN_LAUNCHES = _H['VKN_FLAG_CHAIN_LAUNCHES']
FLAG_CHAIN_PERSISTENT = _H['VKN_FLAG_CHAIN_PERSISTENT']
FLAG_JOIN_EARLY = _H['VKN_FLAG_JOIN_EARLY']
FLAG_LINK_RESERVE = _H['VKN_FLAG_LINK_RESERVE']
FLAG_LINK_NO_RESERVE = _H['VKN_FLAG_LINK_NO_RESERVE']
FLAG_SCALED_F16 = _H['VKN_FLAG_SCALED_F16']
FLAG_CHAIN_BF16X3 = _H['VKN_FLAG_CHAIN_BF16X3']
FLAG_INIT_SEPARATE = _H['VKN_FLAG_INIT_SEPARATE']
FLAG_CHAIN_KSPLIT = _H['VKN_FLAG_CHAIN_KSPLIT']
FLAG_SERIAL_LINK = _H['VKN_FLAG_SERIAL_LINK']

_tls = threading.local()


def _ptr(t):
    return ctypes.c_void_p(t.data_ptr()) if t is not None else ctypes.c_void_p(0)


def _stream():
    return ctypes.c_void_p(torch.cuda.current_stream().cuda_stream)


def _req(t, name):
    if not torch.is_tensor(t) or not t.is_cuda:
        raise _lib.VknLibraryError(f'{name}: expected a CUDA/HIP tensor — the MI355X path has no CPU fallback')
    if t.dtype != torch.float32:
        raise TypeError(f'{name}: expected float32, got {t.dtype}')
    t = t.contiguous()
    if t.data_ptr() % 16:
        t = t.clone(memory_format=torch.contiguous_format)
    return t


_X_DTYPES = {torch.float32: _H['VKN_X_F32'], torch.float16: _H['VKN_X_F16'], torch.bfloat16: _H['VKN_X_BF16']}
FLAG_X_F16, FLAG_X_BF16 = _H['VKN_FLAG_X_F16'], _H['VKN_FLAG_X_BF16']


def _req_x(t, name='x'):
    if not torch.is_tensor(t) or not t.is_cuda:
        raise _lib.VknLibraryError(f'{name}: expected a CUDA/HIP tensor — the MI355X path has no CPU fallback')
    if t.dtype not in _X_DTYPES:
        raise TypeError(f'{name}: expected float32, float16 or bfloat16, got {t.dtype}')
    t = t.contiguous()
    if t.data_ptr() % 16:
        t = t.clone(memory_format=torch.contiguous_format)
    return t, _X_DTYPES[t.dtype]


def _workspace(nbytes, device, scratch=False):
    cache = getattr(_tls, 'ws', None)
    if cache is None:
        cache = _tls.ws = {}
    key = (device, torch.cuda.current_stream(device).cuda_stream)
    buf = cache.get(key)
    need = int(nbytes) + 256
    if buf is None or buf.numel() < need:
        old = buf
        buf = torch.empty(max(need, 512), dtype=torch.uint8, device=device)
        if old is None:
            buf[:256].zero_()
        else:
            buf[:256].copy_(old[:256])
        cache[key] = buf
        gen = getattr(_tls, 'ws_gen', None)
        if gen is None:
            gen = _tls.ws_gen = {}
        gen[key] = gen.get(key, 0) + 1
    return buf[256:] if scratch else buf


def workspace_cache():
    if getattr(_tls, 'ws', None) is None:
        _tls.ws = {}
    if getattr(_tls, 'ws_gen', None) is None:
        _tls.ws_gen = {}
    return _tls.ws, _tls.ws_gen


@contextlib.contextmanager
def adopt_workspace(cache):
    old = getattr(_tls, 'ws', None), getattr(_tls, 'ws_gen', None)
    _tls.ws, _tls.ws_gen = cache
    try:
        yield
    finally:
        _tls.ws, _tls.ws_gen = old


def workspace_generation(device):
    gen = getattr(_tls, 'ws_gen', None) or {}
    return gen.get((device, torch.cuda.current_stream(device).cuda_stream), 0)


def workspace_status(device=None):
    device = torch.device(device if device is not None else torch.cuda.current_device())
    if device.index is None:
        device = torch.device('cuda', torch.cuda.current_device())
    cache = getattr(_tls, 'ws', None) or {}
    buf = cache.get((device, torch.cuda.current_stream(device).cuda_stream))
    if buf is None:
        return
    with torch.cuda.device(device):
        check(_lib.lib().vkn_workspace_status(_ptr(buf), buf.numel(), _stream()))


_THR_CACHE = {}


def thr_logit(hard_mask_thr=0.5):
    key = float(hard_mask_thr)
    if key in _THR_CACHE:
        return _THR_CACHE[key]
    if not 0.0 < key < 1.0:
        raise ValueError('hard_mask_thr must be in (0, 1)')

    def f2o(f):
        u = struct.unpack('<I', struct.pack('<f', f))[0]
        return u ^ 0xFFFFFFFF if u & 0x80000000 else u | 0x80000000

    def o2f(o):
        u = o & 0x7FFFFFFF if o & 0x80000000 else o ^ 0xFFFFFFFF
        return struct.unpack('<f', struct.pack('<I', u & 0xFFFFFFFF))[0]

    def on(o):
        t = torch.full((16,), o2f(o), dtype=torch.float32)
        return bool((t.sigmoid() > key)[0])

    lo, hi = f2o(-200.0), f2o(200.0)
    assert not on(lo) and on(hi)
    while hi - lo > 1:
        mid = (lo + hi) // 2
        if on(mid):
            hi = mid
        else:
            lo = mid
    _THR_CACHE[key] = o2f(hi)
    return _THR_CACHE[key]


def mask_gather(x, mask_logits, hard_mask_thr=0.5, flags=0):
    (x, xdt), m = _req_x(x), _req(mask_logits, 'mask_logits')
    flags |= (0, FLAG_X_F16, FLAG_X_BF16)[xdt]
    B, C = x.shape[0], x.shape[1]
    N = m.shape[1]
    P = x[0, 0].numel()
    if m.shape[0] != B or m[0, 0].numel() != P:
        raise ValueError('x and mask_logits disagree on batch or spatial size')
    L = _lib.lib()
    xraw = torch.empty((B, N, C), dtype=torch.float32, device=x.device)
    cnt = torch.empty((B, N), dtype=torch.float32, device=x.device)
    nb = L.vkn_gather_workspace_bytes(B, N, C, P)
    ws = _workspace(nb, x.device, scratch=True)
    with torch.cuda.device(x.device):
        check(L.vkn_mask_gather_f32(_ptr(x), _ptr(m), thr_logit(hard_mask_thr), _ptr(xraw), _ptr(cnt), B, N, C, P, _ptr(ws),
                                    ws.numel(), flags, _stream()))
    return xraw, cnt


def mask_gather_real(x, a):
    x, a = _req(x, 'x'), _req(a, 'a')
    B, C = x.shape[0], x.shape[1]
    N = a.shape[1]
    P = x[0, 0].numel()
    if a.shape[0] != B or a[0, 0].numel() != P:
        raise ValueError('x and a disagree on batch or spatial size')
    L = _lib.lib()
    out = torch.empty((B, N, C), dtype=torch.float32, device=x.device)
    asum = torch.empty((B, N), dtype=torch.float32, device=x.device)
    ws = _workspace(L.vkn_gather_workspace_bytes(B, N, C, P), x.device, scratch=True)
    with torch.cuda.device(x.device):
        check(L.vkn_mask_gather_real_f32(_ptr(x), _ptr(a), _ptr(out), _ptr(asum), B, N, C, P, _ptr(ws), ws.numel(), _stream()))
    return out, asum


def mask_decode(x, kernels, bias=None, flags=0, out_scale=None):
    (x, xdt), k = _req_x(x), _req(kernels.reshape(kernels.shape[0], kernels.shape[1], -1), 'kernels')
    flags |= (0, FLAG_X_F16, FLAG_X_BF16)[xdt]
    B, C, H, W = x.shape
    N = k.shape[1]
    if k.shape[0] != B or k.shape[2] != C:
        raise ValueError('kernels must be [B, N, C] (conv_kernel_size == 1)')
    bias = _req(bias, 'bias') if bias is not None else None
    L = _lib.lib()
    out = torch.empty((B, N, H, W), dtype=torch.float32, device=x.device)
    nb = L.vkn_decode_workspace_bytes(B, N, C)
    ws = _workspace(nb, x.device, scratch=True)
    with torch.cuda.device(x.device):
        if out_scale is not None:
            sc = _req(out_scale.reshape(1), 'out_scale')
            check(L.vkn_mask_decode_scaled_f32(_ptr(x), _ptr(k), _ptr(bias), _ptr(sc), _ptr(out), B, N, C, H * W, _ptr(ws), ws.numel(),
                                               flags, _stream()))
        else:
            check(L.vkn_mask_decode_f32(_ptr(x), _ptr(k), _ptr(bias), _ptr(out), B, N, C, H * W, _ptr(ws), ws.numel(), flags,
                                        _stream()))
    return out


def upsample_bilinear(masks, scale, out_f16=False):
    m = _req(masks, 'masks')
    B, N, H, W = m.shape
    out = torch.empty((B, N, H * scale, W * scale), dtype=torch.float16 if out_f16 else torch.float32, device=m.device)
    with torch.cuda.device(m.device):
        if out_f16:
            check(_lib.lib().vkn_upsample_bilinear_f16out(_ptr(m), _ptr(out), B * N, H, W, int(scale), _stream()))
        else:
            check(_lib.lib().vkn_upsample_bilinear_f32(_ptr(m), _ptr(out), B * N, H, W, int(scale), _stream()))
    return out


def upsample_bilinear_bwd(grad_out, scale):
    g = _req(grad_out, 'grad_out')
    B, N, OH, OW = g.shape
    H, W = OH // scale, OW // scale
    out = torch.empty((B, N, H, W), dtype=torch.float32, device=g.device)
    with torch.cuda.device(g.device):
        check(_lib.lib().vkn_upsample_bilinear_bwd_f32(_ptr(g), _ptr(out), B * N, H, W, int(scale), _stream()))
    return out


class StagePack:

    def __init__(self, named: dict, device):
        self.keep = []
        self.w = VknStageWeights()
        self.sig = None

        def P(key):
            t = named.get(key)
            if t is None:
                return 0
            t = t.detach()
            if t.device != device or t.dtype != torch.float32 or not t.is_contiguous():
                t = t.to(device=device, dtype=torch.float32).contiguous()
            self.keep.append(t)
            return t.data_ptr()

        w = self.w
        if 'feat_transform.conv.weight' in named:
            ft = named['feat_transform.conv.weight'].detach().to(device=device, dtype=torch.float32)
            ft2 = ft.reshape(ft.shape[0], ft.shape[1]).contiguous()
            ftT = ft2.t().contiguous()
            self.keep += [ft2, ftT]
            w.ft_w, w.ft_wT = ft2.data_ptr(), ftT.data_ptr()
            w.ft_b = P('feat_transform.conv.bias')
        ku = 'kernel_update_conv.'
        w.dyn_w, w.dyn_b = P(ku + 'dynamic_layer.weight'), P(ku + 'dynamic_layer.bias')
        w.inp_w, w.inp_b = P(ku + 'input_layer.weight'), P(ku + 'input_layer.bias')
        w.ig_w, w.ig_b = P(ku + 'input_gate.weight'), P(ku + 'input_gate.bias')
        w.ug_w, w.ug_b = P(ku + 'update_gate.weight'), P(ku + 'update_gate.bias')
        w.norm_in_w, w.norm_in_b = P(ku + 'norm_in.weight'), P(ku + 'norm_in.bias')
        w.norm_out_w, w.norm_out_b = P(ku + 'norm_out.weight'), P(ku + 'norm_out.bias')
        w.inorm_in_w, w.inorm_in_b = P(ku + 'input_norm_in.weight'), P(ku + 'input_norm_in.bias')
        w.inorm_out_w, w.inorm_out_b = P(ku + 'input_norm_out.weight'), P(ku + 'input_norm_out.bias')
        w.fc_w, w.fc_b = P(ku + 'fc_layer.weight'), P(ku + 'fc_layer.bias')
        w.fc_norm_w, w.fc_norm_b = P(ku + 'fc_norm.weight'), P(ku + 'fc_norm.bias')
        w.attn_in_w, w.attn_in_b = P('attention.attn.in_proj_weight'), P('attention.attn.in_proj_bias')
        w.attn_out_w, w.attn_out_b = P('attention.attn.out_proj.weight'), P('attention.attn.out_proj.bias')
        w.attn_norm_w, w.attn_norm_b = P('attention_norm.weight'), P('attention_norm.bias')
        w.ffn1_w, w.ffn1_b = P('ffn.layers.0.0.weight'), P('ffn.layers.0.0.bias')
        w.ffn2_w, w.ffn2_b = P('ffn.layers.1.weight'), P('ffn.layers.1.bias')
        w.ffn_norm_w, w.ffn_norm_b = P('ffn_norm.weight'), P('ffn_norm.bias')
        i = 0
        while f'cls_fcs.{3 * i}.weight' in named:
            w.cls_fc_w[i] = P(f'cls_fcs.{3 * i}.weight')
            w.cls_ln_w[i], w.cls_ln_b[i] = P(f'cls_fcs.{3 * i + 1}.weight'), P(f'cls_fcs.{3 * i + 1}.bias')
            i += 1
        self.n_cls_fcs = i
        i = 0
        while f'mask_fcs.{3 * i}.weight' in named:
            w.mask_fc_w[i] = P(f'mask_fcs.{3 * i}.weight')
            w.mask_ln_w[i], w.mask_ln_b[i] = P(f'mask_fcs.{3 * i + 1}.weight'), P(f'mask_fcs.{3 * i + 1}.bias')
            i += 1
        self.n_mask_fcs = i
        w.fc_cls_w, w.fc_cls_b = P('fc_cls.weight'), P('fc_cls.bias')
        w.fc_mask_w, w.fc_mask_b = P('fc_mask.weight'), P('fc_mask.bias')
        pa = 'attention_previous.attn.'
        w.pa_in_w, w.pa_in_b = P(pa + 'in_proj_weight'), P(pa + 'in_proj_bias')
        w.pa_out_w, w.pa_out_b = P(pa + 'out_proj.weight'), P(pa + 'out_proj.bias')
        w.pa_norm_w, w.pa_norm_b = P('attention_previous_norm.weight'), P('attention_previous_norm.bias')
        w.lffn1_w, w.lffn1_b = P('link_ffn.layers.0.0.weight'), P('link_ffn.layers.0.0.bias')
        w.lffn2_w, w.lffn2_b = P('link_ffn.layers.1.weight'), P('link_ffn.layers.1.bias')
        w.lffn_norm_w, w.lffn_norm_b = P('link_ffn_norm.weight'), P('link_ffn_norm.bias')
        self.has_link = bool(w.pa_in_w and w.lffn1_w)
        self.device = device
        self._prep = None
        self._prep_key = None
        self._ready = None

    def ensure_prepared(self, dims):
        key = (dims.C, dims.ff, dims.ncls, dims.n_cls_fcs, dims.n_mask_fcs)
        if self._prep is not None and self._prep_key == key:
            if self._ready is not None and not self._ready.query():
                torch.cuda.current_stream(self.device).wait_event(self._ready)
            return
        L = _lib.lib()
        self.w.prepared, self.w.prepared_bytes = None, 0
        nb = L.vkn_prepared_bytes(ctypes.byref(dims), ctypes.byref(self.w))
        if nb == 0:
            return
        buf = torch.empty(nb, dtype=torch.uint8, device=self.device)
        with torch.cuda.device(self.device):
            check(L.vkn_prepare_stage_f32(ctypes.byref(dims), ctypes.byref(self.w), _ptr(buf), nb, _stream()))
            self._ready = torch.cuda.Event()
            self._ready.record(torch.cuda.current_stream(self.device))
        self._prep, self._prep_key = buf, key
        self.w.prepared, self.w.prepared_bytes = buf.data_ptr(), nb

    @staticmethod
    def signature(named: dict, device):
        return (str(device),) + tuple((k, t.data_ptr(), t._version) for k, t in sorted(named.items()))


# ... 1159 lines not shown
```

Measured before the change: 10310 frames/s.

## Fold the gather partial reduction into the gather pass via last-block tickets

Adds a per-frame atomic ticket counter so that the last workgroup to finish the gather or fused decode-gather pass sums the per-group partials itself. This replaces the separate k_gather_reduce launch, removing one kernel launch and its launch gap per stage. Partial stores become agent-scope atomic stores, and a fence and barrier handshake is added before the tail. The cost is that a single workgroup per frame does the whole reduction, which lowers parallelism for that step. The path is only taken when the new REDUCE_IN_PASS flag is set and the ticket count fits.

```diff
diff --git a/include/vkn.h b/include/vkn.h
--- a/include/vkn.h
+++ b/include/vkn.h
@@ -36,6 +36,8 @@
 #define VKN_FLAG_SCALED_F16 16384u
 #define VKN_FLAG_CHAIN_BF16X3 65536u
 #define VKN_FLAG_CHAIN_KSPLIT 8192u
+#define VKN_FLAG_REDUCE_LAUNCH 1048576u
+#define VKN_FLAG_REDUCE_IN_PASS 2097152u
 #define VKN_FLAG_SERIAL_LINK 32u
 #define VKN_FLAG_CLIP_LINK 8u
 
diff --git a/video-k-net_amd/csrc/vkn_api.hip b/video-k-net_amd/csrc/vkn_api.hip
--- a/video-k-net_amd/csrc/vkn_api.hip
+++ b/video-k-net_amd/csrc/vkn_api.hip
@@ -25,6 +25,7 @@
         *maskfeat, *kb, *kern32, *lq, *lkv, *lobj, *lupd, *lf;
     _Float16 *kfh, *kfl;
     int* status;
+    unsigned* ticket;
 };
 
 
@@ -180,6 +181,7 @@
     const size_t B = d->B, N = d->N, C = d->C, P = (size_t)d->H * d->W, M = B * N, FF = d->ff;
     const size_t G = vkn_gather_groups(d->B, (int)P), NPT = npt_of(d->N);
     s->status = c.take<int>(64);
+    s->ticket = s->status ? reinterpret_cast<unsigned*>(s->status) + 1 : nullptr;
     s->part = c.take<float>(B * G * NPT * C);
     s->cntp = c.take<float>(B * G * NPT);
     s->xraw = c.take<float>(M * C);
@@ -385,12 +387,18 @@
     return run_link(d, lw, pw, cur, prev, out, s, st, link_track ? (track_src == 2 ? cur : xfeat) : nullptr, flags);
 }
 
+inline unsigned* gather_ticket(const VknDims* d, const StageWs& s, unsigned flags) {
+    if (!(flags & VKN_FLAG_REDUCE_IN_PASS) || (flags & (VKN_FLAG_REDUCE_LAUNCH | VKN_FLAG_REF_KERNELS))) return nullptr;
+    return vkn_gather_tickets(d->B, d->N) ? s.ticket : nullptr;
+}
+
 int run_gather(const VknDims* d, const float* x, const float* masks, const unsigned* bits, const StageWs& s, unsigned flags,
                hipStream_t st, const void* touch = nullptr, size_t touch_bytes = 0) {
     const int B = d->B, N = d->N, C = d->C, P = d->H * d->W, xdt = xdt_of(flags);
     if (flags & VKN_FLAG_REF_KERNELS) return vkn_launch_gather_ref(x, masks, d->thr_logit, s.xraw, s.cnt, B, N, C, P, st);
-    if (bits) return vkn_launch_gather_bits(x, bits, s.xraw, s.cnt, s.part, s.cntp, B, N, C, P, st, xdt, s.status, touch, touch_bytes);
-    return vkn_launch_gather(x, masks, d->thr_logit, s.xraw, s.cnt, s.part, s.cntp, B, N, C, P, st, xdt, s.status, touch, touch_bytes);
+    unsigned* const ticket = gather_ticket(d, s, flags);
+    if (bits) return vkn_launch_gather_bits(x, bits, s.xraw, s.cnt, s.part, s.cntp, B, N, C, P, st, xdt, s.status, touch, touch_bytes, ticket);
+    return vkn_launch_gather(x, masks, d->thr_logit, s.xraw, s.cnt, s.part, s.cntp, B, N, C, P, st, xdt, s.status, touch, touch_bytes, ticket);
 }
 
 int final_decode(const VknDims* d, const float* x, const StageWs& s, const float* kb, float* masks_out, unsigned flags,
@@ -645,7 +653,7 @@
     if (ref_decode) return vkn_launch_decode_ref(c.x, kern32, kb, c.masks_out, B, N, C, P, st);
     if (c.to == TO_GATHER)
         return vkn_launch_fused_decode_gather(c.x, s.kfh, s.kfl, kb, d->thr_logit, s.xraw, s.cnt, s.part, s.cntp, B, N, C, P, st, xdt, s.status,
-                                              touch, touch_bytes);
+                                              touch, touch_bytes, gather_ticket(d, s, flags));
     if (c.to == TO_BITS) return vkn_launch_decode_bits(c.x, s.kfh, s.kfl, kb, c.bits_out, d->thr_logit, B, N, C, P, st, xdt);
     return final_decode(d, c.x, s, kb, c.masks_out, flags, st, c.prof0, c.prof1, c.up_out, c.up_stride, c.up_chunk, c.up_done,
                         link_reserve_wg(d, c.link_reserve, persistent_chain, flags));
diff --git a/video-k-net_amd/csrc/vkn_fused.hip b/video-k-net_amd/csrc/vkn_fused.hip
--- a/video-k-net_amd/csrc/vkn_fused.hip
+++ b/video-k-net_amd/csrc/vkn_fused.hip
@@ -1,4 +1,5 @@
 #include "vkn_common.h"
+#include "vkn_gather_tail.h"
 #include "vkn_launch.h"
 
 #define FU_THREADS 256
@@ -40,7 +41,7 @@
 __global__ __launch_bounds__(FS_THREADS, 2) void k_fused_il(const float* __restrict__ x, const _Float16* __restrict__ kfh,
                                                              const _Float16* __restrict__ kfl, const float* __restrict__ kb,
                                                              float thr, float* __restrict__ part, float* __restrict__ cntp,
-                                                             int N, int NPT, int n0_in, int P, int NZ) {
+                                                             int N, int NPT, int n0_in, int P, int NZ, VknGrTail tl) {
     constexpr int KS = C / 16;
     constexpr int NFG = KS / 16, NFD = KS / 4 - NFG, NF = NFD;
     static_assert(KS % 4 == 0 && 4 * (NFD + NFG) == KS, "C must be a multiple of 64");
@@ -304,7 +305,8 @@
             if (lane == 0 && blockIdx.x == 0 && blockIdx.y == 0)
                 for (int k = 0; k < 8; ++k) g_fs_prof[wave][k] = prof[k];
 #endif
-        if (has_dec && lane < 32 && n0 + wave * 32 + lane < NPT) cntp[((size_t)b * G + gidx) * NPT + n0 + wave * 32 + lane] = (float)cnt_i;
+        vkn_gr_touch(tl.touch, tl.touch_bytes, blockIdx.y * gridDim.x + blockIdx.x, gridDim.x * gridDim.y, tid, 256u);
+        if (has_dec && lane < 32 && n0 + wave * 32 + lane < NPT) vkn_gr_store(cntp + ((size_t)b * G + gidx) * NPT + n0 + wave * 32 + lane, (float)cnt_i, tl.ticket != nullptr);
     } else {
         if constexpr (PF == 3) __builtin_amdgcn_s_setprio(2);
         const int gw = wave - 4;
@@ -418,6 +420,7 @@
             if (lane == 0 && blockIdx.x == 0 && blockIdx.y == 0)
                 for (int k = 0; k < 8; ++k) g_fs_prof[wave][k] = prof[k];
 #endif
+        const bool through = tl.ticket != nullptr;
 #pragma unroll
         for (int j = 0; j < CBW; ++j) {
             const int cb = gw + 4 * j;
@@ -427,10 +430,15 @@
 #pragma unroll
                     for (int r = 0; r < 16; ++r) {
                         const int n = n0 + nb * 32 + vkn_cd_row(r, lane);
-                        if (n < NPT) pp[(size_t)n * C + cb * 32 + li] = accg[j][nb][r];
+                        if (n < NPT) vkn_gr_store(pp + (size_t)n * C + cb * 32 + li, accg[j][nb][r], through);
                     }
             }
         }
+    }
+    if (tl.ticket) {
+        const int t = b * NZ + (int)(blockIdx.x - gidx * NZ);
+        if (vkn_gr_arrive(tl.ticket, t, G, reinterpret_cast<int*>(smem)))
+            vkn_gr_tail(part, cntp, tl.xraw, tl.cnt, tl.ticket, t, b, G, N, NPT, C, min(n0, N), min(n0 + NB * 32, N), tl.status);
     }
 }
 
@@ -457,7 +465,7 @@
 
 int vkn_launch_fused_decode_gather(const float* x, const _Float16* kfh, const _Float16* kfl, const float* kb, float thr,
                                    float* xraw, float* cnt, float* part, float* cntp, int B, int N, int C, int P,
-                                   hipStream_t stream, int xdt, int* status, const void* touch, size_t touch_bytes) {
+                                   hipStream_t stream, int xdt, int* status, const void* touch, size_t touch_bytes, unsigned* ticket) {
     if (B <= 0 || N <= 0 || P <= 0 || xdt < 0 || xdt > 2) return VKN_E_ARG;
     if (!vkn_fused_supported(C, P)) return VKN_E_SHAPE;
     const int NPT = (N + 31) / 32 * 32;
@@ -476,6 +484,15 @@
 #endif
     const int NZ = one_pass ? (NPT + 127) / 128 : 1;
     const int nb_one = (NPT / 32 + NZ - 1) / NZ;
+#ifdef VKN_DEBUG
+    const bool has_tail = variant == 10;
+#else
+    const bool has_tail = true;
+#endif
+    const bool in_pass = ticket && one_pass && has_tail && (long long)B * NZ <= VKN_GR_TICKETS;
+    if (touch_bytes >= (1ull << 31)) touch = nullptr;
+    VknGrTail tl{};
+    if (in_pass) tl = VknGrTail{xraw, cnt, ticket, status, static_cast<const char*>(touch), (unsigned)touch_bytes};
     for (int n0 = 0; n0 < (one_pass ? 1 : NPT); n0 += 128) {
         const int nb = one_pass ? nb_one : ((NPT - n0 >= 128) ? 4 : (NPT - n0) / 32);
         dim3 grid(G * NZ, B, 1);
@@ -497,7 +514,7 @@
     do {                                                                                                                       \
         VKN_ALLOW_FULL_LDS((k_fused_il<NBV, CV, XHV, PFV>));                                                                   \
         hipLaunchKernelGGL((k_fused_il<NBV, CV, XHV, PFV>), grid, dim3(FS_THREADS), lds, stream, x, kfh, kfl, kb, thr, part,   \
-                           cntp, N, NPT, n0, P, NZ);                                                                           \
+                           cntp, N, NPT, n0, P, NZ, tl);                                                                       \
     } while (0)
 #ifdef VKN_DEBUG
 #define FU_LAUNCH_W4(NBV, CV, XHV, PFV)                                                                                        \
@@ -603,6 +620,7 @@
 #endif
         VKN_CHECK_LAUNCH();
     }
+    if (in_pass) return VKN_OK;
     return vkn_launch_gather_reduce(part, cntp, xraw, cnt, B, N, C, G, stream, status, touch, touch_bytes);
 }
 
diff --git a/video-k-net_amd/csrc/vkn_gather.hip b/video-k-net_amd/csrc/vkn_gather.hip
--- a/video-k-net_amd/csrc/vkn_gather.hip
+++ b/video-k-net_amd/csrc/vkn_gather.hip
@@ -1,4 +1,5 @@
 #include "vkn_common.h"
+#include "vkn_gather_tail.h"
 #include "vkn_launch.h"
 
 #define GA_THREADS 512
@@ -11,7 +12,7 @@
                                                                const float* __restrict__ masks, float thr,
                                                                float* __restrict__ part, float* __restrict__ cntp, int N,
                                                                int NPT, int n0, int C, int P, int px_per_wg,
-                                                               long long mask_fs, int ileave, int x_alias) {
+                                                               long long mask_fs, int ileave, int x_alias, VknGrTail tl) {
     extern __shared__ __attribute__((aligned(16))) char smem[];
     constexpr bool REAL = (BITS == 2 || BITS == 3);
     static_assert(!(XH && REAL), "half-storage x: binary operands only");
@@ -279,27 +280,33 @@
         __syncthreads();
     }
 
+    vkn_gr_touch(tl.touch, tl.touch_bytes, blockIdx.y * gridDim.x + blockIdx.x, gridDim.x * gridDim.y, tid, GA_THREADS);
     float* pp = part + ((size_t)b * G + gidx) * NPT * C;
+    const bool through = tl.ticket != nullptr;
     if (has_cb) {
 #pragma unroll
         for (int nb = 0; nb < NB; ++nb)
 #pragma unroll
             for (int r = 0; r < 16; ++r) {
                 const int n = n0 + nb * 32 + vkn_cd_row(r, lane);
-                pp[(size_t)n * C + wave * 32 + li] = acc[nb][r];
+                vkn_gr_store(pp + (size_t)n * C + wave * 32 + li, acc[nb][r], through);
             }
     }
     if (has_cnt && li == 0) {
         float* cp = cntp + ((size_t)b * G + gidx) * NPT;
 #pragma unroll
-        for (int r = 0; r < 16; ++r) cp[n0 + wave * 32 + vkn_cd_row(r, lane)] = accc[r];
+        for (int r = 0; r < 16; ++r) vkn_gr_store(cp + n0 + wave * 32 + vkn_cd_row(r, lane), accc[r], through);
+    }
+    if constexpr (!REAL) {
+        if (tl.ticket && vkn_gr_arrive(tl.ticket, b, G, reinterpret_cast<int*>(smem)))
+            vkn_gr_tail(part, cntp, tl.xraw, tl.cnt, tl.ticket, b, b, G, N, NPT, C, n0, min(n0 + NB * 32, N), tl.status);
     }
 }
 
 template <int NB>
 __global__ __launch_bounds__(GA_THREADS, 2) void k_gather_bits_w(const float* __restrict__ x, const unsigned* __restrict__ bits,
                                                                   float* __restrict__ part, float* __restrict__ cntp, int N,
-                                                                  int NPT, int n0, int C, int P, int px_per_wg, int ileave) {
+                                                                  int NPT, int n0, int C, int P, int px_per_wg, int ileave, VknGrTail tl) {
     extern __shared__ __attribute__((aligned(16))) char smem[];
     constexpr int WTILE = 2 * 32 * GA_LDR;
     const int b = blockIdx.y, gidx = blockIdx.x, G = gridDim.x;
@@ -424,31 +431,28 @@
         }
     }
 
+    vkn_gr_touch(tl.touch, tl.touch_bytes, blockIdx.y * gridDim.x + blockIdx.x, gridDim.x * gridDim.y, tid, GA_THREADS);
     float* pp = part + ((size_t)b * G + gidx) * NPT * C;
+    const bool through = tl.ticket != nullptr;
     if (has_cb) {
 #pragma unroll
         for (int nb = 0; nb < NB; ++nb)
 #pragma unroll
             for (int r = 0; r < 16; ++r) {
                 const int n = n0 + nb * 32 + vkn_cd_row(r, lane);
-                pp[(size_t)n * C + wave * 32 + li] = acc[nb][r];
-            }
-    }
-    if (has_cnt && g == 0) cntp[((size_t)b * G + gidx) * NPT + n0 + wave * 32 + li] = (float)cnt_i;
+                vkn_gr_store(pp + (size_t)n * C + wave * 32 + li, acc[nb][r], through);
+            }
+    }
+    if (has_cnt && g == 0) vkn_gr_store(cntp + ((size_t)b * G + gidx) * NPT + n0 + wave * 32 + li, (float)cnt_i, through);
+    if (tl.ticket && vkn_gr_arrive(tl.ticket, b, G, reinterpret_cast<int*>(smem)))
+        vkn_gr_tail(part, cntp, tl.xraw, tl.cnt, tl.ticket, b, b, G, N, NPT, C, n0, min(n0 + NB * 32, N), tl.status);
 }
 
 __global__ __launch_bounds__(256) void k_gather_reduce(const float* __restrict__ part, const float* __restrict__ cntp,
                                                         float* __restrict__ xraw, float* __restrict__ cnt, int N, int NPT,
                                                         int C, int G, int* __restrict__ status, const char* __restrict__ touch,
                                                         unsigned touch_bytes) {
-    if (touch) {
-        const unsigned per = (touch_bytes / gridDim.x + 15u) & ~15u;
-        const unsigned t0 = blockIdx.x * per, t1 = min(t0 + per, touch_bytes & ~15u);
-        for (unsigned o = t0 + threadIdx.x * 16u; o < t1; o += 256u * 16u) {
-            const f32x4 v = *reinterpret_cast<const f32x4*>(touch + o);
-            asm volatile("" ::"v"(v));
-        }
-    }
+    vkn_gr_touch(touch, touch_bytes, blockIdx.x, gridDim.x, threadIdx.x, 256u);
     __shared__ f32x4 comb[3][64];
     const int row = blockIdx.x;
     const int b = row / N, n = row - b * N;
@@ -456,38 +460,24 @@
     const int k = __builtin_amdgcn_readfirstlane(threadIdx.x >> 6);
     const size_t gstride = (size_t)NPT * C;
     const float* pp = part + ((size_t)b * G * NPT + n) * C;
-    const int G4 = G & ~3;
     for (int c0 = 0; c0 < C; c0 += 256) {
         const int c4 = c0 + lane * 4;
         const bool ok = c4 < C;
-        const float* pc = pp + (ok ? c4 : 0);
-        f32x4 s = {0.f, 0.f, 0.f, 0.f};
-        int gi = k;
-        for (; gi + 28 < G4; gi += 32) {
-            f32x4 v[8];
-#pragma unroll
-            for (int u = 0; u < 8; ++u) v[u] = *reinterpret_cast<const f32x4*>(pc + (size_t)(gi + 4 * u) * gstride);
-#pragma unroll
-            for (int u = 0; u < 8; ++u) s += v[u];
-        }
-        for (; gi < G4; gi += 4) s += *reinterpret_cast<const f32x4*>(pc + (size_t)gi * gstride);
-        if (k == 0)
-            for (gi = G4; gi < G; ++gi) s += *reinterpret_cast<const f32x4*>(pc + (size_t)gi * gstride);
+        const float* pc[1] = {pp + (ok ? c4 : 0)};
+        f32x4 sk[1][1];
+        vkn_gr_walk<1, 1, 8>(pc, gstride, G, k, sk);
+        const f32x4 s = sk[0][0];
         if (c0) __syncthreads();
         if (k) comb[k - 1][lane] = s;
         __syncthreads();
         if (k == 0 && ok) {
-            const f32x4 r = (s + comb[0][lane]) + (comb[1][lane] + comb[2][lane]);
+            const f32x4 r = vkn_gr_combine(s, comb[0][lane], comb[1][lane], comb[2][lane]);
             *reinterpret_cast<f32x4*>(xraw + (size_t)row * C + c4) = r;
-            if (status && !(fabsf(r[0]) <= 3.0e38f && fabsf(r[1]) <= 3.0e38f && fabsf(r[2]) <= 3.0e38f && fabsf(r[3]) <= 3.0e38f))
-                atomicOr(status, 1);
+            if (status && vkn_gr_bad(r)) atomicOr(status, VKN_STATUS_RANGE);
         }
     }
     if (k == 1) {
-        const float* cp = cntp + (size_t)b * G * NPT + n;
-        float s = 0.f;
-        for (int gi = lane; gi < G; gi += 64) s += cp[(size_t)gi * NPT];
-        s = vkn_wave_sum(s);
+        const float s = vkn_gr_count(cntp + (size_t)b * G * NPT + n, NPT, G, lane);
         if (lane == 0) cnt[row] = s;
     }
 }
@@ -521,6 +511,11 @@
     return VKN_OK;
 }
 
+int vkn_gather_tickets(int B, int N) {
+    const long long t = (long long)B * (((N + 31) / 32 * 32 + 127) / 128);
+    return t <= VKN_GR_TICKETS ? (int)t : 0;
+}
+
 int vkn_gather_groups(int B, int P) {
     int wg_per_frame = 256 / (B > 0 ? B : 1);
     if (wg_per_frame < 1) wg_per_frame = 1;
@@ -530,18 +525,19 @@
 }
 
 int vkn_launch_gather(const float* x, const float* masks, float thr, float* xraw, float* cnt, float* part, float* cntp,
-                      int B, int N, int C, int P, hipStream_t stream, int xdt, int* status, const void* touch, size_t touch_bytes) {
-    return vkn_launch_gather_ex(x, masks, thr, xraw, cnt, part, cntp, B, N, C, P, N, stream, xdt, status, touch, touch_bytes);
+                      int B, int N, int C, int P, hipStream_t stream, int xdt, int* status, const void* touch, size_t touch_bytes,
+                      unsigned* ticket) {
+    return vkn_launch_gather_ex(x, masks, thr, xraw, cnt, part, cntp, B, N, C, P, N, stream, xdt, status, touch, touch_bytes, ticket);
 }
 
 static int gather_launch(const float* x, const float* masks, float thr, float* xraw, float* cnt, float* part, float* cntp, int B,
                          int N, int C, int P, int mask_rows, int bits, hipStream_t stream, int xdt = 0, int* status = nullptr,
-                         const void* touch = nullptr, size_t touch_bytes = 0, int x_alias = -1);
+                         const void* touch = nullptr, size_t touch_bytes = 0, int x_alias = -1, unsigned* ticket = nullptr);
 
 int vkn_launch_gather_ex(const float* x, const float* masks, float thr, float* xraw, float* cnt, float* part, float* cntp,
                          int B, int N, int C, int P, int mask_rows, hipStream_t stream, int xdt, int* status, const void* touch,
-                         size_t touch_bytes) {
-    return gather_launch(x, masks, thr, xraw, cnt, part, cntp, B, N, C, P, mask_rows, 0, stream, xdt, status, touch, touch_bytes);
+                         size_t touch_bytes, unsigned* ticket) {
+    return gather_launch(x, masks, thr, xraw, cnt, part, cntp, B, N, C, P, mask_rows, 0, stream, xdt, status, touch, touch_bytes, -1, ticket);
 }
 
 int vkn_launch_gather_real(const float* x, const float* a, float* xraw, float* cnt, float* part, float* cntp, int B, int N, int C,
@@ -557,15 +553,15 @@
 }
 
 int vkn_launch_gather_bits(const float* x, const unsigned* bits, float* xraw, float* cnt, float* part, float* cntp, int B, int N,
-                           int C, int P, hipStream_t stream, int xdt, int* status, const void* touch, size_t touch_bytes) {
+                           int C, int P, hipStream_t stream, int xdt, int* status, const void* touch, size_t touch_bytes, unsigned* ticket) {
     if ((P % 64) != 0) return VKN_E_SHAPE;
     return gather_launch(x, reinterpret_cast<const float*>(bits), 0.f, xraw, cnt, part, cntp, B, N, C, P, N, 1, stream, xdt, status, touch,
-                         touch_bytes);
+                         touch_bytes, -1, ticket);
 }
 
 static int gather_launch(const float* x, const float* masks, float thr, float* xraw, float* cnt, float* part, float* cntp, int B,
                          int N, int C, int P, int mask_rows, int bits, hipStream_t stream, int xdt, int* status, const void* touch,
-                         size_t touch_bytes, int x_alias) {
+                         size_t touch_bytes, int x_alias, unsigned* ticket) {
     if (x_alias >= 0 && bits != 2) return VKN_E_ARG;
     if (B <= 0 || N <= 0 || P <= 0 || mask_rows < N) return VKN_E_ARG;
     if (xdt < 0 || xdt > 2) return VKN_E_ARG;
@@ -581,16 +577,20 @@
     const int ileave = ((P % 64) == 0 && vkn_dbg_env("VKN_GATHER_ILEAVE", 1) != 0) ? 1 : 0;
     const bool wave_indep = bits == 1 && xdt == 0 && vkn_dbg_env("VKN_GATHER_BITS_W", 1) != 0 && (C % 32) == 0 &&
                             (px_per_wg % 64) == 0;
+    const bool in_pass = ticket && bits < 2 && B <= VKN_GR_TICKETS;
+    if (touch_bytes >= (1ull << 31)) touch = nullptr;
     for (int n0 = 0; n0 < NPT; n0 += 128) {
         const int nb = (NPT - n0 >= 128) ? 4 : (NPT - n0) / 32;
         dim3 grid(G, B, 1), block(GA_THREADS);
+        VknGrTail tl{};
+        if (in_pass) tl = VknGrTail{xraw, cnt, ticket, status, n0 + 128 >= NPT ? static_cast<const char*>(touch) : nullptr, (unsigned)touch_bytes};
         if (wave_indep) {
             const size_t ldsw = (size_t)GA_WAVES * 2 * 2 * 32 * GA_LDR * sizeof(_Float16) + 4096;
             const unsigned* bw = reinterpret_cast<const unsigned*>(masks);
 #define GA_WLAUNCH(NBV)                                                                                              \
     case NBV:                                                                                                        \
         VKN_ALLOW_FULL_LDS(k_gather_bits_w<NBV>);                                                                    \
-        hipLaunchKernelGGL(k_gather_bits_w<NBV>, grid, block, ldsw, stream, x, bw, part, cntp, N, NPT, n0, C, P, px_per_wg, ileave); \
+        hipLaunchKernelGGL(k_gather_bits_w<NBV>, grid, block, ldsw, stream, x, bw, part, cntp, N, NPT, n0, C, P, px_per_wg, ileave, tl); \
         break;
             switch (nb) {
                 GA_WLAUNCH(1)
@@ -609,7 +609,7 @@
     do {                                                                                                         \
         VKN_ALLOW_FULL_LDS((k_gather_mfma<NBV, BV, XHV>));                                                       \
         hipLaunchKernelGGL((k_gather_mfma<NBV, BV, XHV>), grid, block, lds, stream, x, masks, thr, part, cntp, N, NPT, n0, C, P, \
-                           px_per_wg, mask_fs, ileave, x_alias);                                                 \
+                           px_per_wg, mask_fs, ileave, x_alias, tl);                                             \
     } while (0)
 #define GA_CASE(NBV)                                 \
     case NBV:                                        \
@@ -634,8 +634,9 @@
 #undef GA_LAUNCH
         VKN_CHECK_LAUNCH();
     }
+    if (in_pass) return VKN_OK;
     hipLaunchKernelGGL(k_gather_reduce, dim3(B * N), dim3(256), 0, stream, part, cntp, xraw, cnt, N, NPT, C, G, status,
-                       static_cast<const char*>(touch), (unsigned)(touch_bytes < (1ull << 31) ? touch_bytes : 0));
+                       static_cast<const char*>(touch), (unsigned)touch_bytes);
     VKN_CHECK_LAUNCH();
     return VKN_OK;
 }
diff --git a/video-k-net_amd/csrc/vkn_gather_tail.h b/video-k-net_amd/csrc/vkn_gather_tail.h
--- /dev/null
+++ b/video-k-net_amd/csrc/vkn_gather_tail.h
@@ -0,0 +1,130 @@
+#pragma once
+#include "vkn_common.h"
+
+template <int NCH, int R, int D>
+__device__ __forceinline__ void vkn_gr_walk(const float* (&pc)[R], size_t gstride, int G, int k0, f32x4 (&s)[R][NCH]) {
+    const int G4 = G & ~3;
+#pragma unroll
+    for (int r = 0; r < R; ++r)
+#pragma unroll
+        for (int c = 0; c < NCH; ++c) s[r][c] = f32x4{0.f, 0.f, 0.f, 0.f};
+    int gi = k0;
+    for (; gi + 4 * (D - 1) < G4; gi += 4 * D) {
+        f32x4 v[R][D][NCH];
+#pragma unroll
+        for (int r = 0; r < R; ++r)
+#pragma unroll
+            for (int u = 0; u < D; ++u)
+#pragma unroll
+                for (int c = 0; c < NCH; ++c) v[r][u][c] = *reinterpret_cast<const f32x4*>(pc[r] + (size_t)(gi + 4 * u + c) * gstride);
+#pragma unroll
+        for (int r = 0; r < R; ++r)
+#pragma unroll
+            for (int u = 0; u < D; ++u)
+#pragma unroll
+                for (int c = 0; c < NCH; ++c) s[r][c] += v[r][u][c];
+    }
+    for (; gi < G4; gi += 4) {
+        f32x4 v[R][NCH];
+#pragma unroll
+        for (int r = 0; r < R; ++r)
+#pragma unroll
+            for (int c = 0; c < NCH; ++c) v[r][c] = *reinterpret_cast<const f32x4*>(pc[r] + (size_t)(gi + c) * gstride);
+#pragma unroll
+        for (int r = 0; r < R; ++r)
+#pragma unroll
+            for (int c = 0; c < NCH; ++c) s[r][c] += v[r][c];
+    }
+    if (k0 == 0)
+        for (gi = G4; gi < G; ++gi) {
+            f32x4 v[R];
+#pragma unroll
+            for (int r = 0; r < R; ++r) v[r] = *reinterpret_cast<const f32x4*>(pc[r] + (size_t)gi * gstride);
+#pragma unroll
+            for (int r = 0; r < R; ++r) s[r][0] += v[r];
+        }
+}
+
+__device__ __forceinline__ f32x4 vkn_gr_combine(const f32x4& s0, const f32x4& s1, const f32x4& s2, const f32x4& s3) { return (s0 + s1) + (s2 + s3); }
+
+__device__ __forceinline__ bool vkn_gr_bad(const f32x4& r) {
+    return !(fabsf(r[0]) <= 3.0e38f && fabsf(r[1]) <= 3.0e38f && fabsf(r[2]) <= 3.0e38f && fabsf(r[3]) <= 3.0e38f);
+}
+
+__device__ __forceinline__ float vkn_gr_count(const float* cp, int NPT, int G, int lane) {
+    float s = 0.f;
+    for (int gi = lane; gi < G; gi += 64) s += cp[(size_t)gi * NPT];
+    return vkn_wave_sum(s);
+}
+
+__device__ __forceinline__ void vkn_gr_store(float* p, float v, bool through) {
+    if (through) __hip_atomic_store(p, v, __ATOMIC_RELAXED, __HIP_MEMORY_SCOPE_AGENT);
+    else *p = v;
+}
+
+#define VKN_GR_TICKETS 126
+
+__device__ __forceinline__ bool vkn_gr_arrive(unsigned* ticket, int t, int G, int* flag) {
+    __builtin_amdgcn_s_waitcnt(0x0F70);
+    __syncthreads();
+    if (threadIdx.x == 0) {
+        __threadfence();
+        const unsigned sh = (t & 1) * 16;
+        const unsigned old = atomicAdd(ticket + (t >> 1), 1u << sh);
+        *flag = (int)(((old >> sh) & 0xFFFFu) == (unsigned)(G - 1));
+    }
+    __syncthreads();
+    const bool last = *flag != 0;
+    if (last) __threadfence();
+    return last;
+}
+
+__device__ __forceinline__ void vkn_gr_tail(const float* part, const float* cntp, float* __restrict__ xraw, float* __restrict__ cnt, unsigned* ticket,
+                                            int t, int b, int G, int N, int NPT, int C, int n_lo, int n_hi, int* status) {
+    const int lane = threadIdx.x & 63, nwave = blockDim.x >> 6;
+    const int wave = __builtin_amdgcn_readfirstlane(threadIdx.x >> 6);
+    const size_t gstride = (size_t)NPT * C;
+    const int c4 = lane * 4;
+    const bool ok = c4 < C;
+    const float* pb = part + (size_t)b * G * gstride + (ok ? c4 : 0);
+    const float* cb = cntp + (size_t)b * G * NPT;
+    bool bad = false;
+    constexpr int R = 4;
+    for (int n = n_lo + R * wave; n < n_hi; n += R * nwave) {
+        int nr[R];
+        const float* pc[R];
+        float cr[R];
+#pragma unroll
+        for (int r = 0; r < R; ++r) {
+            nr[r] = min(n + r, n_hi - 1);
+            pc[r] = pb + (size_t)nr[r] * C;
+            cr[r] = vkn_gr_count(cb + nr[r], NPT, G, lane);
+        }
+        f32x4 s[R][4];
+        vkn_gr_walk<4, R, 2>(pc, gstride, G, 0, s);
+#pragma unroll
+        for (int r = 0; r < R; ++r) {
+            if (r && nr[r] != n + r) continue;
+            const f32x4 v = vkn_gr_combine(s[r][0], s[r][1], s[r][2], s[r][3]);
+            if (ok) {
+                *reinterpret_cast<f32x4*>(xraw + ((size_t)b * N + nr[r]) * C + c4) = v;
+                bad |= vkn_gr_bad(v);
+            }
+            if (lane == 0) cnt[(size_t)b * N + nr[r]] = cr[r];
+        }
+    }
+    if (status && bad) atomicOr(status, VKN_STATUS_RANGE);
+    if (threadIdx.x == 0) atomicSub(ticket + (t >> 1), (unsigned)G << ((t & 1) * 16));
+}
+
+__device__ __forceinline__ void vkn_gr_touch(const char* touch, unsigned touch_bytes, unsigned wg, unsigned nwg, unsigned tid0, unsigned nthr) {
+    if (!touch) return;
+    const unsigned per = (touch_bytes / nwg + 15u) & ~15u;
+    const unsigned t0 = wg * per, t1 = min(t0 + per, touch_bytes & ~15u);
+    for (unsigned o = t0 + tid0 * 16u; o < t1; o += 8u * nthr * 16u) {
+        f32x4 v[8];
+#pragma unroll
+        for (unsigned u = 0; u < 8u; ++u) v[u] = *reinterpret_cast<const f32x4*>(touch + min(o + u * nthr * 16u, t1 - 16u));
+        asm volatile("" ::"v"(v[0]), "v"(v[1]), "v"(v[2]), "v"(v[3]), "v"(v[4]), "v"(v[5]), "v"(v[6]), "v"(v[7]));
+    }
+}
diff --git a/video-k-net_amd/csrc/vkn_launch.h b/video-k-net_amd/csrc/vkn_launch.h
--- a/video-k-net_amd/csrc/vkn_launch.h
+++ b/video-k-net_amd/csrc/vkn_launch.h
@@ -37,9 +37,17 @@
 };
 
 int vkn_gather_groups(int B, int P);
+struct VknGrTail {
+    float *xraw, *cnt;
+    unsigned* ticket;
+    int* status;
+    const char* touch;
+    unsigned touch_bytes;
+};
+int vkn_gather_tickets(int B, int N);
 int vkn_launch_gather_ex(const float* x, const float* masks, float thr, float* xraw, float* cnt, float* part, float* cntp,
                          int B, int N, int C, int P, int mask_rows, hipStream_t stream, int xdt = 0, int* status = nullptr,
-                         const void* touch = nullptr, size_t touch_bytes = 0);
+                         const void* touch = nullptr, size_t touch_bytes = 0, unsigned* ticket = nullptr);
 int vkn_launch_gather_ref_ex(const float* x, const float* masks, float thr, float* xraw, float* cnt, int B, int N, int C,
                              int P, int mask_rows, hipStream_t stream);
 int vkn_launch_gather_real(const float* x, const float* a, float* xraw, float* cnt, float* part, float* cntp, int B, int N, int C,
@@ -48,17 +56,17 @@
                            int N, int C, int P, int mask_rows, hipStream_t stream);
 int vkn_launch_gather_bits(const float* x, const unsigned* bits, float* xraw, float* cnt, float* part, float* cntp, int B, int N,
                            int C, int P, hipStream_t stream, int xdt = 0, int* status = nullptr, const void* touch = nullptr,
-                           size_t touch_bytes = 0);
+                           size_t touch_bytes = 0, unsigned* ticket = nullptr);
 int vkn_launch_gather_reduce(const float* part, const float* cntp, float* xraw, float* cnt, int B, int N, int C, int G,
                              hipStream_t stream, int* status = nullptr, const void* touch = nullptr, size_t touch_bytes = 0);
 int vkn_fused_supported(int C, int P);
 int vkn_launch_fused_decode_gather(const float* x, const _Float16* kfh, const _Float16* kfl, const float* kb, float thr,
                                    float* xraw, float* cnt, float* part, float* cntp, int B, int N, int C, int P,
                                    hipStream_t stream, int xdt = 0, int* status = nullptr, const void* touch = nullptr,
-                                   size_t touch_bytes = 0);
+                                   size_t touch_bytes = 0, unsigned* ticket = nullptr);
 int vkn_launch_gather(const float* x, const float* masks, float thr, float* xraw, float* cnt, float* part, float* cntp,
                       int B, int N, int C, int P, hipStream_t stream, int xdt = 0, int* status = nullptr, const void* touch = nullptr,
-                      size_t touch_bytes = 0);
+                      size_t touch_bytes = 0, unsigned* ticket = nullptr);
 int vkn_launch_gather_ref(const float* x, const float* masks, float thr, float* xraw, float* cnt, int B, int N, int C,
                           int P, hipStream_t stream);
 struct VknDecodeStrides {
diff --git a/video-k-net_amd/ops.py b/video-k-net_amd/ops.py
--- a/video-k-net_amd/ops.py
+++ b/video-k-net_amd/ops.py
@@ -22,6 +22,8 @@
 FLAG_CHAIN_BF16X3 = _H['VKN_FLAG_CHAIN_BF16X3']
 FLAG_INIT_SEPARATE = _H['VKN_FLAG_INIT_SEPARATE']
 FLAG_CHAIN_KSPLIT = _H['VKN_FLAG_CHAIN_KSPLIT']
+FLAG_REDUCE_LAUNCH = _H['VKN_FLAG_REDUCE_LAUNCH']
+FLAG_REDUCE_IN_PASS = _H['VKN_FLAG_REDUCE_IN_PASS']
 FLAG_SERIAL_LINK = _H['VKN_FLAG_SERIAL_LINK']
 
 _tls = threading.local()
```

Measured after the change: 10170 frames/s. -1.4%, worse.
